# dmMaze/comic-text-detector

Hardware: NVIDIA H100
Metric: pages/sec @1024x1024 synthetic (higher is better)
Workload: dtype fp16

## Files before the change

comic-text-detector_b200/csrc/engine.cu:

```cuda
#include <cuda.h>
#include <cuda_fp16.h>
#include <cuda_runtime.h>
#include <stdarg.h>
#include <stdio.h>
#include <string.h>

#include <algorithm>
#include <cstdlib>
#include <map>
#include <string>
#include <tuple>
#include <vector>

#include "engine.h"

using namespace ctd;

namespace {
thread_local std::string g_create_error;
}

int ctd_fail(ctd_handle* h, int code, const char* fmt, ...) {
  char buf[512];
  va_list ap;
  va_start(ap, fmt);
  vsnprintf(buf, sizeof(buf), fmt, ap);
  va_end(ap);
  if (h) h->err = buf;
  else g_create_error = buf;
  return code;
}

#define CK(expr)                                                                                      \
  do {                                                                                                \
    cudaError_t _e = (expr);                                                                          \
    if (_e != cudaSuccess) return ctd_fail(h, CTD_E_CUDA, "%s: %s (%s:%d)", #expr, cudaGetErrorString(_e), __FILE__, __LINE__); \
  } while (0)

int rows_per_image(int ph, int pw) { return 3 * ((ph / 8) * (pw / 8) + (ph / 16) * (pw / 16) + (ph / 32) * (pw / 32)); }
static bool is_gemm(int kind) { return kind == CTD_OP_CONV || kind == CTD_OP_DECONV4 || kind == CTD_OP_DETECT; }

extern "C" const char* ctd_last_error(const ctd_handle* h) { return h ? h->err.c_str() : g_create_error.c_str(); }

extern "C" void ctd_destroy(ctd_handle* h) {
  if (!h) return;
  cudaSetDevice(h->cfg.device);
  ctd_pipeline_shutdown(h);
  if (h->ev_pre) {
    cudaEventSynchronize(h->ev_pre);
    cudaEventDestroy(h->ev_pre);
  }
  cudaFree(h->pre_in);
  cudaFree(h->d_pre_tab);
  for (auto& kv : h->plans)
    if (kv.second.graph) cudaGraphExecDestroy(kv.second.graph);
  for (void* p : h->d_buf) cudaFree(p);
  for (void* p : h->d_buf16) cudaFree(p);
  cudaFree(h->d_wsplit);
  cudaFree(h->d_blob); cudaFree(h->d_pages); cudaFree(h->d_blks); cudaFree(h->d_mask); cudaFree(h->d_mask_u8);
  cudaFree(h->d_lines); cudaFree(h->d_bitmap); cudaFree(h->d_labels);
  cudaFree(h->d_ccl_scratch); cudaFree(h->d_nms_ws); cudaFree(h->d_segrep_scratch);
  h->refine_scratch.release(); h->cc_scratch.release(); h->io_scratch.release(); h->in_stage.release();
  if (h->ev0) cudaEventDestroy(h->ev0);
  if (h->ev1) cudaEventDestroy(h->ev1);
  if (h->tev0) cudaEventDestroy(h->tev0);
  if (h->tev1) cudaEventDestroy(h->tev1);
  for (auto e : h->op_events) cudaEventDestroy(e);
  for (Slot& s : h->slot) s.release();
  if (h->ev_fork) cudaEventDestroy(h->ev_fork);
  if (h->ev_join) cudaEventDestroy(h->ev_join);
  if (h->ev_fork2) cudaEventDestroy(h->ev_fork2);
  if (h->ev_xjoin) cudaEventDestroy(h->ev_xjoin);
  if (h->ev_join2) cudaEventDestroy(h->ev_join2);
  if (h->ev_tin) cudaEventDestroy(h->ev_tin);
  if (h->ev_tout) cudaEventDestroy(h->ev_tout);
  if (h->side) cudaStreamDestroy(h->side);
  if (h->side2) cudaStreamDestroy(h->side2);
  if (h->copy_in) cudaStreamDestroy(h->copy_in);
  if (h->copy_out) cudaStreamDestroy(h->copy_out);
  if (h->stream) cudaStreamDestroy(h->stream);
  delete h;
}

extern "C" int ctd_create(ctd_handle** out, const ctd_config* cfg, const ctd_op* ops, int32_t n_ops,
                          const ctd_bufdesc* bufs, int32_t n_bufs, const void* blob, size_t blob_bytes) {
  ctd_handle* h = nullptr;
  if (!out || !cfg || !ops || !bufs || !blob) return ctd_fail(nullptr, CTD_E_INVALID, "null argument");
  *out = nullptr;
  if (cfg->abi_version != CTD_ABI_VERSION) return ctd_fail(nullptr, CTD_E_INVALID, "ABI version mismatch");
  if (cfg->max_h % 64 || cfg->max_w % 64 || cfg->max_batch < 1) return ctd_fail(nullptr, CTD_E_SHAPE, "bad max shape");
  int ndev = 0;
  if (cudaGetDeviceCount(&ndev) != cudaSuccess || ndev <= cfg->device)
    return ctd_fail(nullptr, CTD_E_NO_DEVICE, "no CUDA device %d (this engine has no CPU fallback)", cfg->device);
  cudaDeviceProp prop;
  if (cudaGetDeviceProperties(&prop, cfg->device) != cudaSuccess || prop.major != 9 || prop.minor != 0)
    return ctd_fail(nullptr, CTD_E_NO_DEVICE, "device %d is not sm_90 (compute %d.%d)", cfg->device, prop.major, prop.minor);
  h = new ctd_handle();
  h->cfg = *cfg;
  h->ops.assign(ops, ops + n_ops);
  h->bufs.assign(bufs, bufs + n_bufs);
  {
    h->db_ancestor.assign(size_t(n_ops), 0);
    std::vector<char> needed(size_t(n_bufs), 0);
    bool have_db = false;
    for (int i = n_ops - 1; i >= 0; --i) {
      const ctd_op& op = ops[i];
      bool anc = false;
      if (op.kind == CTD_OP_DB_TAIL && !have_db) { anc = true; have_db = true; }
      else if (have_db && op.kind != CTD_OP_DETECT && op.kind != CTD_OP_SEG_TAIL && op.kind != CTD_OP_DB_TAIL) {
        const int wbuf = op.kind == CTD_OP_SPPF_POOL ? op.src_buf[0] : op.dst_buf;
        anc = wbuf >= 0 && wbuf < n_bufs && needed[wbuf];
      }
      if (!anc) continue;
      h->db_ancestor[size_t(i)] = 1;
      for (int k = 0; k < op.n_src && k < 3; ++k)
        if (op.src_buf[k] >= 0 && op.src_buf[k] < n_bufs) needed[op.src_buf[k]] = 1;
      if (op.residual && op.dst_buf >= 0 && op.dst_buf < n_bufs) needed[op.dst_buf] = 1;
    }
    h->overlap = have_db;
  }
  h->elem = (cfg->precision == CTD_PREC_FP32_SIMT || cfg->precision == CTD_PREC_SPLIT_TC) ? 4 : 2;
  auto bail = [&](int code) { std::string e = h->err; ctd_destroy(h); g_create_error = e; return code; };
  h->detect_prm.assign(size_t(n_ops), {});
  for (int i = 0; i < n_ops; ++i) {
    if (ops[i].kind != CTD_OP_DETECT) continue;
    if (ops[i].p_off < 0 || size_t(ops[i].p_off) + sizeof(h->detect_prm[0]) > blob_bytes) {
      ctd_fail(h, CTD_E_INVALID, "op %d: detect parameters outside the blob", i);
      return bail(CTD_E_INVALID);
    }
    memcpy(h->detect_prm[size_t(i)].data(), static_cast<const char*>(blob) + ops[i].p_off, sizeof(h->detect_prm[0]));
  }
#define CKC(expr)                                                                                        \
  do {                                                                                                   \
    cudaError_t _e = (expr);                                                                             \
    if (_e != cudaSuccess) {                                                                             \
      ctd_fail(h, CTD_E_CUDA, "%s: %s (%s:%d)", #expr, cudaGetErrorString(_e), __FILE__, __LINE__);          \
      return bail(CTD_E_CUDA);                                                                           \
    }                                                                                                    \
  } while (0)
  CKC(cudaSetDevice(cfg->device));
  {
    int lo = 0, hi = 0;
    CKC(cudaDeviceGetStreamPriorityRange(&lo, &hi));
    CKC(cudaStreamCreateWithPriority(&h->stream, cudaStreamNonBlocking, lo));
    CKC(cudaStreamCreateWithPriority(&h->side, cudaStreamNonBlocking, hi));
    CKC(cudaStreamCreateWithPriority(&h->side2, cudaStreamNonBlocking, hi));
  }
  CKC(cudaEventCreateWithFlags(&h->ev_fork, cudaEventDisableTiming));
  CKC(cudaEventCreateWithFlags(&h->ev_join, cudaEventDisableTiming));
  CKC(cudaEventCreateWithFlags(&h->ev_fork2, cudaEventDisableTiming));
  CKC(cudaEventCreateWithFlags(&h->ev_xjoin, cudaEventDisableTiming));
  CKC(cudaEventCreateWithFlags(&h->ev_join2, cudaEventDisableTiming));
  CKC(cudaEventCreateWithFlags(&h->ev_tin, cudaEventDisableTiming));
  CKC(cudaEventCreateWithFlags(&h->ev_tout, cudaEventDisableTiming));
  CKC(cudaEventCreate(&h->ev0));
  CKC(cudaEventCreate(&h->ev1));
  CKC(cudaEventCreate(&h->tev0));
  CKC(cudaEventCreate(&h->tev1));
  {
    void* fn = nullptr;
    cudaDriverEntryPointQueryResult qres;
    CKC(cudaGetDriverEntryPoint("cuTensorMapEncodeTiled", &fn, cudaEnableDefault, &qres));
    if (!fn || qres != cudaDriverEntryPointSuccess) {
      ctd_fail(h, CTD_E_CUDA, "cuTensorMapEncodeTiled not available from the driver");
      return bail(CTD_E_CUDA);
    }
    h->enc = reinterpret_cast<PFN_encodeTiled>(fn);
  }
  CKC(conv_tc_init());
  CKC(conv_ends_init());
  h->blob_bytes = blob_bytes;
  CKC(cudaMalloc(&h->d_blob, blob_bytes));
  CKC(cudaMemcpy(h->d_blob, blob, blob_bytes, cudaMemcpyHostToDevice));
  const size_t nb = size_t(cfg->max_batch), mh = cfg->max_h, mw = cfg->max_w;
  h->d_buf.assign(n_bufs, nullptr);
  for (int i = 0; i < n_bufs; ++i) {
    const size_t bytes = nb * (mh / bufs[i].down) * (mw / bufs[i].down + 4) * bufs[i].channels * h->elem;
    CKC(cudaMalloc(&h->d_buf[i], bytes));
    CKC(cudaMemset(h->d_buf[i], 0, bytes));
  }
  if (cfg->precision == CTD_PREC_SPLIT_TC) {
    h->d_buf16.assign(n_bufs, nullptr);
    for (int i = 0; i < n_bufs; ++i) {
      const size_t bytes = 2 * nb * (mh / bufs[i].down) * (mw / bufs[i].down + 4) * bufs[i].channels * 2;
      CKC(cudaMalloc(&h->d_buf16[i], bytes));
      CKC(cudaMemset(h->d_buf16[i], 0, bytes));
    }
    h->wsplit_off.assign(size_t(n_ops), 0);
    std::vector<__half> ws;
    const char* hb = static_cast<const char*>(blob);
    for (int i = 0; i < n_ops; ++i) {
      const ctd_op& op = ops[i];
      if (!is_gemm(op.kind)) continue;
      int cin = 0;
      for (int k = 0; k < op.n_src; ++k) cin += op.src_c[k];
      const int taps = op.kind == CTD_OP_DECONV4 ? 4 : op.ksize * op.ksize;
      const int nph = op.kind == CTD_OP_DECONV4 ? 4 : 1;
      const size_t cnt = size_t(nph) * op.cout_pad * taps * cin;
      if (size_t(op.w32_off) + cnt * 4 > blob_bytes || size_t(op.w16_off) + cnt * 2 > blob_bytes) {
        ctd_fail(h, CTD_E_INVALID, "op %d: weights outside the blob", i);
        return bail(CTD_E_INVALID);
      }
      while (ws.size() % 128) ws.push_back(__float2half(0.f));
      h->wsplit_off[size_t(i)] = ws.size() * 2;
      const float* w32 = reinterpret_cast<const float*>(hb + op.w32_off);
      const size_t base = ws.size();
      ws.resize(base + 2 * cnt);
      for (size_t k = 0; k < cnt; ++k) {
        const __half hi = __float2half_rn(w32[k]);
        ws[base + k] = hi;
        ws[base + cnt + k] = __float2half_rn((w32[k] - __half2float(hi)) * kSplitLoScale);
      }
    }
    CKC(cudaMalloc(&h->d_wsplit, ws.size() * 2 + 256));
    CKC(cudaMemcpy(h->d_wsplit, ws.data(), ws.size() * 2, cudaMemcpyHostToDevice));
  }
  const size_t px = nb * mh * mw;
  const int no = 5 + cfg->nc;
  CKC(cudaMalloc(&h->d_pages, px * 3));
  CKC(cudaMalloc(&h->d_blks, nb * rows_per_image(mh, mw) * no * sizeof(float)));
  CKC(cudaMalloc(&h->d_mask, px * 4));
  CKC(cudaMalloc(&h->d_lines, px * 2 * 4));
  CKC(cudaMalloc(&h->d_bitmap, px));
  CKC(cudaMalloc(&h->d_labels, px * 4));
  {
    auto al = [](size_t v) { return (v + 255) / 256 * 256; };
    ArenaLayout& L = h->layout;
    L.det = al(px); L.cnt = L.det + al(nb * 300 * 6 * 4); L.nl = L.cnt + al(nb * 4);
    L.lb = L.nl + al(nb * 4); L.ls = L.lb + al(nb * 1000 * 8 * 2); L.lc = L.ls + al(nb * 1000 * 4);
    L.a_bytes = L.lc + al(nb * 4);
    L.refined = L.a_bytes;
    L.blocks = L.refined + al(px);
    const BlockSection bs = block_section_layout();
    L.rec_off = bs.rec_off; L.lines_off = bs.lines_off; L.dist_off = bs.dist_off; L.blocks_stride = bs.stride;
    L.total = L.blocks + nb * L.blocks_stride;
    CKC(cudaMalloc(&h->d_mask_u8, L.total));
    CKC(cudaMemset(h->d_mask_u8, 0, L.total));
    h->d_det = reinterpret_cast<float*>(h->d_mask_u8 + L.det);
    h->d_det_count = reinterpret_cast<int*>(h->d_mask_u8 + L.cnt);
    h->d_nlabels = reinterpret_cast<int32_t*>(h->d_mask_u8 + L.nl);
    h->d_line_boxes = reinterpret_cast<int16_t*>(h->d_mask_u8 + L.lb);
    h->d_line_scores = reinterpret_cast<float*>(h->d_mask_u8 + L.ls);
    h->d_line_count = reinterpret_cast<int32_t*>(h->d_mask_u8 + L.lc);
  }
  CKC(cudaMalloc(&h->d_ccl_scratch, px * 4 * 3));
  CKC(cudaMalloc(&h->d_segrep_scratch, segrep_scratch_bytes(int(nb), int(mh), int(mw), 1000)));
  const int cap = 4096;
  CKC(cudaMalloc(&h->d_nms_ws, nms_workspace_bytes(int(nb), cap)));
  nms_workspace_bind(h->nms, h->d_nms_ws, int(nb), cap);
  CKC(cudaDeviceSynchronize());
#undef CKC
  *out = h;
  return CTD_OK;
}

static int op_geom(ctd_handle* h, const ctd_op& op, int n, int ph, int pw, ConvGeom& g) {
  memset(&g, 0, sizeof(g));
  fill_conv_geom_taps(g, op.kind == CTD_OP_DETECT ? CTD_OP_CONV : op.kind, op.ksize, op.stride);
  g.n_img = n;
  g.n_src = op.n_src;
  const ctd_bufdesc& sb = h->bufs[op.src_buf[0]];
  g.src_h = ph / sb.down;
  g.src_w = pw / sb.down;
  g.cin_total = 0;
  for (int s = 0; s < op.n_src; ++s) {
    const ctd_bufdesc& b = h->bufs[op.src_buf[s]];
    if (b.down != sb.down) return ctd_fail(h, CTD_E_INVALID, "op sources differ in resolution");
    g.src_c[s] = op.src_c[s];
    g.src_cstride[s] = b.channels;
    g.cin_total += op.src_c[s];
  }
  g.k_total = g.taps * g.cin_total;
  g.gh = op.kind == CTD_OP_DECONV4 ? g.src_h : g.src_h / op.stride;
  g.gw = op.kind == CTD_OP_DECONV4 ? g.src_w : g.src_w / op.stride;
  g.dst_h = g.gh * g.out_mul;
  g.dst_w = g.gw * g.out_mul;
  g.cout = op.cout;
  g.cout_pad = op.cout_pad;
  if (op.dst_buf >= 0) {
    g.dst_cstride = h->bufs[op.dst_buf].channels;
    g.dst_coff = op.dst_coff;
  }
  g.act = op.act;
  g.residual = op.residual;
  return CTD_OK;
}

template <typename P>
static void set_detect(const ctd_handle* h, size_t i, int ph, int pw, P& p) {
  p.blks = h->d_blks;
  p.blks_rows_per_img = rows_per_image(ph, pw);
  int row0 = 0;
  for (int l = 0; l < h->ops[i].aux; ++l) row0 += 3 * (ph / (8 << l)) * (pw / (8 << l));
  p.level_row0 = row0;
  p.nc = h->cfg.nc;
  p.det_stride = h->detect_prm[i][0];
  for (int k = 0; k < 6; ++k) p.anchor_wh[k] = h->detect_prm[i][1 + k];
}

static bool runs_on_tensor_cores(int precision, int kind) {
  switch (precision) {
    case CTD_PREC_SPLIT_TC: return is_gemm(kind);
    case CTD_PREC_FP16_TC: return is_gemm(kind) || kind == CTD_OP_STEM || kind == CTD_OP_SEG_TAIL;
    default: return false;
  }
}

static int build_plans(ctd_handle* h, int n, int ph, int pw, ShapePlan& sp) {
  sp.tc.resize(h->ops.size());
  sp.ends.resize(h->ops.size());
  const bool split = h->cfg.precision == CTD_PREC_SPLIT_TC;
  for (size_t i = 0; i < h->ops.size(); ++i) {
    const ctd_op& op = h->ops[i];
    if (!runs_on_tensor_cores(h->cfg.precision, op.kind)) continue;
    const float* bias = reinterpret_cast<const float*>(h->d_blob + op.b_off);
    const char* e = nullptr;
    if (op.kind == CTD_OP_STEM) {
      const bool f16 = sp.input == INPUT_F32;
      e = conv_ends_plan_stem(sp.ends[i], h->enc, f16 ? static_cast<const void*>(h->in_stage.p) : h->d_pages, f16, n,
                              ph, pw, h->d_blob + op.w16_off, bias, static_cast<__half*>(h->d_buf[op.dst_buf]),
                              h->bufs[op.dst_buf].channels, op.dst_coff, op.cout, op.act);
    } else if (op.kind == CTD_OP_SEG_TAIL) {
      if (op.cout_pad != 16) return ctd_fail(h, CTD_E_INVALID, "op %zu: seg tail needs cout_pad 16", i);
      const ctd_bufdesc& sb = h->bufs[op.src_buf[0]];
      e = conv_ends_plan_seg(sp.ends[i], h->enc, static_cast<const __half*>(h->d_buf[op.src_buf[0]]), sb.channels,
                             op.src_coff[0], op.src_c[0], n, ph / sb.down, pw / sb.down, h->d_blob + op.w16_off,
                             h->d_mask, h->d_mask_u8);
    } else {
      ConvGeom g;
      if (int rc = op_geom(h, op, n, ph, pw, g)) return rc;
      const void* src[CTD_MAX_SRC];
      int coff[CTD_MAX_SRC];
      for (int s = 0; s < op.n_src; ++s) {
        src[s] = (split ? h->d_buf16 : h->d_buf)[op.src_buf[s]];
        coff[s] = op.src_coff[s];
      }
      const void* w = split ? h->d_wsplit + h->wsplit_off[i] : h->d_blob + op.w16_off;
      __half* dst = op.kind == CTD_OP_DETECT ? nullptr : static_cast<__half*>(h->d_buf[op.dst_buf]);
      e = conv_tc_plan(sp.tc[i], h->enc, g, src, coff, w, bias, dst, split);
      if (op.kind == CTD_OP_DETECT) set_detect(h, i, ph, pw, sp.tc[i].p);
    }
    if (e) return ctd_fail(h, CTD_E_INVALID, "op %zu: %s", i, e);
  }
  return CTD_OK;
}

template <typename T>
static int run_op_simt(ctd_handle* h, size_t i, int n, int ph, int pw) {
  const ctd_op& op = h->ops[i];
  ConvSimtParams p;
  memset(&p, 0, sizeof(p));
  if (int rc = op_geom(h, op, n, ph, pw, p.g)) return rc;
  for (int k = 0; k < op.n_src; ++k)
    p.src[k] = static_cast<char*>(h->d_buf[op.src_buf[k]]) + size_t(op.src_coff[k]) * sizeof(T);
  p.w = h->d_blob + (sizeof(T) == 4 ? op.w32_off : op.w16_off);
  p.bias = reinterpret_cast<const float*>(h->d_blob + op.b_off);
  if (op.kind == CTD_OP_DETECT) set_detect(h, i, ph, pw, p);
  else p.dst = h->d_buf[op.dst_buf];
  CK(conv_simt_launch<T>(p, h->stream));
  return CTD_OK;
}

template <typename T>
static int run_op_thin(ctd_handle* h, const ctd_op& op, int n, int ph, int pw, int input) {
  cudaStream_t s = h->stream;
  const ctd_bufdesc* sb = op.kind == CTD_OP_STEM ? nullptr : &h->bufs[op.src_buf[0]];
  const int sh = sb ? ph / sb->down : ph, sw = sb ? pw / sb->down : pw;
  const T* src = sb ? static_cast<const T*>(h->d_buf[op.src_buf[0]]) + op.src_coff[0] : nullptr;
  switch (op.kind) {
    case CTD_OP_STEM: {
      const float* w = reinterpret_cast<const float*>(h->d_blob + op.w32_off);
      const float* b = reinterpret_cast<const float*>(h->d_blob + op.b_off);
      T* dst = static_cast<T*>(h->d_buf[op.dst_buf]);
      const int dc = h->bufs[op.dst_buf].channels;
      if (input == INPUT_U8) {
        CK(stem_launch<T>(h->d_pages, n, ph, pw, w, b, dst, dc, op.dst_coff, op.cout, op.act, s));
      } else {
        CK(stem_launch<T>(reinterpret_cast<const float*>(h->in_stage.p), n, ph, pw, w, b, dst, dc, op.dst_coff,
                          op.cout, op.act, s));
      }
      return CTD_OK;
    }
    case CTD_OP_AVGPOOL2:
      CK(avgpool2_launch<T>(src, n, sh, sw, op.src_c[0], sb->channels,
                            static_cast<T*>(h->d_buf[op.dst_buf]) + op.dst_coff, h->bufs[op.dst_buf].channels, s));
      return CTD_OK;
    case CTD_OP_SPPF_POOL:
      CK(sppf_pool_launch<T>(static_cast<T*>(h->d_buf[op.src_buf[0]]) + op.src_coff[0], n, sh, sw, op.src_c[0],
                             sb->channels, s));
      return CTD_OK;
    case CTD_OP_UPSAMPLE2:
      CK(upsample2_launch<T>(src, n, sh, sw, op.src_c[0], sb->channels,
                             static_cast<T*>(h->d_buf[op.dst_buf]) + op.dst_coff, h->bufs[op.dst_buf].channels, s));
      return CTD_OK;
    case CTD_OP_SEG_TAIL:
      CK(seg_tail_launch<T>(src, n, sh, sw, op.src_c[0], sb->channels,
                            reinterpret_cast<const float*>(h->d_blob + op.p_off), h->d_mask, h->d_mask_u8, s));
      return CTD_OK;
    case CTD_OP_DB_TAIL:
      CK(db_tail_launch<T>(src, n, sh, sw, sb->channels, reinterpret_cast<const float*>(h->d_blob + op.p_off),
                           h->d_lines, h->d_bitmap, h->cfg.db_thresh, s));
      return CTD_OK;
    default: return ctd_fail(h, CTD_E_INVALID, "run_op_thin: bad kind %d", op.kind);
  }
}

static int split_written_slice(ctd_handle* h, const ctd_op& op, int n, int ph, int pw, int* cnt) {
  int buf = op.dst_buf, coff = op.dst_coff, c = op.cout;
  if (op.kind == CTD_OP_SPPF_POOL) { buf = op.src_buf[0]; coff = op.src_coff[0] + op.src_c[0]; c = 3 * op.src_c[0]; }
  else if (op.kind == CTD_OP_AVGPOOL2 || op.kind == CTD_OP_UPSAMPLE2) c = op.src_c[0];
  if (buf < 0 || c <= 0) return CTD_OK;
  const ctd_bufdesc& b = h->bufs[buf];
  const size_t npix = size_t(n) * (ph / b.down) * (pw / b.down);
  __half* hi = static_cast<__half*>(h->d_buf16[buf]) + coff;
  CK(split_planes_launch(static_cast<const float*>(h->d_buf[buf]) + coff, hi, hi + npix * b.channels, npix, c, b.channels,
                         h->stream));
  ++*cnt;
  return CTD_OK;
}

static int run_one_op(ctd_handle* h, size_t i, int n, int ph, int pw, const ShapePlan& sp, int* cnt) {
  const ctd_op& op = h->ops[i];
  const ConvTcPlan& tc = sp.tc[i];
  int rc = CTD_OK;
  if (tc.block_n || sp.ends[i].kind != ctd::CTD_END_NONE) {
    const cudaError_t e = tc.block_n ? conv_tc_launch(tc, h->stream) : conv_ends_launch(sp.ends[i], h->stream);
    if (e != cudaSuccess) rc = ctd_fail(h, CTD_E_CUDA, "tensor-core op %zu: %s", i, cudaGetErrorString(e));
  } else if (is_gemm(op.kind)) {
    rc = h->elem == 4 ? run_op_simt<float>(h, i, n, ph, pw) : run_op_simt<__half>(h, i, n, ph, pw);
  } else {
    rc = h->elem == 4 ? run_op_thin<float>(h, op, n, ph, pw, sp.input) : run_op_thin<__half>(h, op, n, ph, pw, sp.input);
  }
  ++*cnt;
  if (rc || h->d_buf16.empty()) return rc;
  return split_written_slice(h, op, n, ph, pw, cnt);
}

int launch_nms(ctd_handle* h, int n, int ph, int pw, cudaStream_t s, int* cnt, const int32_t* half) {
  CK(nms_launch(h->d_blks, n, rows_per_image(ph, pw), h->cfg.nc, h->cfg.conf_thresh, h->cfg.nms_thresh, h->nms, h->d_det,
                h->d_det_count, s, half));
  *cnt += kNmsLaunches;
  return CTD_OK;
}

int launch_db_post(ctd_handle* h, int n, int ph, int pw, cudaStream_t s, int* cnt) {
  CK(ccl_launch(h->d_bitmap, n, ph, pw, h->d_labels, h->d_ccl_scratch, h->d_nlabels, s));
  CK(segrep_launch(h->d_bitmap, h->d_lines, size_t(2) * ph * pw, h->d_ccl_scratch, n, ph, pw, 1000, 1.5f,
                   h->d_segrep_scratch, h->d_line_boxes, h->d_line_scores, h->d_line_count, s));
  *cnt += kCclLaunches + kSegrepLaunches;
  return CTD_OK;
}

static int run_ops(ctd_handle* h, int n, int ph, int pw, const ShapePlan& sp, int* launches, bool record = false) {
  int cnt = 0;
  size_t evi = 0;
  if (h->overlap && !record && !h->cfg.debug_skip_postproc) {
    for (size_t i = 0; i < h->ops.size(); ++i)
      if (h->db_ancestor[i])
        if (int rc = run_one_op(h, i, n, ph, pw, sp, &cnt)) return rc;
    CK(cudaEventRecord(h->ev_fork, h->stream));
    CK(cudaStreamWaitEvent(h->side, h->ev_fork, 0));
    if (int rc = launch_db_post(h, n, ph, pw, h->side, &cnt)) return rc;
    CK(cudaEventRecord(h->ev_join, h->side));
    size_t last_detect = h->ops.size();
    for (size_t i = 0; i < h->ops.size(); ++i)
      if (!h->db_ancestor[i] && h->ops[i].kind == CTD_OP_DETECT) last_detect = i;
    bool nms_forked = false;
    for (size_t i = 0; i < h->ops.size(); ++i) {
      if (h->db_ancestor[i]) continue;
      if (int rc = run_one_op(h, i, n, ph, pw, sp, &cnt)) return rc;
      if (i == last_detect) {
        CK(cudaEventRecord(h->ev_fork2, h->stream));
        CK(cudaStreamWaitEvent(h->side2, h->ev_fork2, 0));
        if (int rc = launch_nms(h, n, ph, pw, h->side2, &cnt)) return rc;
        CK(cudaEventRecord(h->ev_join2, h->side2));
        nms_forked = true;
      }
    }
    if (!nms_forked) {
      if (int rc = launch_nms(h, n, ph, pw, h->stream, &cnt)) return rc;
    } else {
      CK(cudaStreamWaitEvent(h->stream, h->ev_join2, 0));
    }
    CK(cudaStreamWaitEvent(h->stream, h->ev_join, 0));
    *launches = cnt;
    return CTD_OK;
  }
  if (record) CK(cudaEventRecord(h->op_events[evi++], h->stream));
  for (size_t i = 0; i < h->ops.size(); ++i) {
    if (int rc = run_one_op(h, i, n, ph, pw, sp, &cnt)) return rc;
    if (record) CK(cudaEventRecord(h->op_events[evi++], h->stream));
  }
  *launches = cnt;
  if (h->cfg.debug_skip_postproc) return CTD_OK;
  if (int rc = launch_nms(h, n, ph, pw, h->stream, &cnt)) return rc;
  if (record) CK(cudaEventRecord(h->op_events[evi++], h->stream));
  if (int rc = launch_db_post(h, n, ph, pw, h->stream, &cnt)) return rc;
  if (record) CK(cudaEventRecord(h->op_events[evi++], h->stream));
  *launches = cnt;
  return CTD_OK;
}

static size_t stage_elem(const ctd_handle* h) { return h->cfg.precision == CTD_PREC_FP16_TC ? 2 : 4; }

static int find_plan(ctd_handle* h, int32_t n, int32_t ph, int32_t pw, ShapePlan** out, int input = INPUT_U8) {
  if (n < 1 || n > h->cfg.max_batch) return ctd_fail(h, CTD_E_CAPACITY, "batch %d exceeds max_batch %d", n, h->cfg.max_batch);
  if (ph % 64 || pw % 64 || ph > h->cfg.max_h || pw > h->cfg.max_w || ph < 64 || pw < 64)
    return ctd_fail(h, CTD_E_SHAPE, "page %dx%d must be a multiple of 64 and <= %dx%d", ph, pw, h->cfg.max_h, h->cfg.max_w);
  CK(cudaSetDevice(h->cfg.device));
  auto key = std::make_tuple(int(n), int(ph), int(pw), input);
  auto it = h->plans.find(key);
  if (it == h->plans.end()) {
    ShapePlan sp;
    sp.input = input;
    if (input == INPUT_F32) {
      const size_t bytes = size_t(h->cfg.max_batch) * h->cfg.max_h * h->cfg.max_w * 3 * stage_elem(h);
      if (int rc = h->in_stage.grow(h, bytes, std::nullopt, size_t(1) << 40)) return rc;
    }
    if (int rc = build_plans(h, n, ph, pw, sp)) return rc;
    it = h->plans.emplace(key, std::move(sp)).first;
  }
  *out = &it->second;
  return CTD_OK;
}

int prepare_forward(ctd_handle* h, int32_t n, int32_t ph, int32_t pw, ShapePlan** out, int input) {
  ShapePlan* sp = nullptr;
  if (int rc = find_plan(h, n, ph, pw, &sp, input)) return rc;
  if (h->cfg.use_graph && !sp->graph) {
    cudaGraph_t graph;
    CK(cudaStreamBeginCapture(h->stream, cudaStreamCaptureModeThreadLocal));
    int rc = run_ops(h, n, ph, pw, *sp, &sp->launches);
    cudaError_t e = cudaStreamEndCapture(h->stream, &graph);
    if (rc) return rc;
    CK(e);
    CK(cudaGraphInstantiate(&sp->graph, graph, 0));
    cudaGraphDestroy(graph);
  }
  *out = sp;
  return CTD_OK;
}

int enqueue_forward(ctd_handle* h, int32_t n, int32_t ph, int32_t pw, ShapePlan& sp) {
  if (sp.graph) {
    CK(cudaGraphLaunch(sp.graph, h->stream));
  } else {
    if (int rc = run_ops(h, n, ph, pw, sp, &sp.launches)) return rc;
  }
  CK(cudaEventRecord(h->ev1, h->stream));
  h->last_launches = sp.launches;
  h->n = n; h->ph = ph; h->pw = pw;
  h->have_forward = true;
  return CTD_OK;
}

extern "C" int ctd_forward(ctd_handle* h, const uint8_t* pages, int32_t n, int32_t ph, int32_t pw,
                           int32_t pages_on_device) {
  if (!h || !pages) return CTD_E_INVALID;
  ShapePlan* sp = nullptr;
  if (int rc = prepare_forward(h, n, ph, pw, &sp)) return rc;
  const size_t bytes = size_t(n) * ph * pw * 3;
  CK(cudaEventRecord(h->ev0, h->stream));
  CK(cudaMemcpyAsync(h->d_pages, pages, bytes, pages_on_device ? cudaMemcpyDeviceToDevice : cudaMemcpyHostToDevice,
                     h->stream));
  return enqueue_forward(h, n, ph, pw, *sp);
}

template <typename T>
__global__ void from_f32_kernel(const float* src, T* dst, size_t n) {
  size_t i = blockIdx.x * size_t(blockDim.x) + threadIdx.x;
  if (i < n) dst[i] = T(src[i]);
}

template <typename X>
static int copy_output(ctd_handle* h, X* dst, const float* src, size_t elems) {
  if constexpr (sizeof(X) == 4) {
    CK(cudaMemcpyAsync(dst, src, elems * 4, cudaMemcpyDeviceToDevice, h->stream));
  } else {
    from_f32_kernel<__half><<<unsigned((elems + 255) / 256), 256, 0, h->stream>>>(src, dst, elems);
    CK(cudaGetLastError());
  }
  return CTD_OK;
}

template <typename X>
static int forward_tensor(ctd_handle* h, const X* x, int32_t n, int32_t ph, int32_t pw, void* stream, X* blks, X* mask,
                          X* lines) {
  if (!h || !x) return CTD_E_INVALID;
  if (reinterpret_cast<uintptr_t>(x) % 16) return ctd_fail(h, CTD_E_INVALID, "x must be 16-byte aligned");
  ShapePlan* sp = nullptr;
  if (int rc = prepare_forward(h, n, ph, pw, &sp, INPUT_F32)) return rc;
  cudaStream_t cs = static_cast<cudaStream_t>(stream);
  CK(cudaEventRecord(h->ev_tin, cs));
  CK(cudaStreamWaitEvent(h->stream, h->ev_tin, 0));
  CK(cudaEventRecord(h->ev0, h->stream));
  if (stage_elem(h) == 2)
    CK(nchw_to_hwc_launch(x, n, ph, pw, reinterpret_cast<__half*>(h->in_stage.p), h->stream));
  else
    CK(nchw_to_hwc_launch(x, n, ph, pw, reinterpret_cast<float*>(h->in_stage.p), h->stream));
  if (int rc = enqueue_forward(h, n, ph, pw, *sp)) return rc;
  const size_t px = size_t(n) * ph * pw;
  if (blks)
    if (int rc = copy_output(h, blks, h->d_blks, size_t(n) * rows_per_image(ph, pw) * (5 + h->cfg.nc))) return rc;
  if (mask)
    if (int rc = copy_output(h, mask, h->d_mask, px)) return rc;
  if (lines)
    if (int rc = copy_output(h, lines, h->d_lines, px * 2)) return rc;
  CK(cudaEventRecord(h->ev_tout, h->stream));
  CK(cudaStreamWaitEvent(cs, h->ev_tout, 0));
  return CTD_OK;
}

extern "C" int ctd_forward_tensor(ctd_handle* h, const float* x, int32_t n, int32_t ph, int32_t pw, void* stream,
                                  float* blks, float* mask, float* lines) {
  return forward_tensor(h, x, n, ph, pw, stream, blks, mask, lines);
}

extern "C" int ctd_forward_tensor_f16(ctd_handle* h, const void* x, int32_t n, int32_t ph, int32_t pw, void* stream,
                                      void* blks, void* mask, void* lines) {
  return forward_tensor(h, static_cast<const __half*>(x), n, ph, pw, stream, static_cast<__half*>(blks),
                        static_cast<__half*>(mask), static_cast<__half*>(lines));
}

template <bool kPinned>
int GrowBuf<kPinned>::grow(ctd_handle* h, size_t bytes, std::optional<cudaStream_t> sync, size_t headroom) {
  if (bytes <= cap) return CTD_OK;
  if (sync) CK(cudaStreamSynchronize(*sync));
  release();
  const size_t alloc = bytes + bytes / headroom;
  if (kPinned) CK(cudaHostAlloc(reinterpret_cast<void**>(&p), alloc, cudaHostAllocDefault));
  else CK(cudaMalloc(reinterpret_cast<void**>(&p), alloc));
  cap = alloc;
  return CTD_OK;
}
template <bool kPinned>
void GrowBuf<kPinned>::release() {
  if (kPinned && p) cudaFreeHost(p);
  if (!kPinned) cudaFree(p);
  p = nullptr;
  cap = 0;
}
template struct GrowBuf<false>;
template struct GrowBuf<true>;

void Slot::release() {
  cudaFree(d_stage_in);
  cudaFree(d_stage_out);
  for (cudaEvent_t e : {ev_in_done, ev_in_free, ev_out_ready, ev_out_done, ev_post_done})
    if (e) cudaEventDestroy(e);
  if (pinned) cudaFreeHost(pinned);
  pg_in.release(); pg_res.release(); pg_aux.release(); out_in.release(); d_crop.release(); h_crop.release();
  cudaFree(d_pg_tab);
  if (h_pg_tab) cudaFreeHost(h_pg_tab);
  *this = Slot();
}

extern "C" int ctd_resize_linear_u8(ctd_handle* h, const uint8_t* src, int32_t sh, int32_t sw, int32_t channels, uint8_t* dst,
                                    int32_t dh, int32_t dw) {
  if (!h || !src || !dst) return CTD_E_INVALID;
  if ((channels != 1 && channels != 3) || sh < 1 || sw < 1 || dh < 1 || dw < 1) return ctd_fail(h, CTD_E_SHAPE, "bad resize shape");
  CK(cudaSetDevice(h->cfg.device));
  const size_t sb = size_t(sh) * sw * channels, db = size_t(dh) * dw * channels;
  const size_t so = (sb + 255) / 256 * 256;
  if (int rc = h->io_scratch.grow(h, so + db, h->stream)) return rc;
  CK(cudaMemcpyAsync(h->io_scratch.p, src, sb, cudaMemcpyHostToDevice, h->stream));
  CK(resize_linear_u8_launch(h->io_scratch.p, sh, sw, size_t(sw) * channels, channels, h->io_scratch.p + so, dh, dw, dh, dw, h->stream));
  CK(cudaMemcpyAsync(dst, h->io_scratch.p + so, db, cudaMemcpyDeviceToHost, h->stream));
  CK(cudaStreamSynchronize(h->stream));
  return CTD_OK;
}

extern "C" int ctd_join(ctd_handle* h, ctd_handle* other) {
  if (!h || !other) return CTD_E_INVALID;
  if (h == other) return CTD_OK;
  if (h->cfg.device != other->cfg.device) return ctd_fail(h, CTD_E_INVALID, "ctd_join: handles live on different devices");
  CK(cudaSetDevice(h->cfg.device));
  CK(cudaEventRecord(other->ev_xjoin, other->stream));
  CK(cudaStreamWaitEvent(h->stream, other->ev_xjoin, 0));
  return CTD_OK;
}

#define NEED_FWD()                                                                     \
  if (!h) return CTD_E_INVALID;                                                        \
  if (!h->have_forward) return ctd_fail(h, CTD_E_INVALID, "no forward pass has been run"); \
  CK(cudaSetDevice(h->cfg.device));

extern "C" int ctd_get_net_outputs(ctd_handle* h, float* blks, float* mask, float* lines) {
  NEED_FWD();
  const size_t px = size_t(h->n) * h->ph * h->pw;
  if (blks)
    CK(cudaMemcpyAsync(blks, h->d_blks, size_t(h->n) * rows_per_image(h->ph, h->pw) * (5 + h->cfg.nc) * 4,
                       cudaMemcpyDeviceToHost, h->stream));
  if (mask) CK(cudaMemcpyAsync(mask, h->d_mask, px * 4, cudaMemcpyDeviceToHost, h->stream));
  if (lines) CK(cudaMemcpyAsync(lines, h->d_lines, px * 8, cudaMemcpyDeviceToHost, h->stream));
  CK(cudaStreamSynchronize(h->stream));
  return CTD_OK;
}

extern "C" int ctd_get_mask_u8(ctd_handle* h, uint8_t* mask_u8) {
  NEED_FWD();
  if (!mask_u8) return CTD_E_INVALID;
  CK(cudaMemcpyAsync(mask_u8, h->d_mask_u8, size_t(h->n) * h->ph * h->pw, cudaMemcpyDeviceToHost, h->stream));
  CK(cudaStreamSynchronize(h->stream));
  return CTD_OK;
}

extern "C" int ctd_get_detections(ctd_handle* h, float* det, int32_t* det_count) {
  NEED_FWD();
  if (!det || !det_count) return CTD_E_INVALID;
  CK(cudaMemcpyAsync(det, h->d_det, size_t(h->n) * 300 * 6 * 4, cudaMemcpyDeviceToHost, h->stream));
  CK(cudaMemcpyAsync(det_count, h->d_det_count, size_t(h->n) * 4, cudaMemcpyDeviceToHost, h->stream));
  CK(cudaStreamSynchronize(h->stream));
  return CTD_OK;
}

extern "C" int ctd_get_nms_status(ctd_handle* h, int32_t* cand_total, int32_t* cap) {
  if (!h) return CTD_E_INVALID;
  CK(cudaSetDevice(h->cfg.device));
  if (cap) *cap = h->nms.cap;
  if (cand_total) {
    const int n = h->have_forward ? h->n : 1;
    CK(cudaMemcpyAsync(cand_total, h->nms.cand_total, size_t(n) * 4, cudaMemcpyDeviceToHost, h->stream));
    CK(cudaStreamSynchronize(h->stream));
  }
  return CTD_OK;
}

extern "C" int ctd_get_db_components(ctd_handle* h, uint8_t* bitmap, int32_t* labels, int32_t* n_labels) {
  NEED_FWD();
  const size_t px = size_t(h->n) * h->ph * h->pw;
  if (bitmap) CK(cudaMemcpyAsync(bitmap, h->d_bitmap, px, cudaMemcpyDeviceToHost, h->stream));
  if (labels) CK(cudaMemcpyAsync(labels, h->d_labels, px * 4, cudaMemcpyDeviceToHost, h->stream));
  if (n_labels) CK(cudaMemcpyAsync(n_labels, h->d_nlabels, size_t(h->n) * 4, cudaMemcpyDeviceToHost, h->stream));
  CK(cudaStreamSynchronize(h->stream));
  return CTD_OK;
}

extern "C" int ctd_get_text_lines(ctd_handle* h, int16_t* boxes, float* scores, int32_t* counts) {
  NEED_FWD();
  if (!boxes || !scores || !counts) return CTD_E_INVALID;
  CK(cudaMemcpyAsync(boxes, h->d_line_boxes, size_t(h->n) * 1000 * 8 * 2, cudaMemcpyDeviceToHost, h->stream));
  CK(cudaMemcpyAsync(scores, h->d_line_scores, size_t(h->n) * 1000 * 4, cudaMemcpyDeviceToHost, h->stream));
  CK(cudaMemcpyAsync(counts, h->d_line_count, size_t(h->n) * 4, cudaMemcpyDeviceToHost, h->stream));
  CK(cudaStreamSynchronize(h->stream));
  return CTD_OK;
}

extern "C" int ctd_seg_represent(ctd_handle* h, const float* pred, int32_t ih, int32_t iw, float thresh, int16_t* boxes,
                                 float* scores, int32_t* count) {
  if (!h || !pred || !boxes || !scores || !count) return CTD_E_INVALID;
  if (ih < 1 || iw < 1 || size_t(ih) * iw > size_t(h->cfg.max_h) * h->cfg.max_w || ih > 2048 || iw > 2048)
    return ctd_fail(h, CTD_E_CAPACITY, "map larger than the workspace");
  CK(cudaSetDevice(h->cfg.device));
  const size_t px = size_t(ih) * iw;
  CK(cudaMemcpyAsync(h->d_lines, pred, px * 4, cudaMemcpyHostToDevice, h->stream));
  CK(binarize_launch(h->d_lines, px, thresh, h->d_bitmap, h->stream));
  CK(ccl_launch(h->d_bitmap, 1, ih, iw, h->d_labels, h->d_ccl_scratch, h->d_nlabels, h->stream));
  CK(segrep_launch(h->d_bitmap, h->d_lines, px, h->d_ccl_scratch, 1, ih, iw, 1000, 1.5f, h->d_segrep_scratch,
                   h->d_line_boxes, h->d_line_scores, h->d_line_count, h->stream));
  CK(cudaMemcpyAsync(boxes, h->d_line_boxes, 1000 * 8 * 2, cudaMemcpyDeviceToHost, h->stream));
  CK(cudaMemcpyAsync(scores, h->d_line_scores, 1000 * 4, cudaMemcpyDeviceToHost, h->stream));
  CK(cudaMemcpyAsync(count, h->d_line_count, 4, cudaMemcpyDeviceToHost, h->stream));
  CK(cudaStreamSynchronize(h->stream));
  h->have_forward = false;
  return CTD_OK;
}

extern "C" int ctd_last_forward_ms(ctd_handle* h, float* ms) {
  NEED_FWD();
  if (!ms) return CTD_E_INVALID;
  CK(cudaEventSynchronize(h->ev1));
  CK(cudaEventElapsedTime(ms, h->ev0, h->ev1));
  return CTD_OK;
}

extern "C" int ctd_last_launch_count(ctd_handle* h, int32_t* launches) {
  NEED_FWD();
  if (!launches) return CTD_E_INVALID;
  *launches = h->last_launches;
  return CTD_OK;
}

extern "C" int ctd_timer_start(ctd_handle* h) {
  if (!h) return CTD_E_INVALID;
  CK(cudaSetDevice(h->cfg.device));
  CK(cudaEventRecord(h->tev0, h->stream));
  return CTD_OK;
}
extern "C" int ctd_timer_stop(ctd_handle* h, float* ms) {
  if (!h || !ms) return CTD_E_INVALID;
  CK(cudaSetDevice(h->cfg.device));
  CK(cudaEventRecord(h->tev1, h->stream));
  CK(cudaEventSynchronize(h->tev1));
  CK(cudaEventElapsedTime(ms, h->tev0, h->tev1));
  return CTD_OK;
}

extern "C" int ctd_profile_forward(ctd_handle* h, const uint8_t* pages, int32_t n, int32_t ph, int32_t pw,
                                   int32_t pages_on_device, float* op_ms, int32_t cap) {
  if (!h || !pages || !op_ms) return CTD_E_INVALID;
  const int need = int(h->ops.size()) + 2;
  if (cap < need) return ctd_fail(h, CTD_E_INVALID, "op_ms needs %d entries", need);
  ShapePlan* sp = nullptr;
  if (int rc = find_plan(h, n, ph, pw, &sp)) return rc;
  while (int(h->op_events.size()) < need + 1) {
    cudaEvent_t e;
    CK(cudaEventCreate(&e));
    h->op_events.push_back(e);
  }
  CK(cudaMemcpyAsync(h->d_pages, pages, size_t(n) * ph * pw * 3,
                     pages_on_device ? cudaMemcpyDeviceToDevice : cudaMemcpyHostToDevice, h->stream));
  int launches = 0;
  if (int rc = run_ops(h, n, ph, pw, *sp, &launches, true)) return rc;
  CK(cudaStreamSynchronize(h->stream));
  const int nev = h->cfg.debug_skip_postproc ? int(h->ops.size()) : need;
  for (int i = 0; i < need; ++i) op_ms[i] = 0.f;
  for (int i = 0; i < nev; ++i) CK(cudaEventElapsedTime(&op_ms[i], h->op_events[i], h->op_events[i + 1]));
  h->n = n; h->ph = ph; h->pw = pw;
  h->have_forward = true;
  h->last_launches = launches;
  return CTD_OK;
}

template <typename T>
__global__ void to_f32_kernel(const T* src, float* dst, size_t n) {
  size_t i = blockIdx.x * size_t(blockDim.x) + threadIdx.x;
  if (i < n) dst[i] = float(src[i]);
}

extern "C" int ctd_debug_read_buffer(ctd_handle* h, int32_t buf, float* out, size_t out_elems) {
  NEED_FWD();
  if (buf < 0 || buf >= int(h->bufs.size()) || !out) return ctd_fail(h, CTD_E_INVALID, "bad buffer id");
  const ctd_bufdesc& b = h->bufs[buf];
  const size_t elems = size_t(h->n) * (h->ph / b.down) * (h->pw / b.down) * b.channels;
  if (out_elems < elems) return ctd_fail(h, CTD_E_INVALID, "buffer %d holds %zu elements", buf, elems);
  float* tmp = nullptr;
  CK(cudaMalloc(&tmp, elems * 4));
  if (h->elem == 4) to_f32_kernel<float><<<unsigned((elems + 255) / 256), 256, 0, h->stream>>>(static_cast<float*>(h->d_buf[buf]), tmp, elems);
  else to_f32_kernel<__half><<<unsigned((elems + 255) / 256), 256, 0, h->stream>>>(static_cast<__half*>(h->d_buf[buf]), tmp, elems);
  cudaError_t e = cudaMemcpyAsync(out, tmp, elems * 4, cudaMemcpyDeviceToHost, h->stream);
  if (e == cudaSuccess) e = cudaStreamSynchronize(h->stream);
  cudaFree(tmp);
  CK(e);
  return CTD_OK;
}

extern "C" int ctd_debug_write_buffer(ctd_handle* h, int32_t buf, const float* in, int32_t n, int32_t ph, int32_t pw) {
  if (!h || !in) return CTD_E_INVALID;
  if (buf < 0 || buf >= int(h->bufs.size())) return ctd_fail(h, CTD_E_INVALID, "bad buffer id");
  if (n < 1 || n > h->cfg.max_batch || ph > h->cfg.max_h || pw > h->cfg.max_w) return ctd_fail(h, CTD_E_CAPACITY, "shape");
  CK(cudaSetDevice(h->cfg.device));
  const ctd_bufdesc& b = h->bufs[buf];
  const size_t elems = size_t(n) * (ph / b.down) * (pw / b.down) * b.channels;
  float* tmp = nullptr;
  CK(cudaMalloc(&tmp, elems * 4));
  cudaError_t e = cudaMemcpyAsync(tmp, in, elems * 4, cudaMemcpyHostToDevice, h->stream);
  if (e == cudaSuccess) {
    if (h->elem == 4) from_f32_kernel<float><<<unsigned((elems + 255) / 256), 256, 0, h->stream>>>(tmp, static_cast<float*>(h->d_buf[buf]), elems);
    else from_f32_kernel<__half><<<unsigned((elems + 255) / 256), 256, 0, h->stream>>>(tmp, static_cast<__half*>(h->d_buf[buf]), elems);
    if (h->cfg.precision == CTD_PREC_SPLIT_TC) {
      const size_t npix = elems / b.channels;
      __half* hi = static_cast<__half*>(h->d_buf16[buf]);
      e = split_planes_launch(static_cast<const float*>(h->d_buf[buf]), hi, hi + elems, npix, b.channels, b.channels, h->stream);
    }
    if (e == cudaSuccess) e = cudaStreamSynchronize(h->stream);
  }
  cudaFree(tmp);
  CK(e);
  return CTD_OK;
}

extern "C" int ctd_debug_run_ops(ctd_handle* h, const uint8_t* pages, int32_t n, int32_t ph, int32_t pw, int32_t first_op,
                                 int32_t last_op) {
  if (!h) return CTD_E_INVALID;
  if (first_op < 0 || last_op >= int(h->ops.size()) || first_op > last_op) return ctd_fail(h, CTD_E_INVALID, "bad op range");
  ShapePlan* sp = nullptr;
  if (int rc = find_plan(h, n, ph, pw, &sp)) return rc;
  if (pages) CK(cudaMemcpyAsync(h->d_pages, pages, size_t(n) * ph * pw * 3, cudaMemcpyHostToDevice, h->stream));
  int cnt = 0;
  for (int i = first_op; i <= last_op; ++i)
    if (int rc = run_one_op(h, size_t(i), n, ph, pw, *sp, &cnt)) return rc;
  CK(cudaStreamSynchronize(h->stream));
  h->n = n; h->ph = ph; h->pw = pw;
  h->have_forward = true;
  h->last_launches = cnt;
  return CTD_OK;
}

extern "C" int ctd_debug_postprocess(ctd_handle* h, const float* blks, const float* lines, int32_t n, int32_t ph,
                                     int32_t pw) {
  if (!h || !blks || !lines) return CTD_E_INVALID;
  if (h->cfg.debug_skip_postproc) return ctd_fail(h, CTD_E_INVALID, "ctd_debug_postprocess needs the full pipeline");
  ShapePlan* sp = nullptr;
  if (int rc = find_plan(h, n, ph, pw, &sp)) return rc;
  const size_t hw = size_t(ph) * pw;
  CK(cudaMemcpyAsync(h->d_blks, blks, size_t(n) * rows_per_image(ph, pw) * (5 + h->cfg.nc) * 4, cudaMemcpyHostToDevice,
                     h->stream));
  CK(cudaMemcpyAsync(h->d_lines, lines, size_t(n) * hw * 2 * 4, cudaMemcpyHostToDevice, h->stream));
  for (int i = 0; i < n; ++i)
    CK(binarize_launch(h->d_lines + size_t(i) * 2 * hw, hw, h->cfg.db_thresh, h->d_bitmap + size_t(i) * hw, h->stream));
  int cnt = 0;
  if (int rc = launch_nms(h, n, ph, pw, h->stream, &cnt)) return rc;
  if (int rc = launch_db_post(h, n, ph, pw, h->stream, &cnt)) return rc;
  CK(cudaStreamSynchronize(h->stream));
  h->n = n; h->ph = ph; h->pw = pw;
  h->have_forward = true;
  h->last_launches = cnt;
  return CTD_OK;
}

int cc_device(ctd_handle* h, const uint8_t* d_img, int ih, int iw, int stats_cap, int32_t** d_stats, int32_t* n_labels) {
  const size_t px = size_t(ih) * iw;
  auto al = [](size_t v) { return (v + 255) / 256 * 256; };
  const size_t o_scr = al(px * 4);
  const size_t scr_bytes = al(std::max(px * 12, size_t(stats_cap > 0 ? stats_cap : 0) * 5 * 4));
  const size_t o_nl = o_scr + scr_bytes;
  if (int rc = h->cc_scratch.grow(h, o_nl + 256, h->stream)) return rc;
  uint8_t* base = h->cc_scratch.p;
  int32_t* d_labels = reinterpret_cast<int32_t*>(base);
  int32_t* d_scr = reinterpret_cast<int32_t*>(base + o_scr);
  int32_t* d_nl = reinterpret_cast<int32_t*>(base + o_nl);
  CK(ccl_launch(d_img, 1, ih, iw, d_labels, d_scr, d_nl, h->stream));
  if (stats_cap > 0) CK(ccl_stats_launch(d_labels, ih, iw, d_scr, stats_cap, h->stream));
  CK(cudaMemcpyAsync(n_labels, d_nl, 4, cudaMemcpyDeviceToHost, h->stream));
  CK(cudaStreamSynchronize(h->stream));
  if (d_stats) *d_stats = d_scr;
  return CTD_OK;
}

extern "C" int ctd_connected_components(ctd_handle* h, const uint8_t* img, int32_t ih, int32_t iw, int32_t* labels,
                                        int32_t* stats, int32_t stats_cap, int32_t* n_labels) {
  if (!h || !img || !labels || !n_labels) return CTD_E_INVALID;
  if (ih < 1 || iw < 1 || size_t(ih) * iw > kCclMaxPixels) return ctd_fail(h, CTD_E_SHAPE, "bad image size %dx%d", ih, iw);
  CK(cudaSetDevice(h->cfg.device));
  const size_t px = size_t(ih) * iw;
  if (int rc = h->io_scratch.grow(h, px + 256, h->stream)) return rc;
  CK(cudaMemcpyAsync(h->io_scratch.p, img, px, cudaMemcpyHostToDevice, h->stream));
  int32_t* d_stats = nullptr;
  if (int rc = cc_device(h, h->io_scratch.p, ih, iw, (stats && stats_cap > 0) ? stats_cap : 0, &d_stats, n_labels)) return rc;
  CK(cudaMemcpyAsync(labels, h->cc_scratch.p, px * 4, cudaMemcpyDeviceToHost, h->stream));
  if (stats && stats_cap > 0) CK(cudaMemcpyAsync(stats, d_stats, size_t(stats_cap) * 5 * 4, cudaMemcpyDeviceToHost, h->stream));
  CK(cudaStreamSynchronize(h->stream));
  return CTD_OK;
}

extern "C" int ctd_nms(ctd_handle* h, const float* pred, int32_t rows, float conf_thresh, float iou_thresh, float* det,
                       int32_t* det_count) {
  return ctd_nms_dtype(h, pred, rows, CTD_DTYPE_F32, conf_thresh, iou_thresh, det, det_count);
}

extern "C" int ctd_nms_dtype(ctd_handle* h, const void* pred, int32_t rows, int32_t dtype, float conf_thresh,
                             float iou_thresh, float* det, int32_t* det_count) {
  if (!h || !pred || !det || !det_count) return CTD_E_INVALID;
  if (dtype != CTD_DTYPE_F32 && dtype != CTD_DTYPE_F16) return ctd_fail(h, CTD_E_INVALID, "bad dtype %d", dtype);
  const int no = 5 + h->cfg.nc;
  if (rows > rows_per_image(h->cfg.max_h, h->cfg.max_w) * h->cfg.max_batch)
    return ctd_fail(h, CTD_E_CAPACITY, "too many prediction rows");
  CK(cudaSetDevice(h->cfg.device));
  const size_t elems = size_t(rows) * no;
  const int32_t* d_half = nullptr;
  if (dtype == CTD_DTYPE_F16) {
    std::vector<float> wide(elems);
    const __half* p = static_cast<const __half*>(pred);
    for (size_t i = 0; i < elems; ++i) wide[i] = __half2float(p[i]);
    if (int rc = h->io_scratch.grow(h, 256, h->stream)) return rc;
    const int32_t one = 1;
    CK(cudaMemcpyAsync(h->io_scratch.p, &one, sizeof(one), cudaMemcpyHostToDevice, h->stream));
    CK(cudaMemcpyAsync(h->d_blks, wide.data(), elems * 4, cudaMemcpyHostToDevice, h->stream));
    CK(cudaStreamSynchronize(h->stream));
    d_half = reinterpret_cast<const int32_t*>(h->io_scratch.p);
  } else {
    CK(cudaMemcpyAsync(h->d_blks, pred, elems * 4, cudaMemcpyHostToDevice, h->stream));
  }
  CK(nms_launch(h->d_blks, 1, rows, h->cfg.nc, conf_thresh, iou_thresh, h->nms, h->d_det, h->d_det_count, h->stream,
                d_half));
  CK(cudaMemcpyAsync(det, h->d_det, 300 * 6 * 4, cudaMemcpyDeviceToHost, h->stream));
  CK(cudaMemcpyAsync(det_count, h->d_det_count, 4, cudaMemcpyDeviceToHost, h->stream));
  CK(cudaStreamSynchronize(h->stream));
  h->have_forward = false;
  return CTD_OK;
}
```

comic-text-detector_b200/csrc/engine.h:

```cpp
#pragma once
#include <cuda.h>
#include <cuda_runtime.h>
#include <stdint.h>

#include <math.h>

#include <algorithm>
#include <array>
#include <condition_variable>
#include <deque>
#include <map>
#include <mutex>
#include <optional>
#include <string>
#include <thread>
#include <tuple>
#include <vector>

#include "kernels.h"

using ctd::ConvTcPlan;
using ctd::ConvEndsPlan;
using ctd::NmsWorkspace;
using ctd::PFN_encodeTiled;

struct ArenaLayout {
  size_t det, cnt, nl, lb, ls, lc, a_bytes, refined, blocks, blocks_stride, rec_off, lines_off, dist_off, total;
};

struct BlockSection {
  size_t rec_off, lines_off, dist_off, stride;
};
inline BlockSection block_section_layout() {
  auto al = [](size_t v) { return (v + 255) / 256 * 256; };
  BlockSection b;
  b.rec_off = 64;
  b.lines_off = b.rec_off + al(size_t(CTD_MAX_BLOCKS) * sizeof(ctd_block));
  b.dist_off = b.lines_off + al(size_t(CTD_MAX_BLOCKS) * 32);
  b.stride = b.dist_off + al(size_t(CTD_MAX_BLOCK_DIST) * 8);
  return b;
}

struct Letterbox {
  int unpad_h, unpad_w;
  float ratio_x, ratio_y;
};
inline bool letterbox_of(int ih, int iw, int net_h, int net_w, Letterbox& lb) {
  if (ih < 1 || iw < 1 || net_h < 1 || net_w < 1) return false;
  const double r = std::min(double(net_h) / ih, double(net_w) / iw);
  lb.unpad_w = int(nearbyint(iw * r));
  lb.unpad_h = int(nearbyint(ih * r));
  if (lb.unpad_w < 1 || lb.unpad_h < 1 || lb.unpad_w > net_w || lb.unpad_h > net_h) return false;
  lb.ratio_x = float(double(iw) / double(lb.unpad_w));
  lb.ratio_y = float(double(ih) / double(lb.unpad_h));
  return true;
}

struct PagesHead {
  size_t det, cnt, lb, ls, lc, masks;
};
PagesHead pages_head(int n);

struct JobPage {
  int ih, iw;
  float ratio_x, ratio_y;
  size_t off;
  char* section;
  const uint8_t* mask;
  std::vector<int32_t> wins, boxes;
  std::vector<ctd_region_line> lines;
  std::vector<ctd_region> plan;
  size_t plan_bytes = 0;
};

struct Planes {
  const uint8_t* img;
  uint8_t *mask, *ref, *ref2, *thr;
  size_t total;
};

struct PipeJob {
  int slot = 0, refine_mode = 0;
  char* results_host = nullptr;
  bool rows = false;
  PagesHead head{};
  size_t refined = 0;
  std::vector<JobPage> pages;
  Planes pl{};
  uint8_t* d_blocks = nullptr;
  size_t blocks_bytes = 0;
  int keep_undetected = 0;
  int textheight = 0;
  int results_on_device = 0;
  int refined_input = 0;
  std::vector<ctd_device_page> dev;
  const int32_t* nonfinite = nullptr;
};

struct ctd_handle;
template <bool kPinned>
struct GrowBuf {
  uint8_t* p = nullptr;
  size_t cap = 0;
  int grow(ctd_handle* h, size_t bytes, std::optional<cudaStream_t> sync, size_t headroom = 4);
  void release();
};
using DevBuf = GrowBuf<false>;
using PinnedBuf = GrowBuf<true>;

struct Slot {
  uint8_t* d_stage_in = nullptr;
  uint8_t* d_stage_out = nullptr;
  cudaEvent_t ev_in_done = nullptr, ev_in_free = nullptr, ev_out_ready = nullptr, ev_out_done = nullptr;
  cudaEvent_t ev_post_done = nullptr;
  bool busy = false;
  bool crops = false, on_device = false, masks = true, collected = false;
  int state = 0;
  int rc = 0;
  std::string err;
  char* pinned = nullptr;
  DevBuf pg_in, pg_res, pg_aux;
  DevBuf out_in;
  ctd::PageGeom* h_pg_tab = nullptr;
  ctd::PageGeom* d_pg_tab = nullptr;
  std::vector<ctd_page_entry> dev_pages;
  std::vector<ctd_region> crop_plan;
  std::vector<int32_t> crop_first;
  std::vector<size_t> crop_base;
  DevBuf d_crop;
  PinnedBuf h_crop;
  size_t crop_px_off = 0, crop_bytes = 0;

  void start(bool want_crops, bool want_on_device, bool want_masks = true) {
    crops = want_crops;
    on_device = want_on_device;
    masks = want_masks;
    collected = false;
  }
  void release();
};

struct RefineJob {
  std::vector<ctd::RefineWin> wins;
  std::vector<ctd::RefineChunk> chunks;
  size_t total_px = 0;
  size_t total_words = 0;
  void add(int x1, int y1, int x2, int y2, size_t page_off, int iw, int ih);
  size_t table_bytes() const;
};

struct RegionJob {
  std::vector<ctd::RegionDev> regs;
  std::vector<ctd::RegionTile> tiles;
  size_t out_bytes = 0;
  int add(const ctd_region* plan, int n, const ctd::RegionPage& pg, long long out_base);
  size_t table_bytes() const;
  void write_tables(char* dst) const;
};

enum { INPUT_U8 = 0, INPUT_F32 = 1 };

struct ShapePlan {
  int input = INPUT_U8;
  std::vector<ConvTcPlan> tc;
  std::vector<ConvEndsPlan> ends;
  cudaGraphExec_t graph = nullptr;
  int launches = 0;
};
struct ctd_handle {
  ctd_config cfg{};
  std::vector<ctd_op> ops;
  std::vector<ctd_bufdesc> bufs;
  std::vector<std::array<float, 7>> detect_prm;
  std::string err;
  cudaStream_t stream = nullptr;
  cudaEvent_t ev0 = nullptr, ev1 = nullptr, tev0 = nullptr, tev1 = nullptr;
  std::vector<cudaEvent_t> op_events;
  PFN_encodeTiled enc = nullptr;
  char* d_blob = nullptr;
  size_t blob_bytes = 0;
  std::vector<void*> d_buf;
  std::vector<void*> d_buf16;
  char* d_wsplit = nullptr;
  std::vector<size_t> wsplit_off;
  int elem = 2;
  uint8_t* d_pages = nullptr;
  float* d_blks = nullptr;
  float* d_mask = nullptr;
  uint8_t* d_mask_u8 = nullptr;
  float* d_lines = nullptr;
  uint8_t* d_bitmap = nullptr;
  float* d_det = nullptr;
  int* d_det_count = nullptr;
  int32_t* d_labels = nullptr;
  int32_t* d_nlabels = nullptr;
  int32_t* d_ccl_scratch = nullptr;
  void* d_segrep_scratch = nullptr;
  DevBuf refine_scratch;
  DevBuf cc_scratch;
  DevBuf io_scratch;
  int16_t* d_line_boxes = nullptr;
  float* d_line_scores = nullptr;
  int32_t* d_line_count = nullptr;
  void* d_nms_ws = nullptr;
  NmsWorkspace nms{};
  std::map<std::tuple<int, int, int, int>, ShapePlan> plans;
  DevBuf in_stage;
  cudaEvent_t ev_tin = nullptr, ev_tout = nullptr;
  cudaStream_t copy_in = nullptr, copy_out = nullptr;
  Slot slot[2];
  bool overlap = false;
  cudaStream_t side = nullptr, side2 = nullptr;
  cudaEvent_t ev_fork = nullptr, ev_join = nullptr, ev_fork2 = nullptr, ev_join2 = nullptr;
  cudaEvent_t ev_xjoin = nullptr;
  std::vector<char> db_ancestor;
  ArenaLayout layout{};
  cudaStream_t post = nullptr;
  size_t pipe_pinned_cap = 0;
  std::thread pipe_thread;
  std::mutex pipe_mu;
  std::condition_variable pipe_cv, pipe_done_cv;
  std::deque<PipeJob> pipe_queue;
  bool pipe_quit = false;
  int host_threads = 4;
  size_t pg_gather_off = 0;
  size_t pg_out_off = 0, pg_half_off = 0, pg_flag_off = 0;
  cudaStream_t dev_out = nullptr;
  DevBuf pg_cc;
  DevBuf post_refine;
  uint8_t* pre_in = nullptr;
  size_t pre_in_cap = 0;
  char* d_pre_tab = nullptr;
  cudaEvent_t ev_pre = nullptr;
  int n = 0, ph = 0, pw = 0;
  int last_launches = 0;
  bool have_forward = false;
};


int ctd_fail(ctd_handle* h, int code, const char* fmt, ...);
int prepare_forward(ctd_handle* h, int32_t n, int32_t ph, int32_t pw, ShapePlan** out, int input = INPUT_U8);
int enqueue_forward(ctd_handle* h, int32_t n, int32_t ph, int32_t pw, ShapePlan& sp);
int rows_per_image(int ph, int pw);
int launch_nms(ctd_handle* h, int n, int ph, int pw, cudaStream_t s, int* cnt, const int32_t* half = nullptr);
int launch_db_post(ctd_handle* h, int n, int ph, int pw, cudaStream_t s, int* cnt);
int cc_device(ctd_handle* h, const uint8_t* d_img, int ih, int iw, int stats_cap, int32_t** d_stats, int32_t* n_labels);
int launch_refine(ctd_handle* h, const RefineJob& job, const uint8_t* d_img, const uint8_t* d_mask, int refine_mode,
                  uint8_t* d_out, cudaStream_t st, DevBuf& scratch, char* pinned);
void ctd_pipeline_shutdown(ctd_handle* h);
```

comic-text-detector_b200/csrc/kernels.h:

```cpp
#pragma once
#include <cuda.h>
#include <cuda_fp16.h>
#include <cuda_runtime.h>
#include <stdint.h>

#include "../../include/ctd_b200.h"

namespace ctd {

constexpr int kMaxTaps = 9;

constexpr float kSplitLoScale = 2048.0f;
constexpr float kSplitLoUnscale = 1.0f / 2048.0f;
constexpr int kMaxPhases = 4;

struct ConvGeom {
  int n_img;
  int gh, gw;
  int dst_h, dst_w;
  int out_mul;
  int n_phase;
  int taps;
  int cin_total;
  int k_total;
  int n_src;
  int src_c[CTD_MAX_SRC];
  int src_cstride[CTD_MAX_SRC];
  int src_h, src_w;
  int in_stride;
  int8_t tap_dy[kMaxPhases][kMaxTaps];
  int8_t tap_dx[kMaxPhases][kMaxTaps];
  int cout, cout_pad;
  int dst_cstride, dst_coff;
  int act, residual;
};

void fill_conv_geom_taps(ConvGeom& g, int kind, int ksize, int stride);

struct alignas(64) ConvTcParams {
  CUtensorMap a_map[CTD_MAX_SRC][4];
  CUtensorMap b_map;
  CUtensorMap d_map[kMaxPhases];
  ConvGeom g;
  int kb_elems;
  int src_kblocks[CTD_MAX_SRC];
  int tiles_x, tiles_y;
  int8_t tap_map[kMaxPhases][kMaxTaps];
  __half* dst;
  int dst_map_cols;
  const float* bias;
  float* blks;
  int blks_rows_per_img;
  int level_row0;
  float det_stride;
  float anchor_wh[6];
  int nc;
  int split;
  int split_img_off;
  int split_row_off;
};
static_assert(sizeof(ConvTcParams) <= 4096, "ConvTcParams: kernel parameters are limited to 4 KB");

struct ConvTcPlan {
  ConvTcParams p;
  int block_n;
  int tile_h;
  dim3 grid;
  size_t smem_bytes;
};

typedef CUresult (*PFN_encodeTiled)(CUtensorMap*, CUtensorMapDataType, cuuint32_t, void*, const cuuint64_t*,
                                    const cuuint64_t*, const cuuint32_t*, const cuuint32_t*, CUtensorMapInterleave,
                                    CUtensorMapSwizzle, CUtensorMapL2promotion, CUtensorMapFloatOOBfill);

const char* conv_tc_plan(ConvTcPlan& plan, PFN_encodeTiled enc, const ConvGeom& g, const void* const src_ptr[],
                         const int src_coff[], const void* w16, const float* bias, __half* dst, int split = 0);
cudaError_t conv_tc_launch(const ConvTcPlan& plan, cudaStream_t s);
cudaError_t conv_tc_init();

enum { CTD_END_NONE = 0, CTD_END_STEM = 1, CTD_END_SEG = 2, CTD_END_STEM_F16 = 3 };
struct alignas(64) ConvEndsParams {
  CUtensorMap a_map;
  CUtensorMap b_map;
  CUtensorMap d_map;
  int n_img, gh, gw;
  int tiles_x, tiles_y;
  const float* bias;
  float* mask_f32;
  uint8_t* mask_u8;
};
struct ConvEndsPlan {
  ConvEndsParams p;
  int kind = CTD_END_NONE;
  dim3 grid;
  size_t smem_bytes;
};
const char* conv_ends_plan_stem(ConvEndsPlan& plan, PFN_encodeTiled enc, const void* pages, bool f16_page, int n,
                                int ph, int pw, const void* w16, const float* bias, __half* dst, int dst_cstride,
                                int dst_coff, int cout, int act);
const char* conv_ends_plan_seg(ConvEndsPlan& plan, PFN_encodeTiled enc, const __half* src, int src_cstride,
                               int src_coff, int src_c, int n, int gh, int gw, const void* w16, float* mask_f32,
                               uint8_t* mask_u8);
cudaError_t conv_ends_launch(const ConvEndsPlan& plan, cudaStream_t s);
cudaError_t conv_ends_init();

struct ConvSimtParams {
  ConvGeom g;
  const void* src[CTD_MAX_SRC];
  const void* w;
  const float* bias;
  void* dst;
  float* blks;
  int blks_rows_per_img, level_row0, nc;
  float det_stride;
  float anchor_wh[6];
};
template <typename T>
cudaError_t conv_simt_launch(const ConvSimtParams& p, cudaStream_t s);

template <typename T, typename P>
cudaError_t stem_launch(const P* pages, int n, int h, int w, const float* wgt ,
                        const float* bias, T* dst, int dst_cstride, int dst_coff, int cout, int act, cudaStream_t s);
template <typename X, typename S>
cudaError_t nchw_to_hwc_launch(const X* x, int n, int h, int w, S* dst, cudaStream_t s);
cudaError_t split_planes_launch(const float* src, __half* hi, __half* lo, size_t npix, int c, int cstride,
                                cudaStream_t s);
template <typename T>
cudaError_t avgpool2_launch(const T* src, int n, int h, int w, int c, int src_cstride, T* dst, int dst_cstride,
                            cudaStream_t s);
template <typename T>
cudaError_t sppf_pool_launch(T* buf, int n, int h, int w, int c, int cstride, cudaStream_t s);
template <typename T>
cudaError_t upsample2_launch(const T* src, int n, int h, int w, int c, int src_cstride, T* dst, int dst_cstride,
                             cudaStream_t s);
template <typename T>
cudaError_t seg_tail_launch(const T* src, int n, int h, int w, int c, int cstride, const float* wgt ,
                            float* mask_f32, uint8_t* mask_u8, cudaStream_t s);
template <typename T>
cudaError_t db_tail_launch(const T* src, int n, int h, int w, int cstride, const float* params, float* lines,
                           uint8_t* bitmap, float db_thresh, cudaStream_t s);

struct NmsWorkspace {
  float* cand;
  int* cand_count;
  int* cand_total;
  float* sorted;
  unsigned long long* mask;
  int cap;
};
cudaError_t nms_launch(const float* blks, int n, int rows, int nc, float conf, float iou, NmsWorkspace& ws,
                       float* det , int* det_count, cudaStream_t s, const int32_t* half = nullptr);
constexpr int kNmsLaunches = 5;
size_t nms_workspace_bytes(int n, int cap);
void nms_workspace_bind(NmsWorkspace& ws, void* base, int n, int cap);

cudaError_t ccl_launch(const uint8_t* img, int n, int h, int w, int32_t* labels, int32_t* scratch ,
                       int32_t* n_labels, cudaStream_t s);
constexpr int kCclLaunches = 8;
constexpr size_t kCclMaxPixels = size_t(1) << 28;
cudaError_t ccl_stats_launch(const int32_t* labels, int h, int w, int32_t* stats, int cap, cudaStream_t s);

size_t segrep_scratch_bytes(int n, int h, int w, int max_cand);
cudaError_t segrep_launch(const uint8_t* bitmap, const float* pred, size_t pred_page_stride, const int* Lf, int n, int h,
                          int w, int max_cand, float unclip_ratio, void* scratch, int16_t* boxes, float* scores,
                          int* n_contours, cudaStream_t s);
constexpr int kSegrepLaunches = 15;
cudaError_t binarize_launch(const float* pred, size_t count, float thresh, uint8_t* bitmap, cudaStream_t s);

cudaError_t resize_linear_u8_launch(const uint8_t* src, int sh, int sw, size_t src_pitch, int channels, uint8_t* dst,
                                    int dh, int dw, int canvas_h, int canvas_w, cudaStream_t s);
struct PageGeom {
  long long src_off, dst_off;
  int ih, iw, unpad_h, unpad_w, row0, pad;
};
cudaError_t letterbox_batch_launch(const uint8_t* src, const PageGeom* d_tab, int n, uint8_t* dst, int net_h, int net_w,
                                   cudaStream_t s);
cudaError_t backproject_batch_launch(const uint8_t* mask, int net_h, int net_w, const PageGeom* d_tab, int n,
                                     int total_rows, uint8_t* dst, cudaStream_t s);
enum PreFormat { PRE_F32_NCHW = 0, PRE_F16_NCHW = 1, PRE_U8_NHWC = 2 };
cudaError_t letterbox_tensor_launch(const uint8_t* src, const PageGeom* d_tab, int n, void* dst, int net_h, int net_w,
                                    int format, bool reverse, cudaStream_t s);

struct GatherPage {
  const uint8_t* src;
  long long sh, sw, sc;
  uint8_t* dst;
  int ih, iw, row0, fast, ch, pad;
};
cudaError_t gather_pages_launch(const GatherPage* d_tab, int n, int total_rows, cudaStream_t s);
cudaError_t upload_table_launch(const void* host, size_t bytes, void* dst, cudaStream_t s);

struct OutputGather {
  const void* blks;
  long long bsr, bsc;
  const void* mask;
  long long msh, msw;
  const void* lines;
  long long lsh, lsw;
  int rows, half;
};
cudaError_t gather_outputs_launch(const OutputGather* d_tab, int n, int h, int w, int no, int ws_rows, float thresh,
                                  uint8_t* mask_u8, float* lines, uint8_t* bitmap, float* blks, int32_t* flags,
                                  cudaStream_t s);

struct RefineWin {
  int x1, y1, x2, y2;
  long long off;
  long long page_off;
  int pitch;
};
struct RefineChunk { int win, y0, x0, rows, woff; };
constexpr int kRefineChunkPx = 8192;
__host__ __device__ constexpr int refine_rows_per_chunk(int rw) {
  return kRefineChunkPx / rw >= 8 ? (kRefineChunkPx / rw) & ~3 : (kRefineChunkPx / rw > 0 ? kRefineChunkPx / rw : 1);
}
size_t refine_scratch_bytes(size_t total_px, size_t n_chunks);
size_t refine_mk_state_bytes(int n_wins);
cudaError_t refine_mk_launch(const uint8_t* d_img, const uint8_t* d_mask, const RefineWin* d_wins, int n_wins,
                             const RefineChunk* d_chunks, int n_chunks, int n_multi_chunks, void* d_state, size_t total_px,
                             void* scratch, int refine_mode, uint8_t* d_out, cudaStream_t s);

constexpr int kRegionTilePx = 256;
struct RegionPage {
  const uint8_t* data;
  long long sh, sw, sc;
  int ih, iw;
};
struct RegionDev {
  long long offset;
  const uint8_t* page;
  long long sh, sw, sc;
  int out_h, out_w;
  int warp_w, bw0;
  int rotate, ih, iw, pad;
  double m[9];
};
struct RegionTile { int region, first; };
cudaError_t warp_regions_launch(const RegionDev* d_regs, const RegionTile* d_tiles, int n_tiles, uint8_t* d_out,
                                cudaStream_t s);

}
```

comic-text-detector_b200/csrc/pipeline.cu:

```cuda
#include <cuda.h>
#include <cuda_runtime.h>
#include <math.h>
#include <stdint.h>
#include <string.h>

#include <algorithm>
#include <thread>
#include <vector>

#include "engine.h"

using namespace ctd;

#define CK(expr)                                                                                      \
  do {                                                                                                \
    cudaError_t _e = (expr);                                                                          \
    if (_e != cudaSuccess) return ctd_fail(h, CTD_E_CUDA, "%s: %s (%s:%d)", #expr, cudaGetErrorString(_e), __FILE__, __LINE__); \
  } while (0)

namespace {
inline void norm_slice(int& lo, int& hi, int n) {
  if (lo < 0) lo = std::max(lo + n, 0);
  if (hi < 0) hi = std::max(hi + n, 0);
  lo = std::min(lo, n);
  hi = std::min(hi, n);
  if (hi < lo) hi = lo;
}
}

void RefineJob::add(int x1, int y1, int x2, int y2, size_t page_off, int iw, int ih) {
  norm_slice(x1, x2, iw);
  norm_slice(y1, y2, ih);
  const size_t a = (x2 > x1 && y2 > y1) ? size_t(x2 - x1) * (y2 - y1) : 0;
  if (a == 0) return;
  const int wi = int(wins.size());
  const int rw = x2 - x1, rh = y2 - y1;
  const int rows_per = refine_rows_per_chunk(rw);
  for (int y0 = 0; y0 < rh; y0 += rows_per)
    for (int x0 = 0; x0 < rw; x0 += kRefineChunkPx) {
      const int rows = std::min(rows_per, rh - y0);
      chunks.push_back(RefineChunk{wi, y0, x0, rows, int(total_words)});
      total_words += (size_t(rows) * std::min(rw - x0, kRefineChunkPx) + 31) / 32;
    }
  wins.push_back(RefineWin{x1, y1, x2, y2, (long long)total_px, (long long)page_off, iw});
  total_px = (total_px + a + 3) / 4 * 4;
}
size_t RefineJob::table_bytes() const {
  auto al = [](size_t v) { return (v + 255) / 256 * 256; };
  return al(wins.size() * sizeof(RefineWin)) + al(chunks.size() * sizeof(RefineChunk));
}

int launch_refine(ctd_handle* h, const RefineJob& job, const uint8_t* d_img, const uint8_t* d_mask, int refine_mode,
                  uint8_t* d_out, cudaStream_t st, DevBuf& scratch, char* pinned) {
  if (job.wins.empty()) return CTD_OK;
  auto al = [](size_t v) { return (v + 255) / 256 * 256; };
  const size_t tb = job.table_bytes();
  const size_t sb = refine_mk_state_bytes(int(job.wins.size()));
  if (int rc = scratch.grow(h, tb + sb + refine_scratch_bytes(job.total_px, job.chunks.size()), st, 2)) return rc;
  char* base = reinterpret_cast<char*>(scratch.p);
  const size_t wb = al(job.wins.size() * sizeof(RefineWin));
  std::vector<char> local;
  char* stage = pinned;
  if (!stage) { local.resize(tb); stage = local.data(); }
  memcpy(stage, job.wins.data(), job.wins.size() * sizeof(RefineWin));
  int n_multi = 0;
  {
    RefineChunk* hc = reinterpret_cast<RefineChunk*>(stage + wb);
    const size_t nc = job.chunks.size();
    size_t tail = nc;
    for (size_t i = 0; i < nc;) {
      size_t j = i;
      while (j < nc && job.chunks[j].win == job.chunks[i].win) ++j;
      if (j - i > 1) {
        for (size_t k = i; k < j; ++k) hc[n_multi++] = job.chunks[k];
      } else {
        hc[--tail] = job.chunks[i];
      }
      i = j;
    }
  }
  CK(cudaMemcpyAsync(base, stage, tb, cudaMemcpyHostToDevice, st));
  if (!pinned) CK(cudaStreamSynchronize(st));
  CK(refine_mk_launch(d_img, d_mask, reinterpret_cast<const RefineWin*>(base), int(job.wins.size()),
                      reinterpret_cast<const RefineChunk*>(base + wb), int(job.chunks.size()), n_multi, base + tb,
                      job.total_px, base + tb + sb, refine_mode, d_out, st));
  return CTD_OK;
}

extern "C" int ctd_refine_mask(ctd_handle* h, const uint8_t* img, const uint8_t* mask, int32_t ih, int32_t iw,
                               const int32_t* windows, int32_t n_win, int32_t refine_mode, uint8_t* out) {
  if (!h || !img || !mask || !out || (n_win > 0 && !windows)) return CTD_E_INVALID;
  if (ih < 1 || iw < 1) return ctd_fail(h, CTD_E_SHAPE, "bad image size");
  CK(cudaSetDevice(h->cfg.device));
  RefineJob job;
  for (int i = 0; i < n_win; ++i) job.add(windows[4 * i], windows[4 * i + 1], windows[4 * i + 2], windows[4 * i + 3], 0, iw, ih);
  const size_t px = size_t(ih) * iw, pxa = (px + 255) / 256 * 256;
  if (int rc = h->io_scratch.grow(h, pxa * 5 + 1024, h->stream)) return rc;
  uint8_t* d_img = h->io_scratch.p;
  uint8_t* d_mask = d_img + pxa * 3;
  uint8_t* d_out = d_mask + pxa;
  CK(cudaMemcpyAsync(d_img, img, px * 3, cudaMemcpyHostToDevice, h->stream));
  CK(cudaMemcpyAsync(d_mask, mask, px, cudaMemcpyHostToDevice, h->stream));
  CK(cudaMemsetAsync(d_out, 0, pxa, h->stream));
  if (int rc = launch_refine(h, job, d_img, d_mask, refine_mode, d_out, h->stream, h->refine_scratch, nullptr))
    return rc;
  CK(cudaMemcpyAsync(out, d_out, px, cudaMemcpyDeviceToHost, h->stream));
  CK(cudaStreamSynchronize(h->stream));
  return CTD_OK;
}

namespace {
struct PageIn {
  const float* det; int n_det;
  const int16_t* line_boxes; const float* line_scores; int n_lines;
  const uint8_t* mask; int im_w, im_h;
  float ratio_x, ratio_y;
};

PageIn page_in(const char* res, const PagesHead& head, int i, const JobPage& p) {
  PageIn in;
  in.det = reinterpret_cast<const float*>(res + head.det) + size_t(i) * 300 * 6;
  in.n_det = std::min(std::max(reinterpret_cast<const int32_t*>(res + head.cnt)[i], 0), 300);
  in.line_boxes = reinterpret_cast<const int16_t*>(res + head.lb) + size_t(i) * 1000 * 8;
  in.line_scores = reinterpret_cast<const float*>(res + head.ls) + size_t(i) * 1000;
  in.n_lines = std::min(std::max(reinterpret_cast<const int32_t*>(res + head.lc)[i], 0), 1000);
  in.mask = p.mask; in.im_w = p.iw; in.im_h = p.ih; in.ratio_x = p.ratio_x; in.ratio_y = p.ratio_y;
  return in;
}

std::array<int64_t, 4> expand_textwindow(int64_t x1, int64_t y1, int64_t x2, int64_t y2, int im_w, int im_h) {
  const int64_t w = x2 - x1, h = y2 - y1;
  const int64_t pad = int64_t(nearbyint((double(std::max(h, w)) * 0.25 + double(std::min(h, w)) * 0.75) / 16.0));
  return {std::max<int64_t>(0, x1 - pad), std::max<int64_t>(0, y1 - pad), std::min<int64_t>(im_w - 1, x2 + pad),
          std::min<int64_t>(im_h - 1, y2 + pad)};
}

int host_group_page(const PageIn& in, const BlockSection& L, bool lines_out, JobPage& p) {
  char* section = p.section;
  std::vector<int32_t> bxy(size_t(in.n_det) * 4), bcls(size_t(in.n_det));
  for (int i = 0; i < in.n_det; ++i) {
    const float* d = in.det + 6 * i;
    bxy[4 * i + 0] = int32_t(d[0] * in.ratio_x);
    bxy[4 * i + 1] = int32_t(d[1] * in.ratio_y);
    bxy[4 * i + 2] = int32_t(d[2] * in.ratio_x);
    bxy[4 * i + 3] = int32_t(d[3] * in.ratio_y);
    bcls[i] = int32_t(d[5]);
  }
  std::vector<int32_t> lines;
  lines.reserve(size_t(in.n_lines) * 8);
  for (int i = 0; i < in.n_lines; ++i) {
    if (!(in.line_scores[i] > 0.6f)) continue;
    const int16_t* b = in.line_boxes + 8 * i;
    for (int k = 0; k < 4; ++k) {
      lines.push_back(int32_t(double(b[2 * k]) * double(in.ratio_x)));
      lines.push_back(int32_t(double(b[2 * k + 1]) * double(in.ratio_y)));
    }
  }
  ctd_page_blocks* hdr = reinterpret_cast<ctd_page_blocks*>(section);
  ctd_block* rec = reinterpret_cast<ctd_block*>(section + L.rec_off);
  int32_t* lout = reinterpret_cast<int32_t*>(section + L.lines_off);
  double* dout = reinterpret_cast<double*>(section + L.dist_off);
  int32_t nb = 0;
  int rc = ctd_group_output(bxy.data(), bcls.data(), in.n_det, lines.data(), int32_t(lines.size() / 8), in.im_w, in.im_h, in.mask,
                            1, rec, CTD_MAX_BLOCKS, lout, CTD_MAX_BLOCKS, dout, CTD_MAX_BLOCK_DIST, &nb);
  hdr->flags = 0;
  if (rc == CTD_E_CAPACITY) {
    std::vector<double> big(size_t(CTD_MAX_BLOCKS) * CTD_MAX_BLOCKS / 4);
    rc = ctd_group_output(bxy.data(), bcls.data(), in.n_det, lines.data(), int32_t(lines.size() / 8), in.im_w, in.im_h, in.mask, 1,
                          rec, CTD_MAX_BLOCKS, lout, CTD_MAX_BLOCKS, big.data(), int32_t(big.size()), &nb);
    if (rc == CTD_OK)
      for (int i = 0; i < nb; ++i) { rec[i].n_dist = 0; rec[i].dist_off = 0; }
    hdr->flags |= 1;
  }
  if (rc != CTD_OK) { hdr->n_blocks = 0; hdr->n_lines = 0; hdr->n_dist = 0; hdr->flags |= 2; return rc; }
  hdr->n_blocks = nb;
  int32_t tl = 0, td = 0;
  for (int i = 0; i < nb; ++i) { tl += rec[i].n_lines; td += rec[i].n_dist; }
  hdr->n_lines = tl;
  hdr->n_dist = td;
  for (int i = 0; i < nb; ++i) {
    const int32_t* xy = rec[i].xyxy;
    const auto win = expand_textwindow(xy[0], xy[1], xy[2], xy[3], in.im_w, in.im_h);
    for (int64_t v : win) p.wins.push_back(int32_t(v));
    p.boxes.insert(p.boxes.end(), xy, xy + 4);
  }
  if (!lines_out) return CTD_OK;
  p.lines.reserve(size_t(tl));
  for (int b = 0; b < nb; ++b)
    for (int k = 0; k < rec[b].n_lines; ++k) {
      ctd_region_line l{};
      const int32_t* q = lout + size_t(rec[b].line_off + k) * 8;
      for (int j = 0; j < 8; ++j) l.quad[j] = double(q[j]);
      l.language = rec[b].language;
      l.vertical = rec[b].vertical ? 1 : 0;
      l.font_size = rec[b].font_size;
      p.lines.push_back(l);
    }
  return CTD_OK;
}

template <typename F>
void for_each_page(int n, int threads, F fn) {
  const int nthreads = std::max(1, std::min(n, threads));
  if (nthreads == 1) {
    for (int i = 0; i < n; ++i) fn(i);
    return;
  }
  std::vector<std::thread> th;
  for (int t = 0; t < nthreads; ++t)
    th.emplace_back([&, t] { for (int i = t; i < n; i += nthreads) fn(i); });
  for (auto& x : th) x.join();
}

__global__ void undetected_prep_kernel(uint8_t* __restrict__ mask, const uint8_t* __restrict__ refined,
                                       uint8_t* __restrict__ thr, size_t n) {
  const size_t i = blockIdx.x * size_t(blockDim.x) + threadIdx.x;
  if (i >= n) return;
  uint8_t m = mask[i];
  if (refined[i] > 30) { m = 0; mask[i] = 0; }
  thr[i] = m > 30 ? 255 : 0;
}
__global__ void or_kernel(uint8_t* __restrict__ dst, const uint8_t* __restrict__ src, size_t n) {
  const size_t i = blockIdx.x * size_t(blockDim.x) + threadIdx.x;
  if (i < n) dst[i] |= src[i];
}

int refine_undetected(ctd_handle* h, const std::vector<JobPage>& pages, const Planes& pl, int refine_mode,
                      cudaStream_t st, DevBuf& cc, DevBuf& refine_scratch, char* pinned, size_t pinned_cap) {
  auto al = [](size_t v) { return (v + 255) / 256 * 256; };
  const int n = int(pages.size());
  const size_t total_px = pl.total;
  undetected_prep_kernel<<<unsigned((total_px + 255) / 256), 256, 0, st>>>(pl.mask, pl.ref, pl.thr, total_px);
  CK(cudaGetLastError());
  size_t max_px = 0;
  std::vector<int> cap(static_cast<size_t>(n));
  std::vector<size_t> stats_off(static_cast<size_t>(n));
  for (int i = 0; i < n; ++i) max_px = std::max(max_px, size_t(pages[i].ih) * pages[i].iw);
  const size_t o_scr = al(max_px * 4);
  size_t o = o_scr + al(max_px * 12);
  for (int i = 0; i < n; ++i) {
    cap[size_t(i)] = ((pages[i].ih + 1) / 2) * ((pages[i].iw + 1) / 2) + 2;
    stats_off[size_t(i)] = o;
    o += al(size_t(cap[size_t(i)]) * 5 * 4);
  }
  const size_t o_nl = o;
  if (int rc = cc.grow(h, o_nl + al(size_t(n) * 4), st)) return rc;
  uint8_t* base = cc.p;
  int32_t* d_labels = reinterpret_cast<int32_t*>(base);
  int32_t* d_scr = reinterpret_cast<int32_t*>(base + o_scr);
  int32_t* d_nl = reinterpret_cast<int32_t*>(base + o_nl);
  for (int i = 0; i < n; ++i) {
    const JobPage& p = pages[size_t(i)];
    int32_t* d_stats = reinterpret_cast<int32_t*>(base + stats_off[size_t(i)]);
    CK(ccl_launch(pl.thr + p.off, 1, p.ih, p.iw, d_labels, d_scr, d_nl + i, st));
    CK(ccl_stats_launch(d_labels, p.ih, p.iw, d_stats, cap[size_t(i)], st));
  }
  std::vector<int32_t> n_lab(static_cast<size_t>(n));
  CK(cudaMemcpyAsync(n_lab.data(), d_nl, size_t(n) * 4, cudaMemcpyDeviceToHost, st));
  CK(cudaStreamSynchronize(st));
  std::vector<std::vector<int32_t>> stats(static_cast<size_t>(n));
  for (int i = 0; i < n; ++i) {
    stats[size_t(i)].resize(size_t(std::max(n_lab[size_t(i)], 0)) * 5);
    if (n_lab[size_t(i)] > 0)
      CK(cudaMemcpyAsync(stats[size_t(i)].data(), base + stats_off[size_t(i)], stats[size_t(i)].size() * 4,
                         cudaMemcpyDeviceToHost, st));
  }
  CK(cudaStreamSynchronize(st));
  RefineJob rj2;
  for (int i = 0; i < n; ++i) {
    const JobPage& p = pages[size_t(i)];
    const std::vector<int32_t>& xyxy = p.boxes;
    const size_t nb = xyxy.size() / 4;
    bool first_valid = true;
    for (int li = 0; li < n_lab[size_t(i)]; ++li) {
      const int32_t* s5 = &stats[size_t(i)][size_t(li) * 5];
      if (!(s5[4] > 50)) continue;
      if (first_valid) { first_valid = false; continue; }
      const int64_t bb[4] = {s5[0], s5[1], int64_t(s5[0]) + s5[2], int64_t(s5[1]) + s5[3]};
      int64_t score = -1;
      for (size_t b = 0; b < nb; ++b) {
        const int32_t* q = &xyxy[4 * b];
        const int64_t x1 = std::max<int64_t>(q[0], bb[0]), y1 = std::max<int64_t>(q[1], bb[1]);
        const int64_t x2 = std::min<int64_t>(q[2], bb[2]), y2 = std::min<int64_t>(q[3], bb[3]);
        const int64_t a = (y2 < y1 || x2 < x1) ? -1 : (y2 - y1) * (x2 - x1);
        if (a > score) score = a;
      }
      if (double(score) / double(s5[2]) / double(s5[3]) < 0.5) {
        const auto w4 = expand_textwindow(bb[0], bb[1], bb[2], bb[3], p.iw, p.ih);
        rj2.add(int(w4[0]), int(w4[1]), int(w4[2]), int(w4[3]), p.off, p.iw, p.ih);
      }
    }
  }
  if (!rj2.wins.empty()) {
    CK(cudaMemsetAsync(pl.ref2, 0, total_px, st));
    char* stage = rj2.table_bytes() <= pinned_cap ? pinned : nullptr;
    if (int rc = launch_refine(h, rj2, pl.img, pl.mask, refine_mode, pl.ref2, st, refine_scratch, stage)) return rc;
    or_kernel<<<unsigned((total_px + 255) / 256), 256, 0, st>>>(pl.ref, pl.ref2, total_px);
    CK(cudaGetLastError());
  }
  return CTD_OK;
}
}

extern "C" int ctd_results_layout(ctd_handle* h, ctd_results_layout_t* out) {
  if (!h || !out) return CTD_E_INVALID;
  const ArenaLayout& L = h->layout;
  out->max_batch = h->cfg.max_batch; out->max_h = h->cfg.max_h; out->max_w = h->cfg.max_w; out->reserved = 0;
  out->total_bytes = L.total;
  out->mask_u8 = 0; out->det = L.det; out->det_count = L.cnt; out->n_labels = L.nl;
  out->line_boxes = L.lb; out->line_scores = L.ls; out->line_count = L.lc;
  out->phase_a_bytes = L.a_bytes;
  out->mask_refined = L.refined; out->blocks = L.blocks; out->blocks_stride = L.blocks_stride;
  out->blk_records_off = L.rec_off; out->blk_lines_off = L.lines_off; out->blk_dist_off = L.dist_off;
  return CTD_OK;
}

PagesHead pages_head(int n) {
  auto al = [](size_t v) { return (v + 255) / 256 * 256; };
  const size_t nb = size_t(n);
  PagesHead hd;
  hd.det = 0;
  hd.cnt = hd.det + al(nb * 300 * 6 * 4);
  hd.lb = hd.cnt + al(nb * 4);
  hd.ls = hd.lb + al(nb * 1000 * 8 * 2);
  hd.lc = hd.ls + al(nb * 1000 * 4);
  hd.masks = hd.lc + al(nb * 4);
  return hd;
}

static size_t plan_planes(ctd_page_entry* pages, int n, size_t mask_plane) {
  auto al = [](size_t v) { return (v + 255) / 256 * 256; };
  size_t total = 0;
  for (int i = 0; i < n; ++i) {
    pages[i].page_off = int64_t(total * 3);
    pages[i].mask_off = int64_t(mask_plane + total);
    total += al(size_t(pages[i].ih) * size_t(pages[i].iw));
  }
  for (int i = 0; i < n; ++i) pages[i].refined_off = pages[i].mask_off + int64_t(total);
  return total;
}

extern "C" int ctd_pages_plan(ctd_page_entry* pages, int32_t n, int32_t net_h, int32_t net_w, size_t* input_bytes,
                              size_t* results_bytes) {
  if (!input_bytes || !results_bytes || n < 0 || (n > 0 && !pages)) return CTD_E_INVALID;
  if (net_h < 64 || net_w < 64 || net_h % 64 || net_w % 64) return CTD_E_SHAPE;
  auto al = [](size_t v) { return (v + 255) / 256 * 256; };
  const PagesHead hd = pages_head(n);
  for (int i = 0; i < n; ++i) {
    Letterbox lb;
    if (!letterbox_of(pages[i].ih, pages[i].iw, net_h, net_w, lb)) return CTD_E_SHAPE;
    pages[i].unpad_h = lb.unpad_h;
    pages[i].unpad_w = lb.unpad_w;
  }
  const size_t total = plan_planes(pages, n, hd.masks);
  const size_t stride = al(block_section_layout().stride);
  const size_t blocks = hd.masks + 2 * total;
  for (int i = 0; i < n; ++i) pages[i].blocks_off = int64_t(blocks + size_t(i) * stride);
  *input_bytes = total * 3;
  *results_bytes = blocks + size_t(n) * stride;
  return CTD_OK;
}

extern "C" int ctd_refine_plan(ctd_page_entry* pages, int32_t n, const int32_t* xyxy, const int32_t* n_blocks,
                               int32_t* windows, int32_t* status, size_t* input_bytes, size_t* results_bytes) {
  if (!input_bytes || !results_bytes || n < 0 || (n > 0 && (!pages || !n_blocks))) return CTD_E_INVALID;
  int64_t nb = 0;
  for (int i = 0; i < n; ++i) {
    if (pages[i].ih < 1 || pages[i].iw < 1) return CTD_E_SHAPE;
    if (n_blocks[i] < 0) return CTD_E_INVALID;
    nb += n_blocks[i];
  }
  if (nb > INT32_MAX) return CTD_E_CAPACITY;
  if (nb > 0 && (!xyxy || !windows || !status)) return CTD_E_INVALID;
  for (int i = 0; i < n; ++i) {
    pages[i].unpad_h = pages[i].unpad_w = 0;
    pages[i].blocks_off = 0;
  }
  const size_t total = plan_planes(pages, n, 0);
  size_t b = 0;
  for (int i = 0; i < n; ++i) {
    const int ih = pages[i].ih, iw = pages[i].iw;
    for (int k = 0; k < n_blocks[i]; ++k, ++b) {
      const int32_t* q = xyxy + 4 * b;
      const auto w = expand_textwindow(q[0], q[1], q[2], q[3], iw, ih);
      bool fits = true;
      for (int j = 0; j < 4; ++j) {
        fits = fits && w[j] >= INT32_MIN && w[j] <= INT32_MAX;
        windows[4 * b + j] = int32_t(std::min<int64_t>(std::max<int64_t>(w[j], INT32_MIN), INT32_MAX));
      }
      int x1 = windows[4 * b], y1 = windows[4 * b + 1], x2 = windows[4 * b + 2], y2 = windows[4 * b + 3];
      norm_slice(x1, x2, iw);
      norm_slice(y1, y2, ih);
      status[b] = !fits ? 2 : (x2 > x1 && y2 > y1) ? 0 : 1;
    }
  }
  *input_bytes = total * 5;
  *results_bytes = total * 2;
  return CTD_OK;
}

static int finish_batch(ctd_handle* h, const PipeJob& job, cudaStream_t st) {
  if (!job.results_on_device && job.pl.ref) {
    char* res = job.results_host;
    if (job.keep_undetected) CK(cudaMemcpyAsync(res + job.head.masks, job.pl.mask, job.pl.total, cudaMemcpyDeviceToHost, st));
    CK(cudaMemcpyAsync(res + job.refined, job.pl.ref, job.pl.total, cudaMemcpyDeviceToHost, st));
  }
  CK(cudaEventRecord(h->slot[job.slot].ev_post_done, st));
  return CTD_OK;
}

static std::vector<RegionPage> region_pages(const PipeJob& job) {
  std::vector<RegionPage> src;
  for (size_t i = 0; i < job.pages.size(); ++i) {
    const JobPage& p = job.pages[i];
    if (i < job.dev.size() && job.dev[i].data) {
      const ctd_device_page& d = job.dev[i];
      src.push_back(RegionPage{d.data, (long long)d.stride_h, (long long)d.stride_w, (long long)d.stride_c, p.ih, p.iw});
    } else {
      src.push_back(RegionPage{job.pl.img + p.off * 3, (long long)p.iw * 3, 3, 1, p.ih, p.iw});
    }
  }
  return src;
}

static int crop_stage(ctd_handle* h, Slot& s, const std::vector<RegionPage>& src, const std::vector<JobPage>& pages,
                      bool to_host, cudaStream_t st) {
  const int n = int(src.size());
  RegionJob rg;
  s.crop_plan.clear();
  s.crop_first.assign(size_t(n) + 1, 0);
  s.crop_base.assign(size_t(n) + 1, 0);
  size_t base = 0;
  for (int i = 0; i < n; ++i) {
    const std::vector<ctd_region>& p = pages[size_t(i)].plan;
    if (int bad = rg.add(p.data(), int(p.size()), src[size_t(i)], (long long)base); bad >= 0)
      return ctd_fail(h, CTD_E_INVALID, "malformed crop plan entry %d on page %d of the batch", bad, i);
    s.crop_first[size_t(i)] = int32_t(s.crop_plan.size());
    s.crop_base[size_t(i)] = base;
    for (ctd_region r : p) {
      r.offset += int64_t(base);
      s.crop_plan.push_back(r);
    }
    base += pages[size_t(i)].plan_bytes;
  }
  s.crop_first[size_t(n)] = int32_t(s.crop_plan.size());
  s.crop_base[size_t(n)] = base;
  if (s.crop_plan.size() > size_t(INT32_MAX) || rg.tiles.size() > size_t(INT32_MAX))
    return ctd_fail(h, CTD_E_CAPACITY, "too many crops in one batch");
  s.crop_bytes = base;
  s.crop_px_off = 0;
  if (rg.tiles.empty()) return CTD_OK;
  const size_t tb = rg.table_bytes(), px = s.crop_bytes;
  if (int rc = s.d_crop.grow(h, tb + px, st)) return rc;
  if (int rc = s.h_crop.grow(h, to_host ? tb + px : tb, st)) return rc;
  uint8_t* d_tab = s.d_crop.p;
  rg.write_tables(reinterpret_cast<char*>(s.h_crop.p));
  CK(cudaMemcpyAsync(d_tab, s.h_crop.p, tb, cudaMemcpyHostToDevice, st));
  const size_t rb = (rg.regs.size() * sizeof(RegionDev) + 255) / 256 * 256;
  CK(warp_regions_launch(reinterpret_cast<const RegionDev*>(d_tab), reinterpret_cast<const RegionTile*>(d_tab + rb),
                         int(rg.tiles.size()), d_tab + tb, st));
  if (to_host) CK(cudaMemcpyAsync(s.h_crop.p + tb, d_tab + tb, px, cudaMemcpyDeviceToHost, st));
  s.crop_px_off = tb;
  return CTD_OK;
}

static int host_stage(ctd_handle* h, PipeJob& job) {
  const int n = int(job.pages.size());
  if (!job.rows && job.textheight <= 0) return CTD_OK;
  const BlockSection bs = block_section_layout();
  std::vector<int> prc(size_t(n), CTD_OK), crc(size_t(n), CTD_OK);
  for_each_page(n, h->host_threads, [&](int i) {
    JobPage& p = job.pages[size_t(i)];
    if (job.rows) prc[size_t(i)] = host_group_page(page_in(job.results_host, job.head, i, p), bs, job.textheight > 0, p);
    if (job.textheight > 0 && prc[size_t(i)] == CTD_OK) {
      p.plan.resize(p.lines.size());
      if (!p.lines.empty())
        crc[size_t(i)] = ctd_region_plan(p.lines.data(), int32_t(p.lines.size()), p.iw, p.ih, job.textheight,
                                         p.plan.data(), &p.plan_bytes);
    }
  });
  for (int i = 0; i < n; ++i)
    if (prc[size_t(i)] != CTD_OK) return ctd_fail(h, prc[size_t(i)], "group_output failed on page %d of the batch", i);
  for (int i = 0; i < n; ++i)
    if (crc[size_t(i)] != CTD_OK)
      return ctd_fail(h, crc[size_t(i)], "ctd_region_plan refused page %d of the batch (%dx%d, textheight %d)", i,
                      job.pages[size_t(i)].ih, job.pages[size_t(i)].iw, job.textheight);
  return CTD_OK;
}

static int device_stage(ctd_handle* h, const PipeJob& job, cudaStream_t st, DevBuf& refine_scratch, DevBuf& cc,
                        char* pinned, size_t pinned_cap) {
  if (job.d_blocks)
    CK(cudaMemcpyAsync(job.d_blocks, job.pages[0].section, job.blocks_bytes, cudaMemcpyHostToDevice, st));
  if (job.textheight > 0)
    if (int rc = crop_stage(h, h->slot[job.slot], region_pages(job), job.pages, !job.results_on_device, st)) return rc;
  if (job.pl.ref && !job.refined_input) {
    CK(cudaMemsetAsync(job.pl.ref, 0, job.pl.total, st));
    RefineJob rj;
    for (const JobPage& p : job.pages)
      for (size_t k = 0; k + 3 < p.wins.size(); k += 4)
        rj.add(p.wins[k], p.wins[k + 1], p.wins[k + 2], p.wins[k + 3], p.off, p.iw, p.ih);
    char* stage = rj.table_bytes() <= pinned_cap ? pinned : nullptr;
    if (int rc = launch_refine(h, rj, job.pl.img, job.pl.mask, job.refine_mode, job.pl.ref, st, refine_scratch, stage))
      return rc;
  }
  if (!job.keep_undetected) return CTD_OK;
  return refine_undetected(h, job.pages, job.pl, job.refine_mode, st, cc, refine_scratch, pinned, pinned_cap);
}

static int run_job(ctd_handle* h, PipeJob& job) {
  Slot& s = h->slot[job.slot];
  if (job.rows) {
    CK(cudaEventSynchronize(s.ev_out_done));
    for (int i = 0; job.nonfinite && i < int(job.pages.size()); ++i)
      if (const int32_t f = job.nonfinite[i])
        return ctd_fail(h, CTD_E_INVALID, "page %d of the batch: a non-finite value (NaN or inf) in its %s", i,
                        (f & 1) ? "blks" : (f & 2) ? "mask" : "lines_map");
  }
  if (int rc = host_stage(h, job)) return rc;
  cudaStream_t st = h->post;
  CK(cudaStreamWaitEvent(st, s.ev_out_ready, 0));
  if (int rc = device_stage(h, job, st, h->post_refine, h->pg_cc, s.pinned, h->pipe_pinned_cap)) return rc;
  return finish_batch(h, job, st);
}

static void pipe_worker(ctd_handle* h) {
  cudaSetDevice(h->cfg.device);
  for (;;) {
    PipeJob job;
    {
      std::unique_lock<std::mutex> lk(h->pipe_mu);
      h->pipe_cv.wait(lk, [&] { return h->pipe_quit || !h->pipe_queue.empty(); });
      if (h->pipe_queue.empty()) return;
      job = std::move(h->pipe_queue.front());
      h->pipe_queue.pop_front();
    }
    const int rc = run_job(h, job);
    std::string err;
    if (rc != CTD_OK) err = h->err;
    {
      std::lock_guard<std::mutex> lk(h->pipe_mu);
      Slot& s = h->slot[job.slot];
      s.state = rc == CTD_OK ? 2 : 3;
      s.rc = rc;
      s.err = err;
    }
    h->pipe_done_cv.notify_all();
  }
}

static void queue_job(ctd_handle* h, PipeJob&& job) {
  Slot& s = h->slot[job.slot];
  {
    std::lock_guard<std::mutex> lk(h->pipe_mu);
    s.state = 1;
    h->pipe_queue.push_back(std::move(job));
  }
// ... 823 lines not shown
```

comic-text-detector_b200/csrc/postproc.cu:

```cuda
#include <cuda_fp16.h>
#include <cuda_runtime.h>
#include <limits.h>

#include "kernels.h"

namespace ctd {

constexpr int kCandStride = 8;
constexpr int kMaxDet = 300;
constexpr float kMaxWh = 4096.f;

size_t nms_workspace_bytes(int n, int cap) {
  return size_t(n) * cap * kCandStride * 4 * 2 + size_t(n) * 4 * 8 + size_t(n) * cap * (cap / 64) * 8;
}
void nms_workspace_bind(NmsWorkspace& ws, void* base, int n, int cap) {
  char* p = static_cast<char*>(base);
  ws.cap = cap;
  ws.mask = reinterpret_cast<unsigned long long*>(p);
  p += size_t(n) * cap * (cap / 64) * 8;
  ws.cand = reinterpret_cast<float*>(p);
  p += size_t(n) * cap * kCandStride * 4;
  ws.sorted = reinterpret_cast<float*>(p);
  p += size_t(n) * cap * kCandStride * 4;
  ws.cand_count = reinterpret_cast<int*>(p);
// ... 32 lines not shown
  } else {
    o[0] = x[0] - hw; o[1] = x[1] - hh; o[2] = x[0] + hw; o[3] = x[1] + hh;
  }
  o[4] = __uint_as_float(key); o[5] = float(cls); o[6] = __int_as_float(r); o[7] = 0.f;
}

__device__ __forceinline__ float page_conf(const int32_t* __restrict__ half, int img, float conf_thres, bool* hf) {
  *hf = half && half[img];
  return *hf ? round_half(conf_thres) : conf_thres;
}

__global__ void nms_filter_kernel(const float* __restrict__ blks, int rows, int no, float conf_thres,
                                  const int32_t* __restrict__ half, float* __restrict__ cand,
                                  int* __restrict__ cand_count, int cap) {
  const int img = blockIdx.y;
  const int r = blockIdx.x * blockDim.x + threadIdx.x;
  if (r >= rows) return;
  bool hf;
  const float conf = page_conf(half, img, conf_thres, &hf);
  const float* x = blks + (size_t(img) * rows + r) * no;
  int cls = 0;
  const unsigned key = nms_score_key(x, no, conf, hf, &cls);
  if (key == 0u) return;
  const int slot = atomicAdd(&cand_count[img], 1);
  if (slot >= cap) return;
  write_cand(cand + (size_t(img) * cap + slot) * kCandStride, x, hf, key, cls, r);
}

__global__ void __launch_bounds__(1024) nms_overflow_kernel(const float* __restrict__ blks, int rows, int no,
                                                            float conf_thres, const int32_t* __restrict__ half,
                                                            float* __restrict__ cand,
                                                            int* __restrict__ cand_count, int* __restrict__ cand_total,
                                                            int cap) {
  __shared__ int hist[2048];
  __shared__ unsigned s_prefix, s_maskbits;
  __shared__ int s_need, s_base_take, s_base_tie;
  __shared__ int wsum_take[32], wsum_tie[32];
  const int img = blockIdx.x, t = threadIdx.x, lane = t & 31, wid = t >> 5;
  const int total = cand_count[img];
  if (t == 0) cand_total[img] = total;
  if (total <= cap) return;
  bool hf;
  const float conf = page_conf(half, img, conf_thres, &hf);
  const float* pb = blks + size_t(img) * rows * no;
  if (t == 0) { s_prefix = 0u; s_maskbits = 0u; s_need = cap; }
  const int shifts[3] = {21, 10, 0}, nbins[3] = {2048, 2048, 1024};
#pragma unroll
  for (int lvl = 0; lvl < 3; ++lvl) {
    for (int i = t; i < 2048; i += 1024) hist[i] = 0;
    __syncthreads();
    const unsigned prefix = s_prefix, maskbits = s_maskbits;
    for (int r = t; r < rows; r += 1024) {
      int cls;
      const unsigned key = nms_score_key(pb + size_t(r) * no, no, conf, hf, &cls);
      if (key != 0u && (key & maskbits) == prefix) atomicAdd(&hist[(key >> shifts[lvl]) & unsigned(nbins[lvl] - 1)], 1);
    }
    __syncthreads();
    if (t == 0) {
      int need = s_need, cum = 0, digit = 0;
      for (int b = nbins[lvl] - 1; b >= 0; --b) {
        if (cum + hist[b] >= need) { digit = b; break; }
        cum += hist[b];
      }
      s_need = need - cum;
      s_prefix = prefix | (unsigned(digit) << shifts[lvl]);
      s_maskbits = maskbits | (unsigned(nbins[lvl] - 1) << shifts[lvl]);
    }
    __syncthreads();
  }
  const unsigned T = s_prefix;
  const int need_ties = s_need;
  if (t == 0) { s_base_take = 0; s_base_tie = 0; }
  __syncthreads();
  float* out = cand + size_t(img) * cap * kCandStride;
  for (int r0 = 0; r0 < rows; r0 += 1024) {
    const int r = r0 + t;
    int cls = 0;
    unsigned key = 0u;
    if (r < rows) key = nms_score_key(pb + size_t(r) * no, no, conf, hf, &cls);
    const bool tie = key == T && key != 0u;
    const unsigned tb = __ballot_sync(0xffffffffu, tie);
    if (lane == 0) wsum_tie[wid] = __popc(tb);
    __syncthreads();
    int tie_rank = s_base_tie + __popc(tb & ((1u << lane) - 1u));
    for (int w2 = 0; w2 < wid; ++w2) tie_rank += wsum_tie[w2];
    const bool take = key > T || (tie && tie_rank < need_ties);
    const unsigned kb = __ballot_sync(0xffffffffu, take);
    if (lane == 0) wsum_take[wid] = __popc(kb);
    __syncthreads();
    if (take) {
      int slot = s_base_take + __popc(kb & ((1u << lane) - 1u));
      for (int w2 = 0; w2 < wid; ++w2) slot += wsum_take[w2];
      if (slot < cap) write_cand(out + size_t(slot) * kCandStride, pb + size_t(r) * no, hf, key, cls, r);
    }
    __syncthreads();
    if (t == 0) {
      int a = 0, b = 0;
      for (int w2 = 0; w2 < 32; ++w2) { a += wsum_take[w2]; b += wsum_tie[w2]; }
      s_base_take += a;
      s_base_tie += b;
    }
    __syncthreads();
  }
  if (t == 0) cand_count[img] = cap;
}

template <int P>
__global__ void __launch_bounds__(1024) nms_sort_kernel(const float* __restrict__ cand, int* __restrict__ cand_count,
                                                        float* __restrict__ sorted, int cap) {
  __shared__ float skey[P];
  __shared__ int srow[P];
  __shared__ int sslot[P];
  const int img = blockIdx.x;
  int m = cand_count[img];
  if (m > cap) m = cap;
  const float* c = cand + size_t(img) * cap * kCandStride;
  for (int i = threadIdx.x; i < P; i += blockDim.x) {
    if (i < m) {
      skey[i] = c[i * kCandStride + 4];
      srow[i] = __float_as_int(c[i * kCandStride + 6]);
      sslot[i] = i;
    } else {
      skey[i] = -INFINITY;
      srow[i] = INT_MAX;
      sslot[i] = -1;
    }
  }
  __syncthreads();
  for (int k = 2; k <= P; k <<= 1) {
    for (int j = k >> 1; j > 0; j >>= 1) {
      for (int i = threadIdx.x; i < P; i += blockDim.x) {
        const int ixj = i ^ j;
        if (ixj > i) {
          const bool up = (i & k) == 0;
          const float ka = skey[i], kb = skey[ixj];
          const int ra = srow[i], rb = srow[ixj];
          const bool a_first = (ka > kb) || (ka == kb && ra < rb);
          if (a_first != up) {
            skey[i] = kb; skey[ixj] = ka;
            srow[i] = rb; srow[ixj] = ra;
            const int t = sslot[i]; sslot[i] = sslot[ixj]; sslot[ixj] = t;
          }
        }
      }
      __syncthreads();
    }
  }
  float* o = sorted + size_t(img) * cap * kCandStride;
  for (int i = threadIdx.x; i < m; i += blockDim.x) {
    const int sl = sslot[i];
#pragma unroll
    for (int e = 0; e < kCandStride; ++e) o[i * kCandStride + e] = c[sl * kCandStride + e];
  }
}

__global__ void __launch_bounds__(64) nms_mask_kernel(const float* __restrict__ sorted, const int* __restrict__ cand_count,
                                                      unsigned long long* __restrict__ mask, int cap, float iou_thres) {
  const int img = blockIdx.z;
  int m = cand_count[img];
  if (m > cap) m = cap;
  const int rb = blockIdx.y, cb = blockIdx.x;
  if (rb * 64 >= m || cb * 64 >= m || cb < rb) return;
  __shared__ float cbox[64][5];
  const float* s = sorted + size_t(img) * cap * kCandStride;
  const int cj = cb * 64 + threadIdx.x;
  if (cj < m) {
    const float off = s[cj * kCandStride + 5] * kMaxWh;
    cbox[threadIdx.x][0] = s[cj * kCandStride + 0] + off;
    cbox[threadIdx.x][1] = s[cj * kCandStride + 1] + off;
    cbox[threadIdx.x][2] = s[cj * kCandStride + 2] + off;
    cbox[threadIdx.x][3] = s[cj * kCandStride + 3] + off;
    cbox[threadIdx.x][4] = __fmul_rn(cbox[threadIdx.x][2] - cbox[threadIdx.x][0], cbox[threadIdx.x][3] - cbox[threadIdx.x][1]);
  }
  __syncthreads();
  const int i = rb * 64 + threadIdx.x;
  if (i >= m) return;
  const float off = s[i * kCandStride + 5] * kMaxWh;
  const float x1 = s[i * kCandStride + 0] + off, y1 = s[i * kCandStride + 1] + off;
  const float x2 = s[i * kCandStride + 2] + off, y2 = s[i * kCandStride + 3] + off;
  const float area = __fmul_rn(x2 - x1, y2 - y1);
  unsigned long long bits = 0;
  const int jmax = min(64, m - cb * 64);
  for (int j = 0; j < jmax; ++j) {
    if (cb * 64 + j <= i) continue;
    const float xx1 = fmaxf(x1, cbox[j][0]), yy1 = fmaxf(y1, cbox[j][1]);
    const float xx2 = fminf(x2, cbox[j][2]), yy2 = fminf(y2, cbox[j][3]);
    const float w = fmaxf(0.f, xx2 - xx1), h = fmaxf(0.f, yy2 - yy1);
    const float inter = __fmul_rn(w, h);
    const float ovr = __fdiv_rn(inter, __fsub_rn(__fadd_rn(area, cbox[j][4]), inter));
    if (ovr > iou_thres) bits |= 1ull << j;
  }
  mask[(size_t(img) * cap + i) * (cap / 64) + cb] = bits;
}

__global__ void __launch_bounds__(64) nms_scan_kernel(const float* __restrict__ sorted, const int* __restrict__ cand_count,
                                                      const unsigned long long* __restrict__ mask, int cap,
                                                      float* __restrict__ det, int* __restrict__ det_count) {
  __shared__ unsigned long long remv[64];
  __shared__ unsigned long long diag[64];
  __shared__ unsigned long long s_keepbits;
  __shared__ int s_kept;
  const int img = blockIdx.x, t = threadIdx.x;
  int m = cand_count[img];
  if (m > cap) m = cap;
  const int words = cap / 64;
  const int wlast = (m + 63) >> 6;
  remv[t] = 0ull;
  if (t == 0) s_kept = 0;
  __syncthreads();
  const unsigned long long* mbase = mask + size_t(img) * cap * words;
  const float* s = sorted + size_t(img) * cap * kCandStride;
  float* o = det + size_t(img) * kMaxDet * 6;
  for (int c = 0; c < wlast; ++c) {
    const int i = c * 64 + t;
    diag[t] = (i < m) ? mbase[size_t(i) * words + c] : 0ull;
    __syncthreads();
    if (t == 0) {
      unsigned long long rw = remv[c], keep = 0ull;
      int kept = s_kept;
      const int lim = min(64, m - c * 64);
      for (int j = 0; j < lim && kept < kMaxDet; ++j) {
        if ((rw >> j) & 1ull) continue;
        keep |= 1ull << j;
        rw |= diag[j];
        ++kept;
      }
      s_keepbits = keep;
    }
    __syncthreads();
    const unsigned long long keep = s_keepbits;
    const int base_kept = s_kept;
    if ((keep >> t) & 1ull) {
      const int pos = base_kept + __popcll(keep & ((1ull << t) - 1ull));
      const float* r = s + size_t(c * 64 + t) * kCandStride;
#pragma unroll
      for (int e = 0; e < 6; ++e) o[pos * 6 + e] = r[e];
    }
    if (t > c && t < wlast) {
      unsigned long long acc = remv[t], kb = keep;
      while (kb) {
        const int j = __ffsll((long long)kb) - 1;
        kb &= kb - 1;
        acc |= mbase[size_t(c * 64 + j) * words + t];
      }
      remv[t] = acc;
    }
    __syncthreads();
    if (t == 0) s_kept = base_kept + __popcll(keep);
    __syncthreads();
    if (s_kept >= kMaxDet) break;
  }
  if (t == 0) det_count[img] = s_kept;
}

cudaError_t nms_launch(const float* blks, int n, int rows, int nc, float conf, float iou, NmsWorkspace& ws, float* det,
                       int* det_count, cudaStream_t s, const int32_t* half) {
  cudaError_t e = cudaMemsetAsync(ws.cand_count, 0, sizeof(int) * n, s);
  if (e != cudaSuccess) return e;
  nms_filter_kernel<<<dim3((rows + 255) / 256, n), 256, 0, s>>>(blks, rows, 5 + nc, conf, half, ws.cand, ws.cand_count,
                                                                 ws.cap);
  nms_overflow_kernel<<<n, 1024, 0, s>>>(blks, rows, 5 + nc, conf, half, ws.cand, ws.cand_count, ws.cand_total, ws.cap);
  if (ws.cap == 4096) nms_sort_kernel<4096><<<n, 1024, 0, s>>>(ws.cand, ws.cand_count, ws.sorted, ws.cap);
  else if (ws.cap == 1024) nms_sort_kernel<1024><<<n, 1024, 0, s>>>(ws.cand, ws.cand_count, ws.sorted, ws.cap);
  else return cudaErrorInvalidValue;
  const int blocks = ws.cap / 64;
  nms_mask_kernel<<<dim3(blocks, blocks, n), 64, 0, s>>>(ws.sorted, ws.cand_count, ws.mask, ws.cap, iou);
  if (ws.cap > 4096) return cudaErrorInvalidValue;
  nms_scan_kernel<<<n, 64, 0, s>>>(ws.sorted, ws.cand_count, ws.mask, ws.cap, det, det_count);
  return cudaGetLastError();
}


__device__ __forceinline__ int uf_find(const int* L, int a) {
  int p = L[a];
  while (p != a) {
    a = p;
    p = L[a];
  }
  return a;
}
__device__ __forceinline__ void uf_union(int* L, int a, int b) {
  bool done;
  do {
    a = uf_find(L, a);
    b = uf_find(L, b);
    if (a < b) {
      const int old = atomicMin(&L[b], a);
      done = old == b;
      b = old;
    } else if (b < a) {
      const int old = atomicMin(&L[a], b);
      done = old == a;
      a = old;
    } else {
      done = true;
    }
  } while (!done);
}

constexpr int kCclTile = 32;
constexpr int kScanSeg = 2048;

__global__ void __launch_bounds__(1024) ccl_local_kernel(const uint8_t* __restrict__ img, int h, int w,
                                                         int* __restrict__ Lall, int* __restrict__ keymin_all) {
  __shared__ int s[kCclTile * kCclTile];
  const int page = blockIdx.z;
  const int lx = threadIdx.x & 31, ly = threadIdx.x >> 5;
  const int x = blockIdx.x * kCclTile + lx, y = blockIdx.y * kCclTile + ly;
  const bool inb = x < w && y < h;
  const size_t o = size_t(page) * h * w;
  const int l = threadIdx.x;
  const bool fg = inb && img[o + size_t(y) * w + x] != 0;
  const unsigned m = __ballot_sync(0xffffffffu, fg);
  const unsigned zeros_below = ~m & ((1u << lx) - 1u);
  const int start = zeros_below ? 32 - __clz(zeros_below) : 0;
  s[l] = fg ? (ly << 5) + start : -1;
  __syncthreads();
  if (fg && ly > 0) {
    const bool un = s[l - 32] >= 0;
    if (un) {
      const bool first = (lx == start) || s[l - 33] < 0;
      if (first) uf_union(s, l, l - 32);
    } else {
      if (lx > 0 && s[l - 33] >= 0) uf_union(s, l, l - 33);
      if (lx < 31 && s[l - 31] >= 0) uf_union(s, l, l - 31);
    }
  }
  __syncthreads();
  if (inb) {
    int g = -1;
    if (fg) {
      const int r = uf_find(s, l);
      g = (blockIdx.y * kCclTile + (r >> 5)) * w + blockIdx.x * kCclTile + (r & 31);
    }
    Lall[o + size_t(y) * w + x] = g;
    keymin_all[o + size_t(y) * w + x] = INT_MAX;
  }
}

__global__ void ccl_border_kernel(int h, int w, int* __restrict__ Lall) {
  const int page = blockIdx.y;
  int* L = Lall + size_t(page) * h * w;
  const int nvl = (w - 1) / kCclTile;
  const int nhl = (h - 1) / kCclTile;
  const int i = blockIdx.x * blockDim.x + threadIdx.x;
  if (i < nvl * h) {
    const int x = (i / h + 1) * kCclTile, y = i % h;
    const int p = y * w + x;
    if (L[p] < 0) return;
    if (L[p - 1] >= 0) uf_union(L, p, p - 1);
    if (y > 0 && L[p - w - 1] >= 0) uf_union(L, p, p - w - 1);
    if (y + 1 < h && L[p + w - 1] >= 0) uf_union(L, p, p + w - 1);
  } else if (i < nvl * h + nhl * w) {
    const int j = i - nvl * h;
    const int y = (j / w + 1) * kCclTile, x = j % w;
    const int p = y * w + x;
    if (L[p] < 0) return;
    if (L[p - w] >= 0) uf_union(L, p, p - w);
    if (x > 0 && L[p - w - 1] >= 0) uf_union(L, p, p - w - 1);
    if (x + 1 < w && L[p - w + 1] >= 0) uf_union(L, p, p - w + 1);
  }
}

__global__ void ccl_flatten_key_kernel(int h, int w, int* __restrict__ Lall, int* __restrict__ keymin_all) {
  const int page = blockIdx.y;
  const int p = blockIdx.x * blockDim.x + threadIdx.x;
  const int hw = h * w;
  if (p >= hw) return;
  int* L = Lall + size_t(page) * hw;
  if (L[p] < 0) return;
  const int r = uf_find(L, p);
  L[p] = r;
  const int y = p / w, x = p - y * w;
  if ((y >> 1) == ((r / w) >> 1)) atomicMin(&keymin_all[size_t(page) * hw + r], x >> 1);
}

__global__ void ccl_markfirst_kernel(int h, int w, const int* __restrict__ Lall, const int* __restrict__ keymin_all,
                                     int* __restrict__ bflag_all) {
  const int page = blockIdx.y;
  const int p = blockIdx.x * blockDim.x + threadIdx.x;
  const int hw = h * w;
  if (p >= hw) return;
  const size_t o = size_t(page) * hw;
  if (Lall[o + p] == p) {
    const int bw = (w + 1) / 2;
    bflag_all[o + ((p / w) >> 1) * bw + keymin_all[o + p]] = 1;
  }
}

__global__ void __launch_bounds__(256) ccl_scan_seg_kernel(int h, int w, int* __restrict__ bflag_all, int* __restrict__ segsum,
                                                           int nseg) {
  __shared__ int wsum[8];
  const int page = blockIdx.y, seg = blockIdx.x;
  const int nb = ((h + 1) / 2) * ((w + 1) / 2);
  int* f = bflag_all + size_t(page) * h * w + size_t(seg) * kScanSeg;
  const int base = seg * kScanSeg;
  const int lane = threadIdx.x & 31, warp = threadIdx.x >> 5;
  int v[8], t = 0;
  const int i0 = threadIdx.x * 8;
#pragma unroll
  for (int e = 0; e < 8; ++e) {
    v[e] = (base + i0 + e < nb) ? f[i0 + e] : 0;
    t += v[e];
  }
  int incl = t;
#pragma unroll
  for (int off = 1; off < 32; off <<= 1) {
    const int u = __shfl_up_sync(0xffffffffu, incl, off);
    if (lane >= off) incl += u;
  }
  if (lane == 31) wsum[warp] = incl;
  __syncthreads();
  int woff = 0;
  for (int k = 0; k < warp; ++k) woff += wsum[k];
  int run = woff + incl - t;
#pragma unroll
  for (int e = 0; e < 8; ++e) {
    if (base + i0 + e < nb) f[i0 + e] = run;
    run += v[e];
  }
  if (threadIdx.x == 255) segsum[page * nseg + seg] = woff + incl;
}
__global__ void __launch_bounds__(1024) ccl_scan_top_kernel(int* __restrict__ segsum, int nseg, int* __restrict__ n_labels) {
  __shared__ int part[1024];
  const int page = blockIdx.x;
  int* sgs = segsum + size_t(page) * nseg;
  int carry = 0;
  for (int c0 = 0; c0 < nseg; c0 += 4096) {
    int v[4], loc = 0;
#pragma unroll
    for (int k = 0; k < 4; ++k) {
      const int i = c0 + threadIdx.x * 4 + k;
      v[k] = i < nseg ? sgs[i] : 0;
      loc += v[k];
    }
    part[threadIdx.x] = loc;
    __syncthreads();
    for (int off = 1; off < 1024; off <<= 1) {
      int u = 0;
      if (threadIdx.x >= off) u = part[threadIdx.x - off];
      __syncthreads();
      part[threadIdx.x] += u;
      __syncthreads();
    }
    int run = carry + part[threadIdx.x] - loc;
#pragma unroll
    for (int k = 0; k < 4; ++k) {
      const int i = c0 + threadIdx.x * 4 + k;
      if (i < nseg) sgs[i] = run;
      run += v[k];
    }
    carry += part[1023];
    __syncthreads();
  }
  if (threadIdx.x == 0) n_labels[page] = carry + 1;
}

__global__ void ccl_relabel_kernel(int h, int w, const int* __restrict__ Lall, const int* __restrict__ keymin_all,
                                   const int* __restrict__ rank_all, const int* __restrict__ segoff, int nseg,
                                   int32_t* __restrict__ labels) {
  const int page = blockIdx.y;
  const int p = blockIdx.x * blockDim.x + threadIdx.x;
  const int hw = h * w;
  if (p >= hw) return;
  const size_t o = size_t(page) * hw;
  const int r = Lall[o + p];
  int lab = 0;
  if (r >= 0) {
    const int bw = (w + 1) / 2;
    const int key = ((r / w) >> 1) * bw + keymin_all[o + r];
    lab = segoff[page * nseg + key / kScanSeg] + rank_all[o + key] + 1;
  }
  labels[o + p] = lab;
}

cudaError_t ccl_launch(const uint8_t* img, int n, int h, int w, int32_t* labels, int32_t* scratch, int32_t* n_labels,
                       cudaStream_t s) {
  const int hw = h * w;
  int* L = scratch;
  int* keymin = scratch + size_t(n) * hw;
  int* bflag = scratch + size_t(2) * n * hw;
  const int nb = ((h + 1) / 2) * ((w + 1) / 2);
  const int nseg = (nb + kScanSeg - 1) / kScanSeg;
  int* segsum = bflag + size_t(n - 1) * hw + nb;
  if (size_t(n) * nseg > size_t(hw - nb)) return cudaErrorInvalidValue;
  cudaError_t e = cudaMemset2DAsync(bflag, size_t(hw) * sizeof(int), 0, size_t(nb) * sizeof(int), n, s);
  if (e != cudaSuccess) return e;
  dim3 tgrid((w + kCclTile - 1) / kCclTile, (h + kCclTile - 1) / kCclTile, n);
  ccl_local_kernel<<<tgrid, 1024, 0, s>>>(img, h, w, L, keymin);
  const int nborder = ((w - 1) / kCclTile) * h + ((h - 1) / kCclTile) * w;
  if (nborder > 0) ccl_border_kernel<<<dim3((nborder + 255) / 256, n), 256, 0, s>>>(h, w, L);
  dim3 grid((hw + 255) / 256, n);
  ccl_flatten_key_kernel<<<grid, 256, 0, s>>>(h, w, L, keymin);
  ccl_markfirst_kernel<<<grid, 256, 0, s>>>(h, w, L, keymin, bflag);
  ccl_scan_seg_kernel<<<dim3(nseg, n), 256, 0, s>>>(h, w, bflag, segsum, nseg);
  ccl_scan_top_kernel<<<n, 1024, 0, s>>>(segsum, nseg, n_labels);
  ccl_relabel_kernel<<<grid, 256, 0, s>>>(h, w, L, keymin, bflag, segsum, nseg, labels);
  return cudaGetLastError();
}

__global__ void ccl_stats_init_kernel(int32_t* stats, int cap) {
  const int i = blockIdx.x * blockDim.x + threadIdx.x;
  if (i >= cap) return;
  stats[i * 5 + 0] = INT_MAX;
  stats[i * 5 + 1] = INT_MAX;
  stats[i * 5 + 2] = -1;
  stats[i * 5 + 3] = -1;
  stats[i * 5 + 4] = 0;
}
__global__ void ccl_stats_acc_kernel(const int32_t* __restrict__ labels, int h, int w, int32_t* stats, int cap) {
  const int p = blockIdx.x * blockDim.x + threadIdx.x;
  if (p >= h * w) return;
  const int l = labels[p];
  if (l >= cap) return;
  const int y = p / w, x = p - y * w;
  atomicMin(&stats[l * 5 + 0], x);
  atomicMin(&stats[l * 5 + 1], y);
  atomicMax(&stats[l * 5 + 2], x);
  atomicMax(&stats[l * 5 + 3], y);
  atomicAdd(&stats[l * 5 + 4], 1);
}
__global__ void ccl_stats_fin_kernel(int32_t* stats, int cap) {
  const int i = blockIdx.x * blockDim.x + threadIdx.x;
  if (i >= cap) return;
  if (stats[i * 5 + 4] == 0) {
    stats[i * 5 + 2] = 0;
    stats[i * 5 + 3] = 0;
  } else {
    stats[i * 5 + 2] = stats[i * 5 + 2] - stats[i * 5 + 0] + 1;
    stats[i * 5 + 3] = stats[i * 5 + 3] - stats[i * 5 + 1] + 1;
  }
}
cudaError_t ccl_stats_launch(const int32_t* labels, int h, int w, int32_t* stats, int cap, cudaStream_t s) {
  ccl_stats_init_kernel<<<(cap + 255) / 256, 256, 0, s>>>(stats, cap);
  ccl_stats_acc_kernel<<<(h * w + 255) / 256, 256, 0, s>>>(labels, h, w, stats, cap);
  ccl_stats_fin_kernel<<<(cap + 255) / 256, 256, 0, s>>>(stats, cap);
  return cudaGetLastError();
}

}
```

comic-text-detector_b200/csrc/segrep.cu:

```cuda
#include <cuda_runtime.h>
#include <limits.h>

#include "geom.h"
#include "kernels.h"

namespace ctd {

using ctdgeom::IPt;

__device__ __forceinline__ int uf_find_g(const int* L, int a) {
  int p = L[a];
  while (p != a) {
    a = p;
    p = L[a];
  }
  return a;
}
__device__ __forceinline__ void uf_union_g(int* L, int a, int b) {
  bool done;
  do {
    a = uf_find_g(L, a);
    b = uf_find_g(L, b);
    if (a < b) {
      const int old = atomicMin(&L[b], a);
      done = old == b;
      b = old;
    } else if (b < a) {
      const int old = atomicMin(&L[a], b);
      done = old == a;
      a = old;
    } else {
      done = true;
    }
  } while (!done);
}

__global__ void __launch_bounds__(1024) bg_local_kernel(const uint8_t* __restrict__ img, int h, int w, int* __restrict__ Lall) {
  __shared__ int s[32 * 32];
  const int page = blockIdx.z;
  const int lx = threadIdx.x & 31, ly = threadIdx.x >> 5;
  const int x = blockIdx.x * 32 + lx, y = blockIdx.y * 32 + ly;
  const bool inb = x < w && y < h;
  const size_t o = size_t(page) * h * w;
  const int l = threadIdx.x;
  const bool bg = inb && img[o + size_t(y) * w + x] == 0;
  const unsigned m = __ballot_sync(0xffffffffu, bg);
  const unsigned zeros_below = ~m & ((1u << lx) - 1u);
  const int start = zeros_below ? 32 - __clz(zeros_below) : 0;
  s[l] = bg ? (ly << 5) + start : -1;
  __syncthreads();
  if (bg && ly > 0 && s[l - 32] >= 0) {
    const bool first = (lx == start) || s[l - 33] < 0;
    if (first) uf_union_g(s, l, l - 32);
  }
  __syncthreads();
  if (inb) {
    int g = -1;
    if (bg) {
      const int r = uf_find_g(s, l);
      g = (blockIdx.y * 32 + (r >> 5)) * w + blockIdx.x * 32 + (r & 31);
    }
    Lall[o + size_t(y) * w + x] = g;
  }
}
__global__ void bg_border_kernel(int h, int w, int* __restrict__ Lall) {
  const int page = blockIdx.y;
  int* L = Lall + size_t(page) * h * w;
  const int nvl = (w - 1) / 32, nhl = (h - 1) / 32;
  const int i = blockIdx.x * blockDim.x + threadIdx.x;
  if (i < nvl * h) {
    const int x = (i / h + 1) * 32, y = i % h;
    const int p = y * w + x;
    if (L[p] >= 0 && L[p - 1] >= 0) uf_union_g(L, p, p - 1);
  } else if (i < nvl * h + nhl * w) {
    const int j = i - nvl * h;
    const int y = (j / w + 1) * 32, x = j % w;
    const int p = y * w + x;
    if (L[p] >= 0 && L[p - w] >= 0) uf_union_g(L, p, p - w);
  }
}
__global__ void bg_flatten_kernel(int h, int w, int* __restrict__ Lall) {
  const int page = blockIdx.y;
  const int p = blockIdx.x * blockDim.x + threadIdx.x;
  if (p >= h * w) return;
  int* L = Lall + size_t(page) * h * w;
  if (L[p] < 0) return;
  L[p] = uf_find_g(L, p);
}

constexpr int kFrame = -2;

__global__ void mark_outside_kernel(int h, int w, const int* __restrict__ Lb_all, int* __restrict__ parent_all) {
  const int page = blockIdx.y;
  const int i = blockIdx.x * blockDim.x + threadIdx.x;
  const int per = 2 * w + 2 * h;
  if (i >= per) return;
  int x, y;
  if (i < w) { x = i; y = 0; }
  else if (i < 2 * w) { x = i - w; y = h - 1; }
  else if (i < 2 * w + h) { x = 0; y = i - 2 * w; }
  else { x = w - 1; y = i - 2 * w - h; }
  const size_t o = size_t(page) * h * w;
  const int r = Lb_all[o + size_t(y) * w + x];
  if (r >= 0) parent_all[o + r] = kFrame;
}

__global__ void roots_kernel(int h, int w, const int* __restrict__ Lf_all, const int* __restrict__ Lb_all,
                             int* __restrict__ parent_all, int* __restrict__ flag_all, double* __restrict__ own_sum,
                             int* __restrict__ own_cnt, double* __restrict__ tot_sum, int* __restrict__ tot_cnt,
                             double* __restrict__ ring_sum, int* __restrict__ ring_cnt) {
  const int page = blockIdx.y;
  const int p = blockIdx.x * blockDim.x + threadIdx.x;
  const int hw = h * w;
  if (p >= hw) return;
  const size_t o = size_t(page) * hw;
  const int lf = Lf_all[o + p], lb = Lb_all[o + p];
  int flag = 0;
  if (lf == p) {
    const int x = p % w;
    int par = kFrame;
    if (x > 0) {
      const int q = Lb_all[o + p - 1];
      par = (q >= 0 && parent_all[o + q] != kFrame) ? q : kFrame;
    }
    parent_all[o + p] = par;
    flag = 1;
  } else if (lb == p) {
    if (parent_all[o + p] != kFrame) {
      parent_all[o + p] = Lf_all[o + p - 1];
      flag = 1;
    }
  }
  if (lf == p || lb == p) {
    own_sum[o + p] = 0.0; own_cnt[o + p] = 0;
    tot_sum[o + p] = 0.0; tot_cnt[o + p] = 0;
    ring_sum[o + p] = 0.0; ring_cnt[o + p] = 0;
  }
  flag_all[o + p] = flag;
}

constexpr int kSeg = 2048;
__global__ void __launch_bounds__(256) flag_scan_seg_kernel(int hw, int* __restrict__ flag_all, int* __restrict__ segsum, int nseg) {
  __shared__ int wsum[8];
  const int page = blockIdx.y, seg = blockIdx.x;
  int* f = flag_all + size_t(page) * hw + size_t(seg) * kSeg;
  const int base = seg * kSeg;
  const int lane = threadIdx.x & 31, warp = threadIdx.x >> 5;
  int v[8], t = 0;
  const int i0 = threadIdx.x * 8;
#pragma unroll
  for (int e = 0; e < 8; ++e) {
    v[e] = (base + i0 + e < hw) ? f[i0 + e] : 0;
    t += v[e];
  }
  int incl = t;
#pragma unroll
  for (int off = 1; off < 32; off <<= 1) {
    const int u = __shfl_up_sync(0xffffffffu, incl, off);
    if (lane >= off) incl += u;
  }
  if (lane == 31) wsum[warp] = incl;
  __syncthreads();
  int woff = 0;
  for (int k = 0; k < warp; ++k) woff += wsum[k];
  int run = woff + incl - t;
#pragma unroll
  for (int e = 0; e < 8; ++e) {
    if (base + i0 + e < hw) f[i0 + e] = run | (v[e] << 30);
    run += v[e];
  }
  if (threadIdx.x == 255) segsum[page * nseg + seg] = woff + incl;
}
__global__ void __launch_bounds__(1024) flag_scan_top_kernel(int* __restrict__ segsum, int nseg, int* __restrict__ total) {
  __shared__ int part[1024];
  const int page = blockIdx.x;
  int* sgs = segsum + page * nseg;
  int v[4], loc = 0;
#pragma unroll
  for (int k = 0; k < 4; ++k) {
    const int i = threadIdx.x * 4 + k;
    v[k] = i < nseg ? sgs[i] : 0;
    loc += v[k];
  }
  part[threadIdx.x] = loc;
  __syncthreads();
  for (int off = 1; off < 1024; off <<= 1) {
    int u = 0;
    if (threadIdx.x >= off) u = part[threadIdx.x - off];
    __syncthreads();
    part[threadIdx.x] += u;
    __syncthreads();
  }
  int run = part[threadIdx.x] - loc;
#pragma unroll
  for (int k = 0; k < 4; ++k) {
    const int i = threadIdx.x * 4 + k;
    if (i < nseg) sgs[i] = run;
    run += v[k];
  }
  if (threadIdx.x == 1023) total[page] = part[1023];
}
__global__ void assign_cid_kernel(int h, int w, const int* __restrict__ Lf_all, int* __restrict__ flag_all,
                                  const int* __restrict__ segoff, int nseg, const int* __restrict__ total, int max_cand,
                                  int* __restrict__ c_root, int* __restrict__ rowmin, int* __restrict__ rowmax) {
  const int page = blockIdx.y;
  const int p = blockIdx.x * blockDim.x + threadIdx.x;
  const int hw = h * w;
  if (p >= hw) return;
  const size_t o = size_t(page) * hw;
  const int f = flag_all[o + p];
  int cid = -1;
  if (f & (1 << 30)) {
    const int rank = segoff[page * nseg + p / kSeg] + (f & ((1 << 30) - 1));
    const int c = total[page] - 1 - rank;
    if (c < max_cand) {
      cid = c;
      c_root[page * max_cand + c] = (Lf_all[o + p] == p) ? p : (p | int(0x80000000u));
    }
  }
  flag_all[o + p] = cid;
  (void)rowmin; (void)rowmax;
}
__global__ void rows_init_kernel(int* __restrict__ rowmin, int* __restrict__ rowmax, size_t n, int* __restrict__ c_yrange,
                                 size_t ncont) {
  const size_t i = blockIdx.x * size_t(blockDim.x) + threadIdx.x;
  if (i < n) {
    rowmin[i] = INT_MAX;
    rowmax[i] = -1;
  }
  if (i < ncont) {
    c_yrange[2 * i] = INT_MAX;
    c_yrange[2 * i + 1] = -1;
  }
}

__global__ void accumulate_kernel(int h, int w, const float* __restrict__ pred_all, size_t pred_page_stride,
                                  const int* __restrict__ Lf_all, const int* __restrict__ Lb_all,
                                  const int* __restrict__ parent_all, const int* __restrict__ cid_all,
                                  double* __restrict__ own_sum, int* __restrict__ own_cnt, double* __restrict__ ring_sum,
                                  int* __restrict__ ring_cnt, int* __restrict__ rowmin, int* __restrict__ rowmax,
                                  int* __restrict__ c_yrange, int max_cand) {
  const int page = blockIdx.y;
  const int p = blockIdx.x * blockDim.x + threadIdx.x;
  const int hw = h * w;
  const bool live = p < hw;
  const size_t o = size_t(page) * hw;
  const int lane = threadIdx.x & 31;
  float v = 0.f;
  int y = 0, x = 0, lf = -1, key = -1;
  if (live) {
    v = pred_all[size_t(page) * pred_page_stride + p];
    y = p / w;
    x = p - y * w;
    lf = Lf_all[o + p];
    if (lf >= 0) key = lf;
    else {
      const int lb = Lb_all[o + p];
      if (parent_all[o + lb] != kFrame) key = lb;
    }
  }
  const unsigned long long k64 = (unsigned long long)(unsigned)key | ((unsigned long long)(unsigned)y << 32);
  const unsigned peers = __match_any_sync(0xffffffffu, k64);
  const int leader = __ffs(peers) - 1;
  double s = 0.0;
  int c = 0;
  if (__all_sync(0xffffffffu, peers == 0xffffffffu)) {
    s = (double)v;
#pragma unroll
    for (int off = 16; off > 0; off >>= 1) s += __shfl_down_sync(0xffffffffu, s, off);
    c = 32;
  } else {
#pragma unroll 4
    for (int l = 0; l < 32; ++l) {
      const float ov = __shfl_sync(0xffffffffu, v, l);
      if ((peers >> l) & 1u) {
        s += (double)ov;
        ++c;
      }
    }
  }
  if (live && key >= 0 && lane == leader) {
    atomicAdd(&own_sum[o + key], s);
    atomicAdd(&own_cnt[o + key], c);
    if (lf >= 0) {
      const int cid = cid_all[o + lf];
      if (cid >= 0) {
        const int last = 31 - __clz(peers);
        const size_t ro = (size_t(page) * max_cand + cid) * h + y;
        atomicMin(&rowmin[ro], x);
        atomicMax(&rowmax[ro], x + (last - lane));
        atomicMin(&c_yrange[(page * max_cand + cid) * 2], y);
        atomicMax(&c_yrange[(page * max_cand + cid) * 2 + 1], y);
      }
    }
  }
  if (live && lf >= 0) {
    int hs[4];
    int nh = 0;
    const int nb[4] = {x > 0 ? p - 1 : -1, x + 1 < w ? p + 1 : -1, y > 0 ? p - w : -1, y + 1 < h ? p + w : -1};
#pragma unroll
    for (int k = 0; k < 4; ++k) {
      if (nb[k] < 0) continue;
      const int q = Lb_all[o + nb[k]];
      if (q < 0 || parent_all[o + q] != lf) continue;
      bool dup = false;
      for (int e = 0; e < nh; ++e) dup |= hs[e] == q;
      if (!dup) hs[nh++] = q;
    }
    for (int e = 0; e < nh; ++e) {
      const int q = hs[e];
      atomicAdd(&ring_sum[o + q], (double)v);
      atomicAdd(&ring_cnt[o + q], 1);
      const int c2 = cid_all[o + q];
      if (c2 >= 0) {
        const size_t ro = (size_t(page) * max_cand + c2) * h + y;
        atomicMin(&rowmin[ro], x);
        atomicMax(&rowmax[ro], x);
        atomicMin(&c_yrange[(page * max_cand + c2) * 2], y);
        atomicMax(&c_yrange[(page * max_cand + c2) * 2 + 1], y);
      }
    }
  }
}

__global__ void tree_kernel(int h, int w, const int* __restrict__ Lf_all, const int* __restrict__ Lb_all,
                            const int* __restrict__ parent_all, const double* __restrict__ own_sum,
                            const int* __restrict__ own_cnt, double* __restrict__ tot_sum, int* __restrict__ tot_cnt) {
  const int page = blockIdx.y;
  const int p = blockIdx.x * blockDim.x + threadIdx.x;
  const int hw = h * w;
  if (p >= hw) return;
  const size_t o = size_t(page) * hw;
  const bool root = Lf_all[o + p] == p || (Lb_all[o + p] == p && parent_all[o + p] != kFrame);
  if (!root) return;
  const double s = own_sum[o + p];
  const int c = own_cnt[o + p];
  int a = p;
  int guard = 0;
  while (a >= 0 && guard++ < 4096) {
    atomicAdd(&tot_sum[o + a], s);
    atomicAdd(&tot_cnt[o + a], c);
    a = parent_all[o + a];
  }
}

template <int CAP>
struct ContourScratchT {
  IPt hull[CAP];
  IPt tmp[CAP];
  IPt off[CAP];
  float f0[CAP], f1[CAP], f2[CAP];
};
struct ContourScratch;

__device__ __forceinline__ void hull_start_maxx_warp(IPt* hull, int n, IPt* tmp, int lane) {
  if (n < 3) return;
  int bx = INT_MIN, by = INT_MIN, bi = 0;
  for (int i = lane; i < n; i += 32) {
    const IPt q = hull[i];
    if (q.x > bx || (q.x == bx && q.y > by)) { bx = q.x; by = q.y; bi = i; }
  }
#pragma unroll
  for (int off = 16; off > 0; off >>= 1) {
    const int ox = __shfl_xor_sync(0xffffffffu, bx, off), oy = __shfl_xor_sync(0xffffffffu, by, off);
    const int oi = __shfl_xor_sync(0xffffffffu, bi, off);
    if (ox > bx || (ox == bx && oy > by)) { bx = ox; by = oy; bi = oi; }
  }
  if (bi == 0) return;
  for (int i = lane; i < n; i += 32) { int j = i + bi; if (j >= n) j -= n; tmp[i] = hull[j]; }
  __syncwarp();
  for (int i = lane; i < n; i += 32) hull[i] = tmp[i];
  __syncwarp();
}

__device__ __forceinline__ ctdgeom::MarExt mar_prepass_warp(const IPt* hull, int n, float* vx, float* vy, float* inv, int lane) {
  float lx = 3.402823466e+38f, rx = -3.402823466e+38f, ty = -3.402823466e+38f, by = 3.402823466e+38f;
  int li = 0x7fffffff, ri = 0x7fffffff, ti = 0x7fffffff, bi = 0x7fffffff;
  for (int i = lane; i < n; i += 32) {
    const float px = (float)hull[i].x, py = (float)hull[i].y;
    if (px < lx) { lx = px; li = i; }
    if (px > rx) { rx = px; ri = i; }
    if (py > ty) { ty = py; ti = i; }
    if (py < by) { by = py; bi = i; }
    ctdgeom::mar_edge(hull, n, i, vx, vy, inv);
  }
#pragma unroll
  for (int off = 16; off > 0; off >>= 1) {
    float o; int oi;
    o = __shfl_xor_sync(0xffffffffu, lx, off); oi = __shfl_xor_sync(0xffffffffu, li, off);
    if (o < lx || (o == lx && oi < li)) { lx = o; li = oi; }
    o = __shfl_xor_sync(0xffffffffu, rx, off); oi = __shfl_xor_sync(0xffffffffu, ri, off);
    if (o > rx || (o == rx && oi < ri)) { rx = o; ri = oi; }
    o = __shfl_xor_sync(0xffffffffu, ty, off); oi = __shfl_xor_sync(0xffffffffu, ti, off);
    if (o > ty || (o == ty && oi < ti)) { ty = o; ti = oi; }
    o = __shfl_xor_sync(0xffffffffu, by, off); oi = __shfl_xor_sync(0xffffffffu, bi, off);
    if (o < by || (o == by && oi < bi)) { by = o; bi = oi; }
  }
  __syncwarp();
  return ctdgeom::MarExt{li, bi, ri, ti};
}

__global__ void __launch_bounds__(1024) contour_order_kernel(int max_cand, const int* __restrict__ total,
                                                             const int* __restrict__ c_yrange, int* __restrict__ perm) {
  __shared__ unsigned int key[1024];
  const int page = blockIdx.x, i = threadIdx.x;
  int ncont = total[page];
  if (ncont > max_cand) ncont = max_cand;
  unsigned int k = 0xffffffffu;
  if (i < max_cand) {
    int rows = 0;
    if (i < ncont) {
      const int y0 = c_yrange[(page * max_cand + i) * 2], y1 = c_yrange[(page * max_cand + i) * 2 + 1];
      rows = y1 >= y0 ? y1 - y0 + 1 : 0;
      if (rows > 0xfffff) rows = 0xfffff;
    }
    k = ((0xfffffu - (unsigned int)rows) << 12) | (unsigned int)i;
  }
  key[i] = k;
  __syncthreads();
  for (int size = 2; size <= 1024; size <<= 1)
    for (int stride = size >> 1; stride > 0; stride >>= 1) {
      const int j = i ^ stride;
      if (j > i) {
        const unsigned int a = key[i], b = key[j];
        const bool up = (i & size) == 0;
        if ((a > b) == up) { key[i] = b; key[j] = a; }
      }
      __syncthreads();
    }
  if (i < max_cand) perm[page * max_cand + i] = int(key[i] & 0xfffu);
}

constexpr int kContourWarps = 4;
template <int CAP>
__global__ void __launch_bounds__(32 * kContourWarps) contour_kernel(int h, int w, int max_cand, const int* __restrict__ total,
                                                     const int* __restrict__ c_root, const int* __restrict__ rowmin,
                                                     const int* __restrict__ rowmax, const int* __restrict__ c_yrange,
                                                     const double* __restrict__ tot_sum,
                                                     const int* __restrict__ tot_cnt, const double* __restrict__ ring_sum,
                                                     const int* __restrict__ ring_cnt, ContourScratch* __restrict__ scratch,
                                                     int16_t* __restrict__ boxes, float* __restrict__ scores,
                                                     int* __restrict__ n_out, int dst_w, int dst_h, float unclip_ratio,
                                                     const int* __restrict__ perm, int n_pages,
                                                     int* __restrict__ ovf_count, int* __restrict__ ovf_list, int second) {
  extern __shared__ __align__(16) unsigned char csm[];
  ContourScratchT<CAP>& S = reinterpret_cast<ContourScratchT<CAP>*>(csm)[threadIdx.x >> 5];
  (void)scratch;
  const int page = int(blockIdx.x) % n_pages;
  const int slot = (int(blockIdx.x) / n_pages) * kContourWarps + (threadIdx.x >> 5);
  const int lane = threadIdx.x & 31;
  int ncont = total[page];
  if (ncont > max_cand) ncont = max_cand;
  if (!second && slot == 0 && lane == 0) n_out[page] = ncont;
  if (slot >= max_cand) return;
  int c;
  if (second) {
    if (slot >= ovf_count[page]) return;
    c = ovf_list[page * max_cand + slot];
  } else {
    c = perm[page * max_cand + slot];
  }
  auto defer = [&]() {
    if (!second && lane == 0) ovf_list[page * max_cand + atomicAdd(&ovf_count[page], 1)] = c;
  };
  int16_t* bo = boxes + (size_t(page) * max_cand + c) * 8;
  float* so = scores + size_t(page) * max_cand + c;
  if (lane < 8) bo[lane] = 0;
  if (lane == 0) *so = 0.f;
  if (c >= ncont) return;
  const int entry = c_root[page * max_cand + c];
  const bool is_hole = entry < 0;
  const int root = entry & 0x7fffffff;
  const size_t o = size_t(page) * h * w;
  const int* rmin = rowmin + (size_t(page) * max_cand + c) * h;
  const int* rmax = rowmax + (size_t(page) * max_cand + c) * h;
  const int y_lo = max(0, c_yrange[(page * max_cand + c) * 2]), y_hi = min(h - 1, c_yrange[(page * max_cand + c) * 2 + 1]);
  int* rbuf = reinterpret_cast<int*>(S.f0);
  int k = 0;
  bool overflow = false;
  for (int y0 = y_lo; y0 <= y_hi; y0 += 64) {
    for (int e = lane; e < 64; e += 32) {
      const int y = y0 + e;
      rbuf[e] = y <= y_hi ? rmin[y] : INT_MAX;
      rbuf[64 + e] = y <= y_hi ? rmax[y] : -1;
    }
    __syncwarp();
    if (lane == 0 && !overflow) {
      for (int e = 0; e < 64 && y0 + e <= y_hi && !overflow; ++e) {
        const int a = rbuf[e], b = rbuf[64 + e];
        if (b < 0) continue;
        for (int q = 0; q < (a == b ? 1 : 2); ++q) {
          const IPt pt{y0 + e, q == 0 ? a : b};
          while (k >= 2 && ctdgeom::cross3(S.hull[k - 2], S.hull[k - 1], pt) <= 0) --k;
          if (k >= CAP) { overflow = true; break; }
          S.hull[k++] = pt;
        }
      }
    }
    __syncwarp();
  }
  const int lower = k + 1;
  bool first = true;
  for (int y1 = y_hi; y1 >= y_lo; y1 -= 64) {
    for (int e = lane; e < 64; e += 32) {
      const int y = y1 - e;
      rbuf[e] = y >= y_lo ? rmin[y] : INT_MAX;
      rbuf[64 + e] = y >= y_lo ? rmax[y] : -1;
    }
    __syncwarp();
    if (lane == 0 && !overflow) {
      for (int e = 0; e < 64 && y1 - e >= y_lo && !overflow; ++e) {
        const int a = rbuf[e], b = rbuf[64 + e];
        if (b < 0) continue;
        for (int q = 0; q < (a == b ? 1 : 2); ++q) {
          const IPt pt{y1 - e, q == 0 ? b : a};
          if (first) { first = false; continue; }
          while (k >= lower && ctdgeom::cross3(S.hull[k - 2], S.hull[k - 1], pt) <= 0) --k;
          if (k >= CAP) { overflow = true; break; }
          S.hull[k++] = pt;
        }
      }
    }
    __syncwarp();
  }
  overflow = __shfl_sync(0xffffffffu, int(overflow), 0) != 0;
  k = __shfl_sync(0xffffffffu, k, 0);
  if (overflow) { defer(); return; }
  if (k > 1) --k;
  for (int i = lane; i < k; i += 32) S.tmp[i] = IPt{S.hull[k - 1 - i].y, S.hull[k - 1 - i].x};
  __syncwarp();
  for (int i = lane; i < k; i += 32) S.hull[i] = S.tmp[i];
  __syncwarp();
  if (k < 3) return;
  hull_start_maxx_warp(S.hull, k, S.tmp, lane);
  const ctdgeom::MarExt e1 = mar_prepass_warp(S.hull, k, S.f0, S.f1, S.f2, lane);
  int m = 0;
  __syncwarp();
  if (lane == 0) {
    const ctdgeom::RRect r1 = ctdgeom::mar_core(S.hull, k, S.f0, S.f1, S.f2, e1);
    const float sside = r1.w < r1.h ? r1.w : r1.h;
    if (sside >= 2.f) {
      float px[4], py[4], ox[4], oy[4];
      ctdgeom::box_points(r1, px, py);
      ctdgeom::order_mini_box(px, py, ox, oy);
      m = ctdgeom::unclip_offset(ox, oy, (double)unclip_ratio, S.off, CAP);
      if (m >= 0 && m < 3) m = 0;
    }
  }
  m = __shfl_sync(0xffffffffu, m, 0);
  __syncwarp();
  if (m < 0) { defer(); return; }
  if (m == 0) return;
  for (int i = lane; i < m; i += 32) {
    const IPt p = S.off[i];
    int rank = 0;
    for (int j = 0; j < m; ++j) {
      const IPt q = S.off[j];
      rank += (q.x < p.x) || (q.x == p.x && (q.y < p.y || (q.y == p.y && j < i)));
    }
    S.tmp[rank] = p;
  }
  __syncwarp();
  for (int i = lane; i < m; i += 32) S.off[i] = S.tmp[i];
  __syncwarp();
  int nh2 = 0;
  if (lane == 0) nh2 = ctdgeom::hull_sorted(S.off, m, S.hull, CAP);
  nh2 = __shfl_sync(0xffffffffu, nh2, 0);
  __syncwarp();
  if (nh2 < 0) { defer(); return; }
  if (nh2 < 3) return;
  hull_start_maxx_warp(S.hull, nh2, S.tmp, lane);
  const ctdgeom::MarExt e2 = mar_prepass_warp(S.hull, nh2, S.f0, S.f1, S.f2, lane);
  if (lane != 0) return;
  const ctdgeom::RRect r2 = ctdgeom::mar_core(S.hull, nh2, S.f0, S.f1, S.f2, e2);
  float px[4], py[4], ox[4], oy[4];
  ctdgeom::box_points(r2, px, py);
  ctdgeom::order_mini_box(px, py, ox, oy);
  int16_t box[8];
  for (int q = 0; q < 4; ++q) {
    box[2 * q] = ctdgeom::quantise(ox[q], w, dst_w);
    box[2 * q + 1] = ctdgeom::quantise(oy[q], h, dst_h);
  }
  double sum = tot_sum[o + root];
  long long cnt = tot_cnt[o + root];
  if (is_hole) {
    sum += ring_sum[o + root];
    cnt += ring_cnt[o + root];
  }
  *so = cnt > 0 ? (float)D_MUL(sum, D_DIV(1.0, (double)cnt)) : 0.f;
#pragma unroll
  for (int e = 0; e < 8; ++e) bo[e] = box[e];
}

__global__ void binarize_kernel(const float* __restrict__ pred, size_t count, float thresh, uint8_t* __restrict__ bitmap) {
  const size_t i = blockIdx.x * size_t(blockDim.x) + threadIdx.x;
  if (i < count) bitmap[i] = pred[i] > thresh ? 1 : 0;
}
cudaError_t binarize_launch(const float* pred, size_t count, float thresh, uint8_t* bitmap, cudaStream_t s) {
  binarize_kernel<<<unsigned((count + 255) / 256), 256, 0, s>>>(pred, count, thresh, bitmap);
  return cudaGetLastError();
}

size_t segrep_scratch_bytes(int n, int h, int w, int max_cand) {
  const size_t hw = size_t(n) * h * w;
  return hw * 4 * 4
         + hw * 4 * 2
         + hw * 8 * 3
         + size_t(n) * max_cand * h * 4 * 2
         + size_t(n) * max_cand * 20
         + size_t(n) * 8192 * 4
         + 65536;
}

cudaError_t segrep_launch(const uint8_t* bitmap, const float* pred, size_t pred_page_stride, const int* Lf, int n, int h,
                          int w, int max_cand, float unclip_ratio, void* scratch, int16_t* boxes, float* scores,
                          int* n_contours, cudaStream_t s) {
  const size_t hw = size_t(h) * w, nhw = size_t(n) * hw;
  char* p = static_cast<char*>(scratch);
  auto take = [&](size_t bytes) { char* r = p; p += (bytes + 255) / 256 * 256; return r; };
  int* Lb = reinterpret_cast<int*>(take(nhw * 4));
  int* parent = reinterpret_cast<int*>(take(nhw * 4));
  int* flag = reinterpret_cast<int*>(take(nhw * 4));
  int* own_cnt = reinterpret_cast<int*>(take(nhw * 4));
  int* tot_cnt = reinterpret_cast<int*>(take(nhw * 4));
  int* ring_cnt = reinterpret_cast<int*>(take(nhw * 4));
  double* own_sum = reinterpret_cast<double*>(take(nhw * 8));
  double* tot_sum = reinterpret_cast<double*>(take(nhw * 8));
  double* ring_sum = reinterpret_cast<double*>(take(nhw * 8));
  int* rowmin = reinterpret_cast<int*>(take(size_t(n) * max_cand * h * 4));
  int* rowmax = reinterpret_cast<int*>(take(size_t(n) * max_cand * h * 4));
  int* c_root = reinterpret_cast<int*>(take(size_t(n) * max_cand * 4));
  int* c_yrange = reinterpret_cast<int*>(take(size_t(n) * max_cand * 8));
  int* perm = reinterpret_cast<int*>(take(size_t(n) * max_cand * 4));
  int* segsum = reinterpret_cast<int*>(take(size_t(n) * 4096 * 4));
  int* total = reinterpret_cast<int*>(take(size_t(n) * 4));
  int* ovf_count = reinterpret_cast<int*>(take(size_t(n) * 4));
  int* ovf_list = reinterpret_cast<int*>(take(size_t(n) * max_cand * 4));
  ContourScratch* cs = nullptr;
  const int nseg = int((hw + kSeg - 1) / kSeg);
  if (nseg > 4096) return cudaErrorInvalidValue;

  dim3 tgrid((w + 31) / 32, (h + 31) / 32, n);
  dim3 grid(unsigned((hw + 255) / 256), n);
  cudaError_t e = cudaMemsetAsync(parent, 0xff, nhw * 4, s);
  if (e != cudaSuccess) return e;
  bg_local_kernel<<<tgrid, 1024, 0, s>>>(bitmap, h, w, Lb);
  const int nborder = ((w - 1) / 32) * h + ((h - 1) / 32) * w;
  if (nborder > 0) bg_border_kernel<<<dim3((nborder + 255) / 256, n), 256, 0, s>>>(h, w, Lb);
  bg_flatten_kernel<<<grid, 256, 0, s>>>(h, w, Lb);
  mark_outside_kernel<<<dim3((2 * w + 2 * h + 255) / 256, n), 256, 0, s>>>(h, w, Lb, parent);
  roots_kernel<<<grid, 256, 0, s>>>(h, w, Lf, Lb, parent, flag, own_sum, own_cnt, tot_sum, tot_cnt, ring_sum, ring_cnt);
  flag_scan_seg_kernel<<<dim3(nseg, n), 256, 0, s>>>(int(hw), flag, segsum, nseg);
  flag_scan_top_kernel<<<n, 1024, 0, s>>>(segsum, nseg, total);
  {
    const size_t nr = size_t(n) * max_cand * h;
    rows_init_kernel<<<unsigned((nr + 255) / 256), 256, 0, s>>>(rowmin, rowmax, nr, c_yrange, size_t(n) * max_cand);
  }
  assign_cid_kernel<<<grid, 256, 0, s>>>(h, w, Lf, flag, segsum, nseg, total, max_cand, c_root, rowmin, rowmax);
  accumulate_kernel<<<grid, 256, 0, s>>>(h, w, pred, pred_page_stride, Lf, Lb, parent, flag, own_sum, own_cnt, ring_sum,
                                         ring_cnt, rowmin, rowmax, c_yrange, max_cand);
  tree_kernel<<<grid, 256, 0, s>>>(h, w, Lf, Lb, parent, own_sum, own_cnt, tot_sum, tot_cnt);
  constexpr int kCapSmall = 128, kCapLarge = ctdgeom::kMaxHull;
  const size_t sm_small = sizeof(ContourScratchT<kCapSmall>) * kContourWarps, sm_large = sizeof(ContourScratchT<kCapLarge>) * kContourWarps;
  cudaFuncSetAttribute(contour_kernel<kCapLarge>, cudaFuncAttributeMaxDynamicSharedMemorySize, int(sm_large));
  if (max_cand > 1024) return cudaErrorInvalidValue;
  contour_order_kernel<<<n, 1024, 0, s>>>(max_cand, total, c_yrange, perm);
  e = cudaMemsetAsync(ovf_count, 0, size_t(n) * 4, s);
  if (e != cudaSuccess) return e;
  const unsigned cgrid = unsigned((max_cand + kContourWarps - 1) / kContourWarps) * unsigned(n);
  contour_kernel<kCapSmall><<<cgrid, 32 * kContourWarps, sm_small, s>>>(
      h, w, max_cand, total, c_root, rowmin, rowmax, c_yrange, tot_sum, tot_cnt, ring_sum, ring_cnt, cs, boxes, scores,
      n_contours, w, h, unclip_ratio, perm, n, ovf_count, ovf_list, 0);
  contour_kernel<kCapLarge><<<cgrid, 32 * kContourWarps, sm_large, s>>>(
      h, w, max_cand, total, c_root, rowmin, rowmax, c_yrange, tot_sum, tot_cnt, ring_sum, ring_cnt, cs, boxes, scores,
      n_contours, w, h, unclip_ratio, perm, n, ovf_count, ovf_list, 1);
  return cudaGetLastError();
}

}
```

Before: 1155.

## Defer CCL relabeling and slim segment-representation kernel chain

The main post-processing path's connected-components pass now only does local union, border merge and flatten, counting roots with warp ballots, while the sequential relabeling (keymin, markfirst, scan, relabel) moves into a separate ccl_number_launch that runs only when labels are requested. Segrep fuses flag computation and segment scanning into roots_kernel, drops the full-image parent memset by setting parents during flatten, and replaces rowmin/rowmax with a persistent interleaved int2 rows buffer. That buffer is cleared sparsely after each use, so the dense per-candidate rows_init pass is gone. Tree processing iterates only over a compacted root list. The aim is fewer launches and less full-image memory traffic, at the cost of more state carried across calls (the rows buffer must stay cleared) and extra complexity.

Measured after the change: 1190, median of 6. 1.03x the previous value.

```diff
diff --git a/comic-text-detector_b200/csrc/engine.cu b/comic-text-detector_b200/csrc/engine.cu
--- a/comic-text-detector_b200/csrc/engine.cu
+++ b/comic-text-detector_b200/csrc/engine.cu
@@ -59,7 +59,7 @@
   cudaFree(h->d_wsplit);
   cudaFree(h->d_blob); cudaFree(h->d_pages); cudaFree(h->d_blks); cudaFree(h->d_mask); cudaFree(h->d_mask_u8);
   cudaFree(h->d_lines); cudaFree(h->d_bitmap); cudaFree(h->d_labels);
-  cudaFree(h->d_ccl_scratch); cudaFree(h->d_nms_ws); cudaFree(h->d_segrep_scratch);
+  cudaFree(h->d_ccl_scratch); cudaFree(h->d_nms_ws); cudaFree(h->d_segrep_scratch); cudaFree(h->d_segrep_rows);
   h->refine_scratch.release(); h->cc_scratch.release(); h->io_scratch.release(); h->in_stage.release();
   if (h->ev0) cudaEventDestroy(h->ev0);
   if (h->ev1) cudaEventDestroy(h->ev1);
@@ -245,6 +245,11 @@
   }
   CKC(cudaMalloc(&h->d_ccl_scratch, px * 4 * 3));
   CKC(cudaMalloc(&h->d_segrep_scratch, segrep_scratch_bytes(int(nb), int(mh), int(mw), 1000)));
+  {
+    const size_t rows_bytes = std::max(nb * mh, size_t(2048)) * 1000 * sizeof(int2);
+    CKC(cudaMalloc(&h->d_segrep_rows, rows_bytes));
+    CKC(cudaMemset(h->d_segrep_rows, 0xff, rows_bytes));
+  }
   const int cap = 4096;
   CKC(cudaMalloc(&h->d_nms_ws, nms_workspace_bytes(int(nb), cap)));
   nms_workspace_bind(h->nms, h->d_nms_ws, int(nb), cap);
@@ -444,9 +449,9 @@
 }
 
 int launch_db_post(ctd_handle* h, int n, int ph, int pw, cudaStream_t s, int* cnt) {
-  CK(ccl_launch(h->d_bitmap, n, ph, pw, h->d_labels, h->d_ccl_scratch, h->d_nlabels, s));
+  CK(ccl_launch(h->d_bitmap, n, ph, pw, h->d_ccl_scratch, h->d_nlabels, s));
   CK(segrep_launch(h->d_bitmap, h->d_lines, size_t(2) * ph * pw, h->d_ccl_scratch, n, ph, pw, 1000, 1.5f,
-                   h->d_segrep_scratch, h->d_line_boxes, h->d_line_scores, h->d_line_count, s));
+                   h->d_segrep_scratch, h->d_segrep_rows, h->d_line_boxes, h->d_line_scores, h->d_line_count, s));
   *cnt += kCclLaunches + kSegrepLaunches;
   return CTD_OK;
 }
@@ -730,7 +735,10 @@
   NEED_FWD();
   const size_t px = size_t(h->n) * h->ph * h->pw;
   if (bitmap) CK(cudaMemcpyAsync(bitmap, h->d_bitmap, px, cudaMemcpyDeviceToHost, h->stream));
-  if (labels) CK(cudaMemcpyAsync(labels, h->d_labels, px * 4, cudaMemcpyDeviceToHost, h->stream));
+  if (labels) {
+    CK(ccl_number_launch(h->n, h->ph, h->pw, h->d_ccl_scratch, h->d_labels, h->stream));
+    CK(cudaMemcpyAsync(labels, h->d_labels, px * 4, cudaMemcpyDeviceToHost, h->stream));
+  }
   if (n_labels) CK(cudaMemcpyAsync(n_labels, h->d_nlabels, size_t(h->n) * 4, cudaMemcpyDeviceToHost, h->stream));
   CK(cudaStreamSynchronize(h->stream));
   return CTD_OK;
@@ -755,9 +763,9 @@
   const size_t px = size_t(ih) * iw;
   CK(cudaMemcpyAsync(h->d_lines, pred, px * 4, cudaMemcpyHostToDevice, h->stream));
   CK(binarize_launch(h->d_lines, px, thresh, h->d_bitmap, h->stream));
-  CK(ccl_launch(h->d_bitmap, 1, ih, iw, h->d_labels, h->d_ccl_scratch, h->d_nlabels, h->stream));
+  CK(ccl_launch(h->d_bitmap, 1, ih, iw, h->d_ccl_scratch, h->d_nlabels, h->stream));
   CK(segrep_launch(h->d_bitmap, h->d_lines, px, h->d_ccl_scratch, 1, ih, iw, 1000, 1.5f, h->d_segrep_scratch,
-                   h->d_line_boxes, h->d_line_scores, h->d_line_count, h->stream));
+                   h->d_segrep_rows, h->d_line_boxes, h->d_line_scores, h->d_line_count, h->stream));
   CK(cudaMemcpyAsync(boxes, h->d_line_boxes, 1000 * 8 * 2, cudaMemcpyDeviceToHost, h->stream));
   CK(cudaMemcpyAsync(scores, h->d_line_scores, 1000 * 4, cudaMemcpyDeviceToHost, h->stream));
   CK(cudaMemcpyAsync(count, h->d_line_count, 4, cudaMemcpyDeviceToHost, h->stream));
@@ -920,7 +928,8 @@
   int32_t* d_labels = reinterpret_cast<int32_t*>(base);
   int32_t* d_scr = reinterpret_cast<int32_t*>(base + o_scr);
   int32_t* d_nl = reinterpret_cast<int32_t*>(base + o_nl);
-  CK(ccl_launch(d_img, 1, ih, iw, d_labels, d_scr, d_nl, h->stream));
+  CK(ccl_launch(d_img, 1, ih, iw, d_scr, d_nl, h->stream));
+  CK(ccl_number_launch(1, ih, iw, d_scr, d_labels, h->stream));
   if (stats_cap > 0) CK(ccl_stats_launch(d_labels, ih, iw, d_scr, stats_cap, h->stream));
   CK(cudaMemcpyAsync(n_labels, d_nl, 4, cudaMemcpyDeviceToHost, h->stream));
   CK(cudaStreamSynchronize(h->stream));
diff --git a/comic-text-detector_b200/csrc/engine.h b/comic-text-detector_b200/csrc/engine.h
--- a/comic-text-detector_b200/csrc/engine.h
+++ b/comic-text-detector_b200/csrc/engine.h
@@ -196,6 +196,7 @@
   int32_t* d_nlabels = nullptr;
   int32_t* d_ccl_scratch = nullptr;
   void* d_segrep_scratch = nullptr;
+  int2* d_segrep_rows = nullptr;
   DevBuf refine_scratch;
   DevBuf cc_scratch;
   DevBuf io_scratch;
diff --git a/comic-text-detector_b200/csrc/kernels.h b/comic-text-detector_b200/csrc/kernels.h
--- a/comic-text-detector_b200/csrc/kernels.h
+++ b/comic-text-detector_b200/csrc/kernels.h
@@ -154,17 +154,18 @@
 size_t nms_workspace_bytes(int n, int cap);
 void nms_workspace_bind(NmsWorkspace& ws, void* base, int n, int cap);
 
-cudaError_t ccl_launch(const uint8_t* img, int n, int h, int w, int32_t* labels, int32_t* scratch ,
-                       int32_t* n_labels, cudaStream_t s);
-constexpr int kCclLaunches = 8;
+cudaError_t ccl_launch(const uint8_t* img, int n, int h, int w, int32_t* scratch , int32_t* n_labels,
+                       cudaStream_t s);
+constexpr int kCclLaunches = 3;
+cudaError_t ccl_number_launch(int n, int h, int w, int32_t* scratch, int32_t* labels, cudaStream_t s);
 constexpr size_t kCclMaxPixels = size_t(1) << 28;
 cudaError_t ccl_stats_launch(const int32_t* labels, int h, int w, int32_t* stats, int cap, cudaStream_t s);
 
 size_t segrep_scratch_bytes(int n, int h, int w, int max_cand);
 cudaError_t segrep_launch(const uint8_t* bitmap, const float* pred, size_t pred_page_stride, const int* Lf, int n, int h,
-                          int w, int max_cand, float unclip_ratio, void* scratch, int16_t* boxes, float* scores,
-                          int* n_contours, cudaStream_t s);
-constexpr int kSegrepLaunches = 15;
+                          int w, int max_cand, float unclip_ratio, void* scratch, int2* rows, int16_t* boxes,
+                          float* scores, int* n_contours, cudaStream_t s);
+constexpr int kSegrepLaunches = 14;
 cudaError_t binarize_launch(const float* pred, size_t count, float thresh, uint8_t* bitmap, cudaStream_t s);
 
 cudaError_t resize_linear_u8_launch(const uint8_t* src, int sh, int sw, size_t src_pitch, int channels, uint8_t* dst,
diff --git a/comic-text-detector_b200/csrc/pipeline.cu b/comic-text-detector_b200/csrc/pipeline.cu
--- a/comic-text-detector_b200/csrc/pipeline.cu
+++ b/comic-text-detector_b200/csrc/pipeline.cu
@@ -252,7 +252,8 @@
   for (int i = 0; i < n; ++i) {
     const JobPage& p = pages[size_t(i)];
     int32_t* d_stats = reinterpret_cast<int32_t*>(base + stats_off[size_t(i)]);
-    CK(ccl_launch(pl.thr + p.off, 1, p.ih, p.iw, d_labels, d_scr, d_nl + i, st));
+    CK(ccl_launch(pl.thr + p.off, 1, p.ih, p.iw, d_scr, d_nl + i, st));
+    CK(ccl_number_launch(1, p.ih, p.iw, d_scr, d_labels, st));
     CK(ccl_stats_launch(d_labels, p.ih, p.iw, d_stats, cap[size_t(i)], st));
   }
   std::vector<int32_t> n_lab(static_cast<size_t>(n));
diff --git a/comic-text-detector_b200/csrc/postproc.cu b/comic-text-detector_b200/csrc/postproc.cu
--- a/comic-text-detector_b200/csrc/postproc.cu
+++ b/comic-text-detector_b200/csrc/postproc.cu
@@ -358,7 +358,7 @@
 constexpr int kScanSeg = 2048;
 
 __global__ void __launch_bounds__(1024) ccl_local_kernel(const uint8_t* __restrict__ img, int h, int w,
-                                                         int* __restrict__ Lall, int* __restrict__ keymin_all) {
+                                                         int* __restrict__ Lall, int32_t* __restrict__ n_labels) {
   __shared__ int s[kCclTile * kCclTile];
   const int page = blockIdx.z;
   const int lx = threadIdx.x & 31, ly = threadIdx.x >> 5;
@@ -366,6 +366,7 @@
   const bool inb = x < w && y < h;
   const size_t o = size_t(page) * h * w;
   const int l = threadIdx.x;
+  if (blockIdx.x == 0 && blockIdx.y == 0 && l == 0) n_labels[page] = 1;
   const bool fg = inb && img[o + size_t(y) * w + x] != 0;
   const unsigned m = __ballot_sync(0xffffffffu, fg);
   const unsigned zeros_below = ~m & ((1u << lx) - 1u);
@@ -390,7 +391,6 @@
       g = (blockIdx.y * kCclTile + (r >> 5)) * w + blockIdx.x * kCclTile + (r & 31);
     }
     Lall[o + size_t(y) * w + x] = g;
-    keymin_all[o + size_t(y) * w + x] = INT_MAX;
   }
 }
 
@@ -418,15 +418,28 @@
   }
 }
 
-__global__ void ccl_flatten_key_kernel(int h, int w, int* __restrict__ Lall, int* __restrict__ keymin_all) {
+__global__ void ccl_flatten_kernel(int h, int w, int* __restrict__ Lall, int32_t* __restrict__ n_labels) {
+  const int page = blockIdx.y;
+  const int p = blockIdx.x * blockDim.x + threadIdx.x;
+  const int hw = h * w;
+  int* L = Lall + size_t(page) * hw;
+  bool root = false;
+  if (p < hw && L[p] >= 0) {
+    const int r = uf_find(L, p);
+    L[p] = r;
+    root = r == p;
+  }
+  const unsigned roots = __ballot_sync(0xffffffffu, root);
+  if (roots && (threadIdx.x & 31) == 0) atomicAdd(&n_labels[page], __popc(roots));
+}
+
+__global__ void ccl_key_kernel(int h, int w, const int* __restrict__ Lall, int* __restrict__ keymin_all) {
   const int page = blockIdx.y;
   const int p = blockIdx.x * blockDim.x + threadIdx.x;
   const int hw = h * w;
   if (p >= hw) return;
-  int* L = Lall + size_t(page) * hw;
-  if (L[p] < 0) return;
-  const int r = uf_find(L, p);
-  L[p] = r;
+  const int r = Lall[size_t(page) * hw + p];
+  if (r < 0) return;
   const int y = p / w, x = p - y * w;
   if ((y >> 1) == ((r / w) >> 1)) atomicMin(&keymin_all[size_t(page) * hw + r], x >> 1);
 }
@@ -477,7 +490,7 @@
   }
   if (threadIdx.x == 255) segsum[page * nseg + seg] = woff + incl;
 }
-__global__ void __launch_bounds__(1024) ccl_scan_top_kernel(int* __restrict__ segsum, int nseg, int* __restrict__ n_labels) {
+__global__ void __launch_bounds__(1024) ccl_scan_top_kernel(int* __restrict__ segsum, int nseg) {
   __shared__ int part[1024];
   const int page = blockIdx.x;
   int* sgs = segsum + size_t(page) * nseg;
@@ -509,7 +522,6 @@
     carry += part[1023];
     __syncthreads();
   }
-  if (threadIdx.x == 0) n_labels[page] = carry + 1;
 }
 
 __global__ void ccl_relabel_kernel(int h, int w, const int* __restrict__ Lall, const int* __restrict__ keymin_all,
@@ -530,8 +542,18 @@
   labels[o + p] = lab;
 }
 
-cudaError_t ccl_launch(const uint8_t* img, int n, int h, int w, int32_t* labels, int32_t* scratch, int32_t* n_labels,
-                       cudaStream_t s) {
+cudaError_t ccl_launch(const uint8_t* img, int n, int h, int w, int32_t* scratch, int32_t* n_labels, cudaStream_t s) {
+  const int hw = h * w;
+  int* L = scratch;
+  dim3 tgrid((w + kCclTile - 1) / kCclTile, (h + kCclTile - 1) / kCclTile, n);
+  ccl_local_kernel<<<tgrid, 1024, 0, s>>>(img, h, w, L, n_labels);
+  const int nborder = ((w - 1) / kCclTile) * h + ((h - 1) / kCclTile) * w;
+  if (nborder > 0) ccl_border_kernel<<<dim3((nborder + 255) / 256, n), 256, 0, s>>>(h, w, L);
+  ccl_flatten_kernel<<<dim3((hw + 255) / 256, n), 256, 0, s>>>(h, w, L, n_labels);
+  return cudaGetLastError();
+}
+
+cudaError_t ccl_number_launch(int n, int h, int w, int32_t* scratch, int32_t* labels, cudaStream_t s) {
   const int hw = h * w;
   int* L = scratch;
   int* keymin = scratch + size_t(n) * hw;
@@ -540,17 +562,15 @@
   const int nseg = (nb + kScanSeg - 1) / kScanSeg;
   int* segsum = bflag + size_t(n - 1) * hw + nb;
   if (size_t(n) * nseg > size_t(hw - nb)) return cudaErrorInvalidValue;
-  cudaError_t e = cudaMemset2DAsync(bflag, size_t(hw) * sizeof(int), 0, size_t(nb) * sizeof(int), n, s);
+  cudaError_t e = cudaMemsetAsync(keymin, 0x7f, size_t(n) * hw * sizeof(int), s);
   if (e != cudaSuccess) return e;
-  dim3 tgrid((w + kCclTile - 1) / kCclTile, (h + kCclTile - 1) / kCclTile, n);
-  ccl_local_kernel<<<tgrid, 1024, 0, s>>>(img, h, w, L, keymin);
-  const int nborder = ((w - 1) / kCclTile) * h + ((h - 1) / kCclTile) * w;
-  if (nborder > 0) ccl_border_kernel<<<dim3((nborder + 255) / 256, n), 256, 0, s>>>(h, w, L);
+  e = cudaMemset2DAsync(bflag, size_t(hw) * sizeof(int), 0, size_t(nb) * sizeof(int), n, s);
+  if (e != cudaSuccess) return e;
   dim3 grid((hw + 255) / 256, n);
-  ccl_flatten_key_kernel<<<grid, 256, 0, s>>>(h, w, L, keymin);
+  ccl_key_kernel<<<grid, 256, 0, s>>>(h, w, L, keymin);
   ccl_markfirst_kernel<<<grid, 256, 0, s>>>(h, w, L, keymin, bflag);
   ccl_scan_seg_kernel<<<dim3(nseg, n), 256, 0, s>>>(h, w, bflag, segsum, nseg);
-  ccl_scan_top_kernel<<<n, 1024, 0, s>>>(segsum, nseg, n_labels);
+  ccl_scan_top_kernel<<<n, 1024, 0, s>>>(segsum, nseg);
   ccl_relabel_kernel<<<grid, 256, 0, s>>>(h, w, L, keymin, bflag, segsum, nseg, labels);
   return cudaGetLastError();
 }
diff --git a/comic-text-detector_b200/csrc/segrep.cu b/comic-text-detector_b200/csrc/segrep.cu
--- a/comic-text-detector_b200/csrc/segrep.cu
+++ b/comic-text-detector_b200/csrc/segrep.cu
@@ -79,20 +79,27 @@
     if (L[p] >= 0 && L[p - w] >= 0) uf_union_g(L, p, p - w);
   }
 }
-__global__ void bg_flatten_kernel(int h, int w, int* __restrict__ Lall) {
+__global__ void bg_flatten_kernel(int h, int w, int* __restrict__ Lall, int* __restrict__ parent_all) {
   const int page = blockIdx.y;
   const int p = blockIdx.x * blockDim.x + threadIdx.x;
   if (p >= h * w) return;
   int* L = Lall + size_t(page) * h * w;
   if (L[p] < 0) return;
-  L[p] = uf_find_g(L, p);
+  const int r = uf_find_g(L, p);
+  L[p] = r;
+  if (r == p) parent_all[size_t(page) * h * w + p] = -1;
 }
 
 constexpr int kFrame = -2;
 
-__global__ void mark_outside_kernel(int h, int w, const int* __restrict__ Lb_all, int* __restrict__ parent_all) {
+__global__ void mark_outside_kernel(int h, int w, const int* __restrict__ Lb_all, int* __restrict__ parent_all,
+                                    int* __restrict__ c_yrange, int max_cand) {
   const int page = blockIdx.y;
   const int i = blockIdx.x * blockDim.x + threadIdx.x;
+  if (i < max_cand) {
+    c_yrange[(page * max_cand + i) * 2] = INT_MAX;
+    c_yrange[(page * max_cand + i) * 2 + 1] = -1;
+  }
   const int per = 2 * w + 2 * h;
   if (i >= per) return;
   int x, y;
@@ -105,72 +112,70 @@
   if (r >= 0) parent_all[o + r] = kFrame;
 }
 
-__global__ void roots_kernel(int h, int w, const int* __restrict__ Lf_all, const int* __restrict__ Lb_all,
-                             int* __restrict__ parent_all, int* __restrict__ flag_all, double* __restrict__ own_sum,
-                             int* __restrict__ own_cnt, double* __restrict__ tot_sum, int* __restrict__ tot_cnt,
-                             double* __restrict__ ring_sum, int* __restrict__ ring_cnt) {
-  const int page = blockIdx.y;
-  const int p = blockIdx.x * blockDim.x + threadIdx.x;
-  const int hw = h * w;
-  if (p >= hw) return;
-  const size_t o = size_t(page) * hw;
-  const int lf = Lf_all[o + p], lb = Lb_all[o + p];
-  int flag = 0;
-  if (lf == p) {
-    const int x = p % w;
-    int par = kFrame;
-    if (x > 0) {
-      const int q = Lb_all[o + p - 1];
-      par = (q >= 0 && parent_all[o + q] != kFrame) ? q : kFrame;
-    }
-    parent_all[o + p] = par;
-    flag = 1;
-  } else if (lb == p) {
-    if (parent_all[o + p] != kFrame) {
-      parent_all[o + p] = Lf_all[o + p - 1];
-      flag = 1;
-    }
-  }
-  if (lf == p || lb == p) {
-    own_sum[o + p] = 0.0; own_cnt[o + p] = 0;
-    tot_sum[o + p] = 0.0; tot_cnt[o + p] = 0;
-    ring_sum[o + p] = 0.0; ring_cnt[o + p] = 0;
-  }
-  flag_all[o + p] = flag;
-}
-
 constexpr int kSeg = 2048;
-__global__ void __launch_bounds__(256) flag_scan_seg_kernel(int hw, int* __restrict__ flag_all, int* __restrict__ segsum, int nseg) {
+
+__device__ __forceinline__ int cta_flag_prefix(bool flag, int* excl, int* wsum) {
+  const int lane = threadIdx.x & 31, warp = threadIdx.x >> 5;
+  const unsigned b = __ballot_sync(0xffffffffu, flag);
+  __syncthreads();
+  if (lane == 0) wsum[warp] = __popc(b);
+  __syncthreads();
+  int off = 0, tot = 0;
+#pragma unroll
+  for (int k = 0; k < 8; ++k) {
+    off += k < warp ? wsum[k] : 0;
+    tot += wsum[k];
+  }
+  *excl = off + __popc(b & ((1u << lane) - 1u));
+  return tot;
+}
+
+__global__ void __launch_bounds__(256) roots_kernel(int h, int w, const int* __restrict__ Lf_all, const int* __restrict__ Lb_all,
+                                                    int* __restrict__ parent_all, double* __restrict__ own_sum,
+                                                    int* __restrict__ own_cnt, double* __restrict__ tot_sum,
+                                                    int* __restrict__ tot_cnt, double* __restrict__ ring_sum,
+                                                    int* __restrict__ ring_cnt, int* __restrict__ segsum, int nseg) {
   __shared__ int wsum[8];
   const int page = blockIdx.y, seg = blockIdx.x;
-  int* f = flag_all + size_t(page) * hw + size_t(seg) * kSeg;
-  const int base = seg * kSeg;
-  const int lane = threadIdx.x & 31, warp = threadIdx.x >> 5;
-  int v[8], t = 0;
-  const int i0 = threadIdx.x * 8;
-#pragma unroll
-  for (int e = 0; e < 8; ++e) {
-    v[e] = (base + i0 + e < hw) ? f[i0 + e] : 0;
-    t += v[e];
-  }
-  int incl = t;
-#pragma unroll
-  for (int off = 1; off < 32; off <<= 1) {
-    const int u = __shfl_up_sync(0xffffffffu, incl, off);
-    if (lane >= off) incl += u;
-  }
-  if (lane == 31) wsum[warp] = incl;
+  const int hw = h * w;
+  const size_t o = size_t(page) * hw;
+  int cnt = 0;
+  for (int e = 0; e < kSeg / 256; ++e) {
+    const int p = seg * kSeg + e * 256 + threadIdx.x;
+    if (p >= hw) break;
+    const int lf = Lf_all[o + p], lb = Lb_all[o + p];
+    if (lf == p) {
+      const int x = p % w;
+      int par = kFrame;
+      if (x > 0) {
+        const int q = Lb_all[o + p - 1];
+        par = (q >= 0 && parent_all[o + q] != kFrame) ? q : kFrame;
+      }
+      parent_all[o + p] = par;
+      ++cnt;
+    } else if (lb == p) {
+      if (parent_all[o + p] != kFrame) {
+        parent_all[o + p] = Lf_all[o + p - 1];
+        ++cnt;
+      }
+    }
+    if (lf == p || lb == p) {
+      own_sum[o + p] = 0.0; own_cnt[o + p] = 0;
+      tot_sum[o + p] = 0.0; tot_cnt[o + p] = 0;
+      ring_sum[o + p] = 0.0; ring_cnt[o + p] = 0;
+    }
+  }
+#pragma unroll
+  for (int off = 16; off > 0; off >>= 1) cnt += __shfl_xor_sync(0xffffffffu, cnt, off);
+  if ((threadIdx.x & 31) == 0) wsum[threadIdx.x >> 5] = cnt;
   __syncthreads();
-  int woff = 0;
-  for (int k = 0; k < warp; ++k) woff += wsum[k];
-  int run = woff + incl - t;
-#pragma unroll
-  for (int e = 0; e < 8; ++e) {
-    if (base + i0 + e < hw) f[i0 + e] = run | (v[e] << 30);
-    run += v[e];
-  }
-  if (threadIdx.x == 255) segsum[page * nseg + seg] = woff + incl;
-}
+  if (threadIdx.x == 0) {
+    int t = 0;
+    for (int k = 0; k < 8; ++k) t += wsum[k];
+    segsum[page * nseg + seg] = t;
+  }
+}
+
 __global__ void __launch_bounds__(1024) flag_scan_top_kernel(int* __restrict__ segsum, int nseg, int* __restrict__ total) {
   __shared__ int part[1024];
   const int page = blockIdx.x;
@@ -200,46 +205,55 @@
   }
   if (threadIdx.x == 1023) total[page] = part[1023];
 }
-__global__ void assign_cid_kernel(int h, int w, const int* __restrict__ Lf_all, int* __restrict__ flag_all,
-                                  const int* __restrict__ segoff, int nseg, const int* __restrict__ total, int max_cand,
-                                  int* __restrict__ c_root, int* __restrict__ rowmin, int* __restrict__ rowmax) {
-  const int page = blockIdx.y;
-  const int p = blockIdx.x * blockDim.x + threadIdx.x;
+__global__ void __launch_bounds__(256) assign_cid_kernel(int h, int w, const int* __restrict__ Lf_all,
+                                                         const int* __restrict__ Lb_all, const int* __restrict__ parent_all,
+                                                         const int* __restrict__ segoff, int nseg, const int* __restrict__ total,
+                                                         int max_cand, int* __restrict__ cid_all, int* __restrict__ c_root,
+                                                         int* __restrict__ root_list) {
+  __shared__ int wsum[8];
+  const int page = blockIdx.y, seg = blockIdx.x;
   const int hw = h * w;
-  if (p >= hw) return;
   const size_t o = size_t(page) * hw;
-  const int f = flag_all[o + p];
-  int cid = -1;
-  if (f & (1 << 30)) {
-    const int rank = segoff[page * nseg + p / kSeg] + (f & ((1 << 30) - 1));
-    const int c = total[page] - 1 - rank;
-    if (c < max_cand) {
-      cid = c;
-      c_root[page * max_cand + c] = (Lf_all[o + p] == p) ? p : (p | int(0x80000000u));
-    }
-  }
-  flag_all[o + p] = cid;
-  (void)rowmin; (void)rowmax;
-}
-__global__ void rows_init_kernel(int* __restrict__ rowmin, int* __restrict__ rowmax, size_t n, int* __restrict__ c_yrange,
-                                 size_t ncont) {
-  const size_t i = blockIdx.x * size_t(blockDim.x) + threadIdx.x;
-  if (i < n) {
-    rowmin[i] = INT_MAX;
-    rowmax[i] = -1;
-  }
-  if (i < ncont) {
-    c_yrange[2 * i] = INT_MAX;
-    c_yrange[2 * i + 1] = -1;
-  }
+  int base = segoff[page * nseg + seg];
+  for (int e = 0; e < kSeg / 256; ++e) {
+    const int p = seg * kSeg + e * 256 + threadIdx.x;
+    if (seg * kSeg + e * 256 >= hw) break;
+    bool fg_root = false, flag = false;
+    if (p < hw) {
+      fg_root = Lf_all[o + p] == p;
+      flag = fg_root || (Lb_all[o + p] == p && parent_all[o + p] != kFrame);
+    }
+    int excl;
+    const int tot = cta_flag_prefix(flag, &excl, wsum);
+    if (flag) {
+      const int rank = base + excl;
+      root_list[o + rank] = p;
+      const int c = total[page] - 1 - rank;
+      int cid = -1;
+      if (c < max_cand) {
+        cid = c;
+        c_root[page * max_cand + c] = fg_root ? p : (p | int(0x80000000u));
+      }
+      cid_all[o + p] = cid;
+    }
+    base += tot;
+  }
+}
+__global__ void rows_clear_kernel(int h, int max_cand, const int* __restrict__ total, const int* __restrict__ c_yrange,
+                                  int2* __restrict__ rows) {
+  const int page = blockIdx.y, c = blockIdx.x;
+  if (c >= total[page]) return;
+  const int y0 = c_yrange[(page * max_cand + c) * 2], y1 = c_yrange[(page * max_cand + c) * 2 + 1];
+  int2* r = rows + (size_t(page) * max_cand + c) * h;
+  for (int y = y0 + int(threadIdx.x); y <= y1; y += blockDim.x) r[y] = make_int2(-1, -1);
 }
 
 __global__ void accumulate_kernel(int h, int w, const float* __restrict__ pred_all, size_t pred_page_stride,
                                   const int* __restrict__ Lf_all, const int* __restrict__ Lb_all,
                                   const int* __restrict__ parent_all, const int* __restrict__ cid_all,
                                   double* __restrict__ own_sum, int* __restrict__ own_cnt, double* __restrict__ ring_sum,
-                                  int* __restrict__ ring_cnt, int* __restrict__ rowmin, int* __restrict__ rowmax,
-                                  int* __restrict__ c_yrange, int max_cand) {
+                                  int* __restrict__ ring_cnt, int2* __restrict__ rows, int* __restrict__ c_yrange,
+                                  int max_cand) {
   const int page = blockIdx.y;
   const int p = blockIdx.x * blockDim.x + threadIdx.x;
   const int hw = h * w;
@@ -287,8 +301,8 @@
       if (cid >= 0) {
         const int last = 31 - __clz(peers);
         const size_t ro = (size_t(page) * max_cand + cid) * h + y;
-        atomicMin(&rowmin[ro], x);
-        atomicMax(&rowmax[ro], x + (last - lane));
+        atomicMin(reinterpret_cast<unsigned*>(&rows[ro].x), unsigned(x));
+        atomicMax(&rows[ro].y, x + (last - lane));
         atomicMin(&c_yrange[(page * max_cand + cid) * 2], y);
         atomicMax(&c_yrange[(page * max_cand + cid) * 2 + 1], y);
       }
@@ -314,8 +328,8 @@
       const int c2 = cid_all[o + q];
       if (c2 >= 0) {
         const size_t ro = (size_t(page) * max_cand + c2) * h + y;
-        atomicMin(&rowmin[ro], x);
-        atomicMax(&rowmax[ro], x);
+        atomicMin(reinterpret_cast<unsigned*>(&rows[ro].x), unsigned(x));
+        atomicMax(&rows[ro].y, x);
         atomicMin(&c_yrange[(page * max_cand + c2) * 2], y);
         atomicMax(&c_yrange[(page * max_cand + c2) * 2 + 1], y);
       }
@@ -323,16 +337,14 @@
   }
 }
 
-__global__ void tree_kernel(int h, int w, const int* __restrict__ Lf_all, const int* __restrict__ Lb_all,
+__global__ void tree_kernel(int h, int w, const int* __restrict__ root_list, const int* __restrict__ total,
                             const int* __restrict__ parent_all, const double* __restrict__ own_sum,
                             const int* __restrict__ own_cnt, double* __restrict__ tot_sum, int* __restrict__ tot_cnt) {
   const int page = blockIdx.y;
-  const int p = blockIdx.x * blockDim.x + threadIdx.x;
-  const int hw = h * w;
-  if (p >= hw) return;
-  const size_t o = size_t(page) * hw;
-  const bool root = Lf_all[o + p] == p || (Lb_all[o + p] == p && parent_all[o + p] != kFrame);
-  if (!root) return;
+  const int i = blockIdx.x * blockDim.x + threadIdx.x;
+  if (i >= total[page]) return;
+  const size_t o = size_t(page) * h * w;
+  const int p = root_list[o + i];
   const double s = own_sum[o + p];
   const int c = own_cnt[o + p];
   int a = p;
@@ -434,8 +446,8 @@
 constexpr int kContourWarps = 4;
 template <int CAP>
 __global__ void __launch_bounds__(32 * kContourWarps) contour_kernel(int h, int w, int max_cand, const int* __restrict__ total,
-                                                     const int* __restrict__ c_root, const int* __restrict__ rowmin,
-                                                     const int* __restrict__ rowmax, const int* __restrict__ c_yrange,
+                                                     const int* __restrict__ c_root, const int2* __restrict__ rows,
+                                                     const int* __restrict__ c_yrange,
                                                      const double* __restrict__ tot_sum,
                                                      const int* __restrict__ tot_cnt, const double* __restrict__ ring_sum,
                                                      const int* __restrict__ ring_cnt, ContourScratch* __restrict__ scratch,
@@ -472,8 +484,7 @@
   const bool is_hole = entry < 0;
   const int root = entry & 0x7fffffff;
   const size_t o = size_t(page) * h * w;
-  const int* rmin = rowmin + (size_t(page) * max_cand + c) * h;
-  const int* rmax = rowmax + (size_t(page) * max_cand + c) * h;
+  const int2* rr = rows + (size_t(page) * max_cand + c) * h;
   const int y_lo = max(0, c_yrange[(page * max_cand + c) * 2]), y_hi = min(h - 1, c_yrange[(page * max_cand + c) * 2 + 1]);
   int* rbuf = reinterpret_cast<int*>(S.f0);
   int k = 0;
@@ -481,8 +492,8 @@
   for (int y0 = y_lo; y0 <= y_hi; y0 += 64) {
     for (int e = lane; e < 64; e += 32) {
       const int y = y0 + e;
-      rbuf[e] = y <= y_hi ? rmin[y] : INT_MAX;
-      rbuf[64 + e] = y <= y_hi ? rmax[y] : -1;
+      rbuf[e] = y <= y_hi ? rr[y].x : INT_MAX;
+      rbuf[64 + e] = y <= y_hi ? rr[y].y : -1;
     }
     __syncwarp();
     if (lane == 0 && !overflow) {
@@ -504,8 +515,8 @@
   for (int y1 = y_hi; y1 >= y_lo; y1 -= 64) {
     for (int e = lane; e < 64; e += 32) {
       const int y = y1 - e;
-      rbuf[e] = y >= y_lo ? rmin[y] : INT_MAX;
-      rbuf[64 + e] = y >= y_lo ? rmax[y] : -1;
+      rbuf[e] = y >= y_lo ? rr[y].x : INT_MAX;
+      rbuf[64 + e] = y >= y_lo ? rr[y].y : -1;
     }
     __syncwarp();
     if (lane == 0 && !overflow) {
@@ -603,32 +614,30 @@
 
 size_t segrep_scratch_bytes(int n, int h, int w, int max_cand) {
   const size_t hw = size_t(n) * h * w;
-  return hw * 4 * 4
+  return hw * 4 * 5
          + hw * 4 * 2
          + hw * 8 * 3
-         + size_t(n) * max_cand * h * 4 * 2
          + size_t(n) * max_cand * 20
          + size_t(n) * 8192 * 4
          + 65536;
 }
 
 cudaError_t segrep_launch(const uint8_t* bitmap, const float* pred, size_t pred_page_stride, const int* Lf, int n, int h,
-                          int w, int max_cand, float unclip_ratio, void* scratch, int16_t* boxes, float* scores,
-                          int* n_contours, cudaStream_t s) {
+                          int w, int max_cand, float unclip_ratio, void* scratch, int2* rows, int16_t* boxes,
+                          float* scores, int* n_contours, cudaStream_t s) {
   const size_t hw = size_t(h) * w, nhw = size_t(n) * hw;
   char* p = static_cast<char*>(scratch);
   auto take = [&](size_t bytes) { char* r = p; p += (bytes + 255) / 256 * 256; return r; };
   int* Lb = reinterpret_cast<int*>(take(nhw * 4));
   int* parent = reinterpret_cast<int*>(take(nhw * 4));
-  int* flag = reinterpret_cast<int*>(take(nhw * 4));
+  int* cid = reinterpret_cast<int*>(take(nhw * 4));
+  int* root_list = reinterpret_cast<int*>(take(nhw * 4));
   int* own_cnt = reinterpret_cast<int*>(take(nhw * 4));
   int* tot_cnt = reinterpret_cast<int*>(take(nhw * 4));
   int* ring_cnt = reinterpret_cast<int*>(take(nhw * 4));
   double* own_sum = reinterpret_cast<double*>(take(nhw * 8));
   double* tot_sum = reinterpret_cast<double*>(take(nhw * 8));
   double* ring_sum = reinterpret_cast<double*>(take(nhw * 8));
-  int* rowmin = reinterpret_cast<int*>(take(size_t(n) * max_cand * h * 4));
-  int* rowmax = reinterpret_cast<int*>(take(size_t(n) * max_cand * h * 4));
   int* c_root = reinterpret_cast<int*>(take(size_t(n) * max_cand * 4));
   int* c_yrange = reinterpret_cast<int*>(take(size_t(n) * max_cand * 8));
   int* perm = reinterpret_cast<int*>(take(size_t(n) * max_cand * 4));
@@ -639,41 +648,38 @@
   ContourScratch* cs = nullptr;
   const int nseg = int((hw + kSeg - 1) / kSeg);
   if (nseg > 4096) return cudaErrorInvalidValue;
+  if (max_cand > 1024) return cudaErrorInvalidValue;
 
   dim3 tgrid((w + 31) / 32, (h + 31) / 32, n);
   dim3 grid(unsigned((hw + 255) / 256), n);
-  cudaError_t e = cudaMemsetAsync(parent, 0xff, nhw * 4, s);
-  if (e != cudaSuccess) return e;
+  dim3 sgrid(unsigned(nseg), n);
   bg_local_kernel<<<tgrid, 1024, 0, s>>>(bitmap, h, w, Lb);
   const int nborder = ((w - 1) / 32) * h + ((h - 1) / 32) * w;
   if (nborder > 0) bg_border_kernel<<<dim3((nborder + 255) / 256, n), 256, 0, s>>>(h, w, Lb);
-  bg_flatten_kernel<<<grid, 256, 0, s>>>(h, w, Lb);
-  mark_outside_kernel<<<dim3((2 * w + 2 * h + 255) / 256, n), 256, 0, s>>>(h, w, Lb, parent);
-  roots_kernel<<<grid, 256, 0, s>>>(h, w, Lf, Lb, parent, flag, own_sum, own_cnt, tot_sum, tot_cnt, ring_sum, ring_cnt);
-  flag_scan_seg_kernel<<<dim3(nseg, n), 256, 0, s>>>(int(hw), flag, segsum, nseg);
+  bg_flatten_kernel<<<grid, 256, 0, s>>>(h, w, Lb, parent);
+  mark_outside_kernel<<<dim3((max(2 * w + 2 * h, max_cand) + 255) / 256, n), 256, 0, s>>>(h, w, Lb, parent, c_yrange,
+                                                                                          max_cand);
+  roots_kernel<<<sgrid, 256, 0, s>>>(h, w, Lf, Lb, parent, own_sum, own_cnt, tot_sum, tot_cnt, ring_sum, ring_cnt, segsum,
+                                     nseg);
   flag_scan_top_kernel<<<n, 1024, 0, s>>>(segsum, nseg, total);
-  {
-    const size_t nr = size_t(n) * max_cand * h;
-    rows_init_kernel<<<unsigned((nr + 255) / 256), 256, 0, s>>>(rowmin, rowmax, nr, c_yrange, size_t(n) * max_cand);
-  }
-  assign_cid_kernel<<<grid, 256, 0, s>>>(h, w, Lf, flag, segsum, nseg, total, max_cand, c_root, rowmin, rowmax);
-  accumulate_kernel<<<grid, 256, 0, s>>>(h, w, pred, pred_page_stride, Lf, Lb, parent, flag, own_sum, own_cnt, ring_sum,
-                                         ring_cnt, rowmin, rowmax, c_yrange, max_cand);
-  tree_kernel<<<grid, 256, 0, s>>>(h, w, Lf, Lb, parent, own_sum, own_cnt, tot_sum, tot_cnt);
+  assign_cid_kernel<<<sgrid, 256, 0, s>>>(h, w, Lf, Lb, parent, segsum, nseg, total, max_cand, cid, c_root, root_list);
+  accumulate_kernel<<<grid, 256, 0, s>>>(h, w, pred, pred_page_stride, Lf, Lb, parent, cid, own_sum, own_cnt, ring_sum,
+                                         ring_cnt, rows, c_yrange, max_cand);
+  tree_kernel<<<grid, 256, 0, s>>>(h, w, root_list, total, parent, own_sum, own_cnt, tot_sum, tot_cnt);
   constexpr int kCapSmall = 128, kCapLarge = ctdgeom::kMaxHull;
   const size_t sm_small = sizeof(ContourScratchT<kCapSmall>) * kContourWarps, sm_large = sizeof(ContourScratchT<kCapLarge>) * kContourWarps;
   cudaFuncSetAttribute(contour_kernel<kCapLarge>, cudaFuncAttributeMaxDynamicSharedMemorySize, int(sm_large));
-  if (max_cand > 1024) return cudaErrorInvalidValue;
   contour_order_kernel<<<n, 1024, 0, s>>>(max_cand, total, c_yrange, perm);
-  e = cudaMemsetAsync(ovf_count, 0, size_t(n) * 4, s);
+  cudaError_t e = cudaMemsetAsync(ovf_count, 0, size_t(n) * 4, s);
   if (e != cudaSuccess) return e;
   const unsigned cgrid = unsigned((max_cand + kContourWarps - 1) / kContourWarps) * unsigned(n);
   contour_kernel<kCapSmall><<<cgrid, 32 * kContourWarps, sm_small, s>>>(
-      h, w, max_cand, total, c_root, rowmin, rowmax, c_yrange, tot_sum, tot_cnt, ring_sum, ring_cnt, cs, boxes, scores,
+      h, w, max_cand, total, c_root, rows, c_yrange, tot_sum, tot_cnt, ring_sum, ring_cnt, cs, boxes, scores,
       n_contours, w, h, unclip_ratio, perm, n, ovf_count, ovf_list, 0);
   contour_kernel<kCapLarge><<<cgrid, 32 * kContourWarps, sm_large, s>>>(
-      h, w, max_cand, total, c_root, rowmin, rowmax, c_yrange, tot_sum, tot_cnt, ring_sum, ring_cnt, cs, boxes, scores,
+      h, w, max_cand, total, c_root, rows, c_yrange, tot_sum, tot_cnt, ring_sum, ring_cnt, cs, boxes, scores,
       n_contours, w, h, unclip_ratio, perm, n, ovf_count, ovf_list, 1);
+  rows_clear_kernel<<<dim3(max_cand, n), 128, 0, s>>>(h, max_cand, total, c_yrange, rows);
   return cudaGetLastError();
 }
 
```
